# zqqqqz2000/MixGRPO

Hardware: AMD Instinct MI355X
Metric: GRPO train-step images/sec, FLUX.1-dev 1024^2 (higher is better)
Workload: dtype bf16

## Files before the change

### include/mixgrpo_hip.h

```cpp
#ifndef MIXGRPO_HIP_H
#define MIXGRPO_HIP_H
#include <stdint.h>
#ifdef __cplusplus
extern "C" {
#endif

int mgx_version(void);
const char* mgx_last_error(void);

typedef struct {
  float sigma_x0;
  float c_x;
  float c_v;
  float dt_mean;
  float sd_noise;
  float dt_det;
  float den;
  float log_sd;
  float log_c;
} mgx_flow_coeffs;

long mgx_logp_workspace_elems(int B, long n);

int mgx_flow_step_fwd(const float* x, const uint16_t* v, const uint16_t* noise, const float* prev_in,
// ... 11 lines not shown
  float s_b;
  float one_m_s;
  float s_sq;
  float half_eta2;
  float sd;
  float den;
} mgx_dance_coeffs;

int mgx_dance_step_fwd(const float* x, const uint16_t* v, const float* noise, const float* prev_in,
                       float* prev_out, float* x0_out, float* logp, double* ws, int B, long n,
                       const mgx_dance_coeffs* k , int sde, void* stream);
int mgx_dance_step_bwd(const float* x, const uint16_t* v, const float* prev, const float* g_logp, uint16_t* dv,
                       int B, long n, const mgx_dance_coeffs* k , int sde, void* stream);

typedef struct {
  int order;
  int sde;
  float sigma_x0;
  float inv_r0;
  float inv_r1;
  float c_r;
  float inv_r01;
  float cm[4];
  float cx[4];
  float sd_noise;
  float den;
  float log_sd;
  float log_c;
} mgx_dpm_coeffs;

int mgx_dpm_step_fwd(const float* sample, const uint16_t* v, const float* m1, const float* m2, const float* noise,
                     float* x_out, float* x0_out, float* logp, double* ws, int B, long n,
                     const mgx_dpm_coeffs* k , void* stream);

int mgx_dpm_step_bwd(const float* sample, const uint16_t* v, const float* x_t, const float* g_logp, uint16_t* dv, int B,
                     long n, const mgx_dpm_coeffs* k , float sigma_b, void* stream);

int mgx_x0_pred(const float* sample, const uint16_t* v, float* x0_out, long total, float sigma_x0, void* stream);

int mgx_pack_latents(const void* in, void* out, int B, int C, int H, int W, int elem_size, void* stream);
int mgx_unpack_latents(const void* in, void* out, int B, int C, int H, int W, int elem_size, void* stream);

int mgx_group_advantage(const float* rewards, float* out, int n, int G, float trimmed_ratio, float weight,
                        int accumulate, void* stream);
int mgx_global_advantage(const float* rewards, const float* gathered, float* out, int n, int n_all, void* stream);

int mgx_grpo_loss(const float* new_logp, const float* old_logp, const float* adv, int B, float clip_range,
                  float adv_clip_max, float kl_coeff, float denom, float* loss, float* policy, float* kl,
                  float* clip_frac, float* g_logp, void* stream);

enum { MGX_EPI_BIAS = 0, MGX_EPI_BIAS_GELU = 1, MGX_EPI_BIAS_GATE_RES = 2, MGX_EPI_F32_ACC = 3, MGX_EPI_DGELU = 4 };

int mgx_gemm_bf16(const uint16_t* A, const uint16_t* W, const uint16_t* bias, void* C, const uint16_t* gate,
                  uint16_t* aux, long ldaux, int M, int N, int K, long lda, long a_rpb, long a_bstride, long ldw, long ldc,
                  long c_rpb, long c_bstride, long gate_ld, int epilogue, float beta, void* stream);
long mgx_gemm_sk_workspace_elems(void);
int mgx_gemm_bf16_sk(const uint16_t* A, const uint16_t* W, const uint16_t* bias, void* C, const uint16_t* gate,
                     uint16_t* aux, long ldaux, int M, int N, int K, long lda, long a_rpb, long a_bstride, long ldw, long ldc,
                     long c_rpb, long c_bstride, long gate_ld, int epilogue, float beta, float* sk_workspace,
                     long sk_workspace_elems, void* stream);
int mgx_linear_qk_norm_rope(const uint16_t* X, const uint16_t* Wqk, const uint16_t* bias, const float* wq, const float* wk,
                            const float* cos, const float* sin, const float* cos_sin_pairs ,
                            uint16_t* Q, uint16_t* K, int B, int H, int S, int rows_per_batch, int s0, int Kdim, long ldx,
                            long ldw, float q_scale, void* stream);

int mgx_linear_bf16_t(const uint16_t* X, const uint16_t* W, const uint16_t* bias, uint16_t* Ct, int tokens, int F, int K,
                      long ldx, long ldw, long ld_ct, long tok_rpb, long ct_bstride, float* sk_workspace,
                      long sk_workspace_elems, void* stream);

int mgx_gemm_bf16_pair(const uint16_t* A1, const uint16_t* W1, const uint16_t* bias1, void* C1, const uint16_t* gate1,
                       uint16_t* aux1, int M1, long a1_rpb, long a1_bstride, long c1_rpb, long c1_bstride,
                       const uint16_t* A2, const uint16_t* W2, const uint16_t* bias2, void* C2, const uint16_t* gate2,
                       uint16_t* aux2, int M2, long a2_rpb, long a2_bstride, long c2_rpb, long c2_bstride, int N, int K,
                       long lda, long ldw, long ldc, long ldaux, long gate_ld, int epilogue, float beta,
                       float* sk_workspace, long sk_workspace_elems, void* stream);

long mgx_transpose_partial_elems(int M, int N);
int mgx_transpose_bf16(const uint16_t* in, uint16_t* out, float* colsum_partial, float* colsum_out, float colsum_beta,
                       int M, int N, long ld_in, long in_rpb, long in_bstride, long ld_out, void* stream);

int mgx_ln_modulate_fwd(const uint16_t* x, long ldx, long x_rpb, long x_bstride, const uint16_t* shift,
                        const uint16_t* scale, long mod_ld, uint16_t* y, long ldy, float* stats, long M, int D,
                        void* stream);
long mgx_ln_modulate_bwd_workspace(long M, long rpb, int D);
int mgx_ln_modulate_bwd(const uint16_t* dy, long lddy, const uint16_t* x, long ldx, long x_rpb, long x_bstride,
                        const uint16_t* scale, long mod_ld, uint16_t* dx, long lddx, long dx_rpb, long dx_bstride,
                        int accumulate, uint16_t* dshift, uint16_t* dscale, float* ws, long M, int D, void* stream);

int mgx_qk_norm_rope_fwd(const uint16_t* qkv, long ld, const float* wq, const float* wk, const float* cos,
                         const float* sin, uint16_t* Q, uint16_t* K, uint16_t* Vt, uint16_t* V, uint16_t* Qt,
                         uint16_t* Kt, int B, int H, int S, int Sp, int rows_per_batch, int s0, void* stream);
int mgx_qk_norm_rope_fwd_qs(const uint16_t* qkv, long ld, const float* wq, const float* wk, const float* cos,
                            const float* sin, uint16_t* Q, uint16_t* K, uint16_t* Vt, uint16_t* V, uint16_t* Qt,
                            uint16_t* Kt, int B, int H, int S, int Sp, int rows_per_batch, int s0, float q_scale,
                            void* stream);
long mgx_qk_norm_rope_bwd_workspace(int B, int H, int rows_per_batch);
int mgx_qk_norm_rope_bwd(const uint16_t* qkv, long ld, const float* wq, const float* wk, const float* cos,
                         const float* sin, const uint16_t* dQ, const uint16_t* dK, const uint16_t* dV, uint16_t* dqkv,
                         long ld_dqkv , float* gwq, float* gwk, float* ws, int B,
                         int H, int S, int Sp, int rows_per_batch, int s0, void* stream);

int mgx_qk_norm_rope_bwd_qs(const uint16_t* qkv, long ld, const float* wq, const float* wk, const float* cos,
                            const float* sin, const uint16_t* dQ, const uint16_t* dK, const uint16_t* dV, uint16_t* dqkv,
                            long ld_dqkv, float* gwq, float* gwk, float* ws, int B, int H, int S, int Sp,
                            int rows_per_batch, int s0, float q_scale, void* stream);

int mgx_attn_fwd(const uint16_t* Q, const uint16_t* K, const uint16_t* Vt, uint16_t* O, float* lse, int B, int H, int S,
                 int Sp, long ldo, long o_bstride, float scale, void* stream);

int mgx_attn_fwd_log2(const uint16_t* Q2, const uint16_t* K, const uint16_t* Vt, uint16_t* O, float* lse, int B, int H,
                      int S, int Sp, long ldo, long o_bstride, void* stream);

int mgx_attn_fwd_path(int B, int H, int S, int Sp, long ldo, long o_bstride);
int mgx_attn_bwd_path(int B, int H, int S, int Sp, long ldo, long o_bstride);

int mgx_attn_fp8_quantize(const uint16_t* Q, const uint16_t* K, const uint16_t* Vt, uint8_t* Q8, uint8_t* K8,
                          uint8_t* V8t, float* amax, int B, int H, int S, int Sp, void* stream);
int mgx_attn_fwd_fp8(const uint8_t* Q8, const uint8_t* K8, const uint8_t* V8t, const float* amax, uint16_t* O,
                     float* lse, int B, int H, int S, int Sp, long ldo, long o_bstride, float scale, void* stream);

int mgx_attn_bwd(const uint16_t* Q, const uint16_t* K, const uint16_t* V, const uint16_t* Qt, const uint16_t* Kt,
                 const uint16_t* O, const uint16_t* dO, const float* lse, float* delta, uint16_t* dOt, uint16_t* dQ,
                 uint16_t* dK, uint16_t* dV, int B, int H, int S, int Sp, long ldo, long o_bstride, float scale,
                 void* stream);

int mgx_skinny_linear(const uint16_t* x, long ldx, const uint16_t* W, long ldw, const uint16_t* bias, uint16_t* out,
                      long ldo, int Bn, int N, int K, void* stream);
int mgx_skinny_wgrad(const uint16_t* dout, long ldd, const uint16_t* x, long ldx, float* dW, long ldw, float* dbias,
                     int Bn, int N, int K, void* stream);
long mgx_skinny_dgrad_workspace(int Bn, int K);
int mgx_skinny_dgrad(const uint16_t* dout, long ldd, const uint16_t* W, long ldw, uint16_t* dx, long lddx, float* ws,
                     int Bn, int N, int K, int accumulate, void* stream);
int mgx_ew_bf16(const uint16_t* a, const uint16_t* b, uint16_t* y, long n, int op, void* stream);
int mgx_sincos_embed(const float* t, uint16_t* out, int Bn, void* stream);
int mgx_cast_f32_bf16(const float* x, uint16_t* y, long n, void* stream);
int mgx_cast_bf16_f32(const uint16_t* x, float* y, long n, float scale, void* stream);
int mgx_transpose_gelu_bf16(const uint16_t* in, uint16_t* out, int M, int N, long ld_in, long ld_out, void* stream);
int mgx_gelu_bf16(const uint16_t* x, long ldx, uint16_t* y, long ldy, long M, int N, void* stream);
long mgx_gate_bwd_workspace(long batches, long rows_per_batch, int D);
int mgx_gate_bwd(const uint16_t* dout, long ldd, long d_bstride, const uint16_t* y, long ldy, const uint16_t* gate,
                 long gate_ld, uint16_t* dy, long lddy, uint16_t* dgate, float* ws, int batches, long rows_per_batch,
                 int D, void* stream);

long mgx_sqnorm_workspace(void);
int mgx_sqnorm_f32(const float* g, long n, double* ws, float* out, float beta, void* stream);
int mgx_adamw_step(float* w, uint16_t* w16, const float* g, float* m, float* v, long n, double lr, double beta1,
                   double beta2, double eps, double weight_decay, int step, const float* gnorm_sq, float max_norm,
                   float grad_scale, void* stream);
int mgx_scale_f32(float* x, long n, float s, void* stream);


int mgx_conv3x3_nhwc(const uint16_t* x, const uint16_t* Wt, const uint16_t* bias, uint16_t* out, long ld_out,
                     const uint16_t* ones, int H, int W, int C, int Cout, int residual, void* stream);
long mgx_group_norm_workspace(long M, int C, int G);
int mgx_group_norm_nhwc(const uint16_t* x, long ld, const uint16_t* gamma, const uint16_t* beta, uint16_t* out, long out_row,
                        long out_px, float* ws, int H, int W, int C, int G, float eps, int silu, void* stream);
int mgx_upsample2x_pad_nhwc(const uint16_t* x, uint16_t* out, int H, int W, int C, void* stream);
int mgx_latents_to_pad_nhwc(const float* z, uint16_t* out, int Cin, int H, int W, int C, void* stream);
int mgx_nhwc_to_image(const uint16_t* x, long ld, uint16_t* img, int Cout, int H, int W, void* stream);
int mgx_softmax_rows_f32(const float* S, long lds, uint16_t* P, long ldp, int M, int n, float scale, void* stream);

#ifdef __cplusplus
}
#endif
#endif
```

### mixgrpo_amd/_lib.py

```python
import ctypes as C
import os

import torch

_HERE = os.path.dirname(os.path.abspath(__file__))
LIB_PATH = os.path.join(_HERE, "csrc", "libmixgrpo_hip.so")


class MgxError(RuntimeError):
    pass


class FlowCoeffs(C.Structure):
    _fields_ = [(n, C.c_float) for n in ("sigma_x0", "c_x", "c_v", "dt_mean", "sd_noise", "dt_det", "den", "log_sd",
                                         "log_c")]


class DanceCoeffs(C.Structure):
    _fields_ = [(n, C.c_float) for n in ("ds_r", "s_r", "ds", "ds_b", "s_b", "one_m_s", "s_sq", "half_eta2", "sd", "den")]


class DpmCoeffs(C.Structure):
    _fields_ = [("order", C.c_int), ("sde", C.c_int), ("sigma_x0", C.c_float), ("inv_r0", C.c_float),
                ("inv_r1", C.c_float), ("c_r", C.c_float), ("inv_r01", C.c_float), ("cm", C.c_float * 4),
                ("cx", C.c_float * 4), ("sd_noise", C.c_float), ("den", C.c_float), ("log_sd", C.c_float),
                ("log_c", C.c_float)]


_P = C.c_void_p
_I = C.c_int
_L = C.c_long
_F = C.c_float
_D = C.c_double

SIGNATURES = {
    "mgx_version": (_I, []),
    "mgx_last_error": (C.c_char_p, []),
    "mgx_logp_workspace_elems": (_L, [_I, _L]),
    "mgx_flow_step_fwd": (_I, [_P] * 9 + [_I, _L, C.POINTER(FlowCoeffs), _I, _P]),
    "mgx_flow_step_bwd": (_I, [_P] * 5 + [_I, _L, C.POINTER(FlowCoeffs), _P]),
    "mgx_dance_step_fwd": (_I, [_P] * 8 + [_I, _L, C.POINTER(DanceCoeffs), _I, _P]),
    "mgx_dance_step_bwd": (_I, [_P] * 5 + [_I, _L, C.POINTER(DanceCoeffs), _I, _P]),
    "mgx_dpm_step_fwd": (_I, [_P] * 9 + [_I, _L, C.POINTER(DpmCoeffs), _P]),
    "mgx_dpm_step_bwd": (_I, [_P] * 5 + [_I, _L, C.POINTER(DpmCoeffs), _F, _P]),
    "mgx_x0_pred": (_I, [_P, _P, _P, _L, _F, _P]),
    "mgx_pack_latents": (_I, [_P, _P, _I, _I, _I, _I, _I, _P]),
    "mgx_unpack_latents": (_I, [_P, _P, _I, _I, _I, _I, _I, _P]),
    "mgx_group_advantage": (_I, [_P, _P, _I, _I, _F, _F, _I, _P]),
    "mgx_global_advantage": (_I, [_P, _P, _P, _I, _I, _P]),
    "mgx_grpo_loss": (_I, [_P, _P, _P, _I, _F, _F, _F, _F, _P, _P, _P, _P, _P, _P]),
    "mgx_gemm_bf16": (_I, [_P] * 6 + [_L, _I, _I, _I] + [_L] * 8 + [_I, _F, _P]),
    "mgx_gemm_sk_workspace_elems": (_L, []),
    "mgx_gemm_bf16_sk": (_I, [_P] * 6 + [_L, _I, _I, _I] + [_L] * 8 + [_I, _F, _P, _L, _P]),
    "mgx_linear_bf16_t": (_I, [_P] * 4 + [_I] * 3 + [_L] * 5 + [_P, _L, _P]),
    "mgx_linear_qk_norm_rope": (_I, [_P] * 10 + [_I] * 6 + [_L, _L, _F, _P]),
    "mgx_gemm_bf16_pair": (_I, ([_P] * 6 + [_I] + [_L] * 4) * 2 + [_I, _I] + [_L] * 5 + [_I, _F, _P, _L, _P]),
    "mgx_transpose_partial_elems": (_L, [_I, _I]),
    "mgx_transpose_bf16": (_I, [_P, _P, _P, _P, _F, _I, _I, _L, _L, _L, _L, _P]),
    "mgx_ln_modulate_fwd": (_I, [_P, _L, _L, _L, _P, _P, _L, _P, _L, _P, _L, _I, _P]),
    "mgx_ln_modulate_bwd_workspace": (_L, [_L, _L, _I]),
    "mgx_ln_modulate_bwd": (_I, [_P, _L, _P, _L, _L, _L, _P, _L, _P, _L, _L, _L, _I, _P, _P, _P, _L, _I, _P]),
    "mgx_qk_norm_rope_fwd": (_I, [_P, _L] + [_P] * 10 + [_I] * 6 + [_P]),
    "mgx_qk_norm_rope_fwd_qs": (_I, [_P, _L] + [_P] * 10 + [_I] * 6 + [_F, _P]),
    "mgx_qk_norm_rope_bwd_workspace": (_L, [_I, _I, _I]),
    "mgx_qk_norm_rope_bwd": (_I, [_P, _L] + [_P] * 8 + [_L] + [_P] * 3 + [_I] * 6 + [_P]),
    "mgx_qk_norm_rope_bwd_qs": (_I, [_P, _L] + [_P] * 8 + [_L] + [_P] * 3 + [_I] * 6 + [_F, _P]),
    "mgx_attn_fwd": (_I, [_P] * 5 + [_I] * 4 + [_L, _L, _F, _P]),
    "mgx_attn_fwd_log2": (_I, [_P] * 5 + [_I] * 4 + [_L, _L, _P]),
    "mgx_attn_fwd_path": (_I, [_I] * 4 + [_L, _L]),
    "mgx_attn_bwd_path": (_I, [_I] * 4 + [_L, _L]),
    "mgx_attn_fp8_quantize": (_I, [_P] * 7 + [_I] * 4 + [_P]),
    "mgx_attn_fwd_fp8": (_I, [_P] * 6 + [_I] * 4 + [_L, _L, _F, _P]),
    "mgx_attn_bwd": (_I, [_P] * 13 + [_I] * 4 + [_L, _L, _F, _P]),
    "mgx_skinny_linear": (_I, [_P, _L, _P, _L, _P, _P, _L, _I, _I, _I, _P]),
    "mgx_skinny_wgrad": (_I, [_P, _L, _P, _L, _P, _L, _P, _I, _I, _I, _P]),
    "mgx_skinny_dgrad_workspace": (_L, [_I, _I]),
    "mgx_conv3x3_nhwc": (_I, [_P, _P, _P, _P, _L, _P, _I, _I, _I, _I, _I, _P]),
    "mgx_group_norm_workspace": (_L, [_L, _I, _I]),
    "mgx_group_norm_nhwc": (_I, [_P, _L, _P, _P, _P, _L, _L, _P, _I, _I, _I, _I, _F, _I, _P]),
    "mgx_upsample2x_pad_nhwc": (_I, [_P, _P, _I, _I, _I, _P]),
    "mgx_latents_to_pad_nhwc": (_I, [_P, _P, _I, _I, _I, _I, _P]),
    "mgx_nhwc_to_image": (_I, [_P, _L, _P, _I, _I, _I, _P]),
    "mgx_softmax_rows_f32": (_I, [_P, _L, _P, _L, _I, _I, _F, _P]),
    "mgx_skinny_dgrad": (_I, [_P, _L, _P, _L, _P, _L, _P, _I, _I, _I, _I, _P]),
    "mgx_ew_bf16": (_I, [_P, _P, _P, _L, _I, _P]),
    "mgx_sincos_embed": (_I, [_P, _P, _I, _P]),
    "mgx_cast_f32_bf16": (_I, [_P, _P, _L, _P]),
    "mgx_cast_bf16_f32": (_I, [_P, _P, _L, _F, _P]),
    "mgx_gelu_bf16": (_I, [_P, _L, _P, _L, _L, _I, _P]),
    "mgx_transpose_gelu_bf16": (_I, [_P, _P, _I, _I, _L, _L, _P]),
    "mgx_gate_bwd_workspace": (_L, [_L, _L, _I]),
    "mgx_gate_bwd": (_I, [_P, _L, _L, _P, _L, _P, _L, _P, _L, _P, _P, _I, _L, _I, _P]),
    "mgx_sqnorm_workspace": (_L, []),
    "mgx_sqnorm_f32": (_I, [_P, _L, _P, _P, _F, _P]),
    "mgx_adamw_step": (_I, [_P, _P, _P, _P, _P, _L, _D, _D, _D, _D, _D, _I, _P, _F, _F, _P]),
    "mgx_scale_f32": (_I, [_P, _L, _F, _P]),
}

_lib = None


def lib():
    global _lib
    if _lib is None:
        if not os.path.exists(LIB_PATH):
            raise MgxError(f"{LIB_PATH} is missing: run `python -m mixgrpo_amd.build` (hipcc, gfx950). "
                           "There is no CPU fallback for the product path.")
        h = C.CDLL(LIB_PATH)
        h.mgx_version.restype = _I
        v = h.mgx_version()
        if v < 0:
            raise MgxError(f"{LIB_PATH} is a DIAGNOSTIC build (mgx_version() = {v}, -DMGX_DIAGNOSTIC_BUILD): its timing-only "
                           "switches compute wrong results.  Rebuild with `python -m mixgrpo_amd.build --force`.")
        for name, (res, args) in SIGNATURES.items():
            fn = getattr(h, name)
            fn.restype = res
            fn.argtypes = args
        _lib = h
    return _lib


def check(code):
    if code != 0:
        raise MgxError(f"libmixgrpo_hip error {code}: {lib().mgx_last_error().decode()}")


def ptr(t):
    if t is None:
        return None
    if not t.is_cuda:
        raise MgxError("mixgrpo_amd HIP ops need device tensors (got a CPU tensor); there is no CPU path")
    if not t.is_contiguous():
        raise MgxError("mixgrpo_amd HIP ops need contiguous tensors")
    return t.data_ptr()


def stream():
    return torch.cuda.current_stream().cuda_stream


_ws_cache = {}


def logp_workspace(B, n, device):
    need = lib().mgx_logp_workspace_elems(B, n)
    key = (device, torch.cuda.current_stream().cuda_stream)
    w = _ws_cache.get(key)
    if w is None or w.numel() < need:
        w = torch.empty(max(need, 4096), dtype=torch.float64, device=device)
        _ws_cache[key] = w
    return w
```

### mixgrpo_amd/csrc/gemm.hip

```cpp
#include "../../include/mixgrpo_hip.h"
#include "common.h"

#include <cmath>
#include <cstdlib>

namespace {

constexpr int BM = 128, BN = 128, BK = 64;
constexpr int NT = 256;

struct RowMap {
  long ld;
  long rpb;
  long bstride;
};

__device__ __forceinline__ long row_off(const RowMap& r, long m) {
  const uint32_t rpb = (uint32_t)r.rpb;
  const uint32_t b = (uint32_t)m / rpb;
  return (long)b * r.bstride + (long)((uint32_t)m - b * rpb) * r.ld;
}

enum Epi { EPI_BIAS = 0, EPI_BIAS_GELU = 1, EPI_BIAS_GATE_RES = 2, EPI_F32_ACC = 3, EPI_BIAS_MULAUX = 4,
           EPI_QKNORM = 5 ,
           EPI_QKNORM_P = 6  };

struct GemmArgs {
  const bf16_raw* A;
  const bf16_raw* W;
  const bf16_raw* bias;
  void* C;
  const bf16_raw* gate;
  bf16_raw* aux;
  long ldaux;
  long gate_ld;
  int M, N, K;
  RowMap a, c;
  long ldw;
  float beta;
  int rowwise_ok;
  int span32;
  int band;
  int conv_shift;
  long conv_dy, conv_dx;
  float* sk_ws;
  int sk_minparts;
  int m_split;
  long a1_off, w1_off;
  long a2_off, w2_off;
  RowMap a2, c2;
  void* C2;
  const bf16_raw* bias2;
  const bf16_raw* gate2;
  bf16_raw* aux2;
  int bias_rows;
  long col_rpb, col_bstride;
  const float* qn_wq;
  const float* qn_wk;
  const float* qn_cos;
  const float* qn_sin;
  const float* qn_cs2;
  bf16_raw* qn_Q;
  bf16_raw* qn_K;
  int qn_H, qn_S, qn_s0, qn_dmodel;
  float qn_qscale;
};

template <bool PAIR>
__device__ __forceinline__ GemmArgs seg_args(const GemmArgs& g, long& m0) {
  if (!PAIR || g.m_split == 0 || m0 < g.m_split) {
    GemmArgs r = g;
    if (PAIR && g.m_split) r.M = g.m_split;
    return r;
  }
  GemmArgs r = g;
  r.C = g.C2; r.c = g.c2; r.bias = g.bias2; r.gate = g.gate2; r.aux = g.aux2;
  r.M = g.M - g.m_split;
  m0 -= g.m_split;
  return r;
}

template <bool CONV>
__device__ __forceinline__ long a_koff(const GemmArgs& g, int kt) {
  if (!CONV) return (long)kt * BK;
// ... 152 lines not shown
    *reinterpret_cast<uint4*>(base_ + 2 * RS * 128) = ra2;                       \
    *reinterpret_cast<uint4*>(base_ + 3 * RS * 128) = ra3;                       \
    *reinterpret_cast<uint4*>(base_ + TB) = rw0;                                 \
    *reinterpret_cast<uint4*>(base_ + TB + RS * 128) = rw1;                      \
    *reinterpret_cast<uint4*>(base_ + TB + 2 * RS * 128) = rw2;                  \
    *reinterpret_cast<uint4*>(base_ + TB + 3 * RS * 128) = rw3;                  \
  } while (0)

  f32x4 acc[NTL][MT];
#pragma unroll
  for (int i = 0; i < NTL; ++i)
#pragma unroll
    for (int j = 0; j < MT; ++j) acc[i][j] = f32x4{0.f, 0.f, 0.f, 0.f};

  const int fr = lane & 15, fq = lane >> 4;
  const int nkt = g.K / BK;
  LOAD_TILE(0);
  STORE_TILE(0);
  __syncthreads();
  int cur = 0;
  for (int kt = 0; kt < nkt; ++kt) {
    if (kt + 1 < nkt) LOAD_TILE(kt + 1);
    const char* sa = smem + cur * STAGE;
    const char* sw = sa + TB;
    s16x8 fa[2][MT], fw[2][NTL];
#pragma unroll
    for (int ks = 0; ks < 2; ++ks) {
#pragma unroll
      for (int t = 0; t < NTL; ++t) {
        const int rw_ = wn * 64 + t * 16 + fr;
        fw[ks][t] = *reinterpret_cast<const s16x8*>(sw + rw_ * 128 + swz(rw_, ks * 4 + fq) * 16);
      }
#pragma unroll
      for (int t = 0; t < MT; ++t) {
        const int ra_ = wm * (MT * 16) + t * 16 + fr;
        fa[ks][t] = *reinterpret_cast<const s16x8*>(sa + ra_ * 128 + swz(ra_, ks * 4 + fq) * 16);
      }
    }
#pragma unroll
    for (int ks = 0; ks < 2; ++ks) {
#pragma unroll
      for (int j = 0; j < MT; ++j)
#pragma unroll
        for (int i = 0; i < NTL; ++i)
          acc[i][j] = __builtin_amdgcn_mfma_f32_16x16x32_bf16(fw[ks][i], fa[ks][j], acc[i][j], 0, 0, 0);
    }
    if (kt + 1 < nkt) STORE_TILE(cur ^ 1);
    __syncthreads();
    cur ^= 1;
  }
#undef LOAD_TILE
#undef STORE_TILE

  gemm_epilogue<EPI, MT, NTL>(g, acc, lane, m0, n0, wm, wn);
}

__global__ void __launch_bounds__(256) transpose_kernel(const bf16_raw* __restrict__ in, bf16_raw* __restrict__ out,
                                                        float* __restrict__ part, int M, int N, RowMap im, long ldo) {
  __shared__ bf16_raw tile[64][66];
  const int m0 = blockIdx.y * 64, n0 = blockIdx.x * 64;
  const int tx = threadIdx.x & 63, ty = threadIdx.x >> 6;
  for (int r = ty; r < 64; r += 4) {
    const long m = m0 + r;
    const int n = n0 + tx;
    bf16_raw v = 0;
    if (m < M && n < N) v = in[row_off(im, m) + n];
    tile[r][tx] = v;
  }
  __syncthreads();
  for (int r = ty; r < 64; r += 4) {
    const int n = n0 + r;
    const long m = m0 + tx;
    if (n < N && m < ldo) out[(long)n * ldo + m] = (m < M) ? tile[tx][r] : (bf16_raw)0;
  }
  if (part && m0 < M) {
    if (ty == 0) {
      float s = 0.f;
      for (int r = 0; r < 64; ++r) s += bf2f(tile[r][tx]);
      if (n0 + tx < N) part[(long)blockIdx.y * N + n0 + tx] = s;
    }
  }
}

__device__ __forceinline__ uint32_t lo16(uint32_t a, uint32_t b) { return __builtin_amdgcn_perm(b, a, 0x05040100); }
__device__ __forceinline__ uint32_t hi16(uint32_t a, uint32_t b) { return __builtin_amdgcn_perm(b, a, 0x07060302); }
template <bool GELU>
__global__ void __launch_bounds__(256) transpose8_kernel(const bf16_raw* __restrict__ in, bf16_raw* __restrict__ out,
                                                         float* __restrict__ part, int M, int N, RowMap im, long ldo) {
  __shared__ float cs[16][129];
  const int tx = (threadIdx.x & 7) | (((threadIdx.x >> 6) & 1) << 3), ty = ((threadIdx.x >> 3) & 7) | ((threadIdx.x >> 7) << 3);
  const int n0 = blockIdx.x * 128 + tx * 8;
  const long m0 = (long)blockIdx.y * 128 + ty * 8;
  uint32_t r[8][4];
  float csum[8];
#pragma unroll
  for (int j = 0; j < 8; ++j) csum[j] = 0.f;
  const bool ncol_ok = n0 < N;
#pragma unroll
  for (int i = 0; i < 8; ++i) {
    const long m = m0 + i;
    uint4 v = make_uint4(0, 0, 0, 0);
    if (ncol_ok && m < M) v = *reinterpret_cast<const uint4*>(in + row_off(im, m) + n0);
    if (GELU && ncol_ok && m < M) {
      auto gl = [](uint32_t u) {
        return (uint32_t)f2bf(gelu_tanh_f(bf2f(u & 0xffff))) | ((uint32_t)f2bf(gelu_tanh_f(bf2f(u >> 16))) << 16);
      };
      v.x = gl(v.x); v.y = gl(v.y); v.z = gl(v.z); v.w = gl(v.w);
    }
    r[i][0] = v.x; r[i][1] = v.y; r[i][2] = v.z; r[i][3] = v.w;
    if (part) {
      csum[0] += bf2f(v.x & 0xffff); csum[1] += bf2f(v.x >> 16); csum[2] += bf2f(v.y & 0xffff); csum[3] += bf2f(v.y >> 16);
      csum[4] += bf2f(v.z & 0xffff); csum[5] += bf2f(v.z >> 16); csum[6] += bf2f(v.w & 0xffff); csum[7] += bf2f(v.w >> 16);
    }
  }
  if (ncol_ok && m0 < ldo) {
#pragma unroll
    for (int c2 = 0; c2 < 4; ++c2) {
      uint4 e, o;
      e.x = lo16(r[0][c2], r[1][c2]); e.y = lo16(r[2][c2], r[3][c2]); e.z = lo16(r[4][c2], r[5][c2]); e.w = lo16(r[6][c2], r[7][c2]);
      o.x = hi16(r[0][c2], r[1][c2]); o.y = hi16(r[2][c2], r[3][c2]); o.z = hi16(r[4][c2], r[5][c2]); o.w = hi16(r[6][c2], r[7][c2]);
      *reinterpret_cast<uint4*>(out + (long)(n0 + 2 * c2) * ldo + m0) = e;
      *reinterpret_cast<uint4*>(out + (long)(n0 + 2 * c2 + 1) * ldo + m0) = o;
    }
  }
  if (part) {
#pragma unroll
    for (int j = 0; j < 8; ++j) cs[ty][tx * 8 + j] = csum[j];
    __syncthreads();
    if (threadIdx.x < 128) {
      float t = 0.f;
#pragma unroll
      for (int k = 0; k < 16; ++k) t += cs[k][threadIdx.x];
      const int n = blockIdx.x * 128 + threadIdx.x;
      if (n < N && (long)blockIdx.y * 128 < M) part[(long)blockIdx.y * N + n] = t;
    }
  }
}

__global__ void __launch_bounds__(256) colsum_finish_kernel(const float* __restrict__ part, float* __restrict__ out, int nblk,
                                                            int N, float beta) {
  __shared__ float red[4][64];
  const int cx = threadIdx.x & 63, ky = threadIdx.x >> 6;
  const int n = blockIdx.x * 64 + cx;
  float s = 0.f;
  if (n < N)
    for (int b = ky; b < nblk; b += 4) s += part[(long)b * N + n];
  red[ky][cx] = s;
  __syncthreads();
  if (ky == 0 && n < N) out[n] = beta * out[n] + ((red[0][cx] + red[1][cx]) + (red[2][cx] + red[3][cx]));
}

__device__ __forceinline__ int wperm(int p) { return (p >> 5) * 32 + ((p & 15) >> 2) * 8 + ((p >> 4) & 1) * 4 + (p & 3); }
__device__ __forceinline__ int lane_feat(int fq, int t) { return (t >> 1) * 32 + fq * 8 + (t & 1) * 4; }

__device__ __forceinline__ void unpack8(const uint4& u, float* v) {
  v[0] = bf2f(u.x & 0xffff); v[1] = bf2f(u.x >> 16); v[2] = bf2f(u.y & 0xffff); v[3] = bf2f(u.y >> 16);
  v[4] = bf2f(u.z & 0xffff); v[5] = bf2f(u.z >> 16); v[6] = bf2f(u.w & 0xffff); v[7] = bf2f(u.w >> 16);
}
__device__ __forceinline__ uint4 pack8(const float* v) {
  uint4 o;
  o.x = (uint32_t)f2bf(v[0]) | ((uint32_t)f2bf(v[1]) << 16);
  o.y = (uint32_t)f2bf(v[2]) | ((uint32_t)f2bf(v[3]) << 16);
  o.z = (uint32_t)f2bf(v[4]) | ((uint32_t)f2bf(v[5]) << 16);
  o.w = (uint32_t)f2bf(v[6]) | ((uint32_t)f2bf(v[7]) << 16);
  return o;
}

__device__ __forceinline__ float vmul1(float a, float b) { float r; asm("v_mul_f32 %0, %1, %2" : "=v"(r) : "v"(a), "v"(b)); return r; }
// ... 926 lines not shown
  MGX_REQUIRE(X && Wqk && wq && wk && cos && sin && Q && K, "null argument");
  MGX_REQUIRE(!cos_sin_pairs || (uintptr_t)cos_sin_pairs % 16 == 0, "pair table must be 16-byte aligned");
  MGX_REQUIRE(B > 0 && H > 0 && rows_per_batch > 0 && s0 >= 0 && s0 + rows_per_batch <= S && Kdim > 0 && q_scale > 0.f, "bad sizes");
  static const int off = getenv("MGX_GEMM_QKNORM") ? atoi(getenv("MGX_GEMM_QKNORM")) == 0 : 0;
  const long tokens = (long)B * rows_per_batch;
  const int dmodel = H * 128;
  const bool ok = !off && dmodel % 256 == 0 && rows_per_batch % 128 == 0 && Kdim % BK == 0 && ldx % 8 == 0 && ldw % 8 == 0 &&
                  tokens < (1L << 31) && ((uintptr_t)X % 16 == 0) && ((uintptr_t)Wqk % 16 == 0) && ((uintptr_t)Q % 16 == 0) &&
                  ((uintptr_t)K % 16 == 0) && ((uintptr_t)cos % 16 == 0) && ((uintptr_t)sin % 16 == 0) &&
                  ((uintptr_t)wq % 16 == 0) && ((uintptr_t)wk % 16 == 0) && (!bias || (uintptr_t)bias % 16 == 0);
  if (!ok) return 1;
  GemmArgs g{};
  g.A = X; g.W = Wqk; g.bias = bias; g.C = Q;
  g.M = (int)tokens; g.N = 2 * dmodel; g.K = Kdim;
  g.a = RowMap{ldx, 1L << 30, 0};
  g.c = RowMap{128, rows_per_batch, 0};
  g.ldw = ldw;
  g.conv_shift = -1;
  g.rowwise_ok = 1;
  g.span32 = (tokens * ldx) * 2 < (1L << 32) && ((long)g.N * ldw) * 2 < (1L << 32);
  g.qn_wq = wq; g.qn_wk = wk; g.qn_cos = cos; g.qn_sin = sin; g.qn_cs2 = cos_sin_pairs; g.qn_Q = Q; g.qn_K = K;
  g.qn_H = H; g.qn_S = S; g.qn_s0 = s0; g.qn_dmodel = dmodel; g.qn_qscale = q_scale;
  if (!persistent_ok(g)) return 1;
  return cos_sin_pairs ? launch<EPI_QKNORM_P>(g, (hipStream_t)stream) : launch<EPI_QKNORM>(g, (hipStream_t)stream);
}

extern "C" int mgx_gemm_bf16(const uint16_t* A, const uint16_t* W, const uint16_t* bias, void* C, const uint16_t* gate,
                             uint16_t* aux, long ldaux, int M, int N, int K, long lda, long a_rpb, long a_bstride, long ldw, long ldc,
                             long c_rpb, long c_bstride, long gate_ld, int epilogue, float beta, void* stream) {
  return mgx_gemm_bf16_sk(A, W, bias, C, gate, aux, ldaux, M, N, K, lda, a_rpb, a_bstride, ldw, ldc, c_rpb, c_bstride, gate_ld,
                          epilogue, beta, nullptr, 0, stream);
}

extern "C" int mgx_conv3x3_nhwc(const uint16_t* x, const uint16_t* Wt, const uint16_t* bias, uint16_t* out, long ld_out,
                                const uint16_t* ones, int H, int Wd, int C, int Cout, int residual, void* stream) {
  MGX_REQUIRE(x && Wt && out && H > 0 && Wd > 0, "bad argument");
  MGX_REQUIRE(C == 64 || C == 128 || C == 256 || C == 512, "channels per tap must be 64, 128, 256 or 512 (pad with zeros)");
  MGX_REQUIRE(Cout > 0 && Cout % 4 == 0 && ld_out >= Cout && ld_out % 4 == 0, "output channels must be a multiple of 4");
  MGX_REQUIRE(!residual || ones, "the residual form needs a vector of Cout ones (bf16)");
  MGX_REQUIRE(((uintptr_t)x % 16 == 0) && ((uintptr_t)Wt % 16 == 0) && ((uintptr_t)out % 8 == 0), "operands must be 16-byte aligned");
  const long Wp = Wd + 2;
  MGX_REQUIRE((long)(H + 2) * Wp * C * 2 < (1L << 32) && (long)Cout * 9 * C * 2 < (1L << 32), "image too large for one call");
  GemmArgs g{};
  g.A = x; g.W = Wt; g.bias = bias; g.C = out; g.gate = residual ? ones : nullptr; g.aux = nullptr; g.ldaux = 0; g.gate_ld = 0;
  g.M = H * Wd; g.N = Cout; g.K = 9 * C;
  g.a = RowMap{C, Wd, Wp * C};
  g.c = RowMap{ld_out, 1L << 30, 0};
  g.ldw = 9L * C;
  g.beta = 0.f;
  g.conv_shift = C == 64 ? 0 : (C == 128 ? 1 : (C == 256 ? 2 : 3));
  g.conv_dy = Wp * C; g.conv_dx = C;
  g.sk_ws = nullptr; g.sk_minparts = 0; g.m_split = 0;
  g.rowwise_ok = (Cout % 8 == 0) && (ld_out % 8 == 0) && ((uintptr_t)out % 16 == 0) && (!bias || (uintptr_t)bias % 16 == 0) &&
                 (!residual || (uintptr_t)ones % 16 == 0);
  g.span32 = 1;
  hipStream_t st = (hipStream_t)stream;
  return residual ? launch<EPI_BIAS_GATE_RES, true>(g, st) : launch<EPI_BIAS, true>(g, st);
}

extern "C" long mgx_transpose_partial_elems(int M, int N) { return (long)cdiv(M, 64) * N; }

extern "C" int mgx_transpose_bf16(const uint16_t* in, uint16_t* out, float* colsum_partial, float* colsum_out,
                                  float colsum_beta, int M, int N, long ld_in, long in_rpb, long in_bstride, long ld_out,
                                  void* stream) {
  MGX_REQUIRE(in && out && M > 0 && N > 0, "bad argument");
  MGX_REQUIRE(ld_out >= M, "output leading dimension must cover M");
  MGX_REQUIRE((colsum_partial == nullptr) == (colsum_out == nullptr), "column sums need both workspace and output");
  hipStream_t st = (hipStream_t)stream;
  const bool fast = N % 8 == 0 && ld_in % 8 == 0 && in_bstride % 8 == 0 && ld_out % 8 == 0 &&
                    ((uintptr_t)in % 16 == 0) && ((uintptr_t)out % 16 == 0);
  if (fast) {
    dim3 grid(cdiv(N, 128), cdiv(ld_out, 128));
    transpose8_kernel<false><<<grid, 256, 0, st>>>(in, out, colsum_partial, M, N, RowMap{ld_in, in_rpb < (1L << 30) ? in_rpb : (1L << 30), in_bstride}, ld_out);
    if (colsum_out) colsum_finish_kernel<<<cdiv(N, 64), 256, 0, st>>>(colsum_partial, colsum_out, cdiv(M, 128), N, colsum_beta);
  } else {
    dim3 grid(cdiv(N, 64), cdiv(ld_out, 64));
    transpose_kernel<<<grid, 256, 0, st>>>(in, out, colsum_partial, M, N, RowMap{ld_in, in_rpb < (1L << 30) ? in_rpb : (1L << 30), in_bstride}, ld_out);
    if (colsum_out) colsum_finish_kernel<<<cdiv(N, 64), 256, 0, st>>>(colsum_partial, colsum_out, cdiv(M, 64), N, colsum_beta);
  }
  MGX_CHECK_LAUNCH();
  return MGX_OK;
}

extern "C" int mgx_transpose_gelu_bf16(const uint16_t* in, uint16_t* out, int M, int N, long ld_in, long ld_out, void* stream) {
  MGX_REQUIRE(in && out && M > 0 && N > 0, "bad argument");
  MGX_REQUIRE(ld_out >= M, "output leading dimension must cover M");
  MGX_REQUIRE(N % 8 == 0 && ld_in % 8 == 0 && ld_out % 8 == 0 && ((uintptr_t)in % 16 == 0) && ((uintptr_t)out % 16 == 0),
              "rows must be 16-byte addressable");
  dim3 grid(cdiv(N, 128), cdiv(ld_out, 128));
  transpose8_kernel<true><<<grid, 256, 0, (hipStream_t)stream>>>(in, out, nullptr, M, N, RowMap{ld_in, 1L << 30, 0}, ld_out);
  MGX_CHECK_LAUNCH();
  return MGX_OK;
}

extern "C" int mgx_gelu_bf16(const uint16_t* x, long ldx, uint16_t* y, long ldy, long M, int N, void* stream) {
  MGX_REQUIRE(x && y && M > 0 && N > 0, "bad argument");
  MGX_REQUIRE(N % 8 == 0 && ldx % 8 == 0 && ldy % 8 == 0 && ((uintptr_t)x % 16 == 0) && ((uintptr_t)y % 16 == 0),
              "rows must be 16-byte addressable");
  const long total = M * (N / 8);
  const int grid = (int)((total + 255) / 256 < 256L * 32 ? (total + 255) / 256 : 256L * 32);
  gelu_rows_kernel<<<grid, 256, 0, (hipStream_t)stream>>>(x, ldx, y, ldy, M, N / 8);
  MGX_CHECK_LAUNCH();
  return MGX_OK;
}
```

### mixgrpo_amd/csrc/norm.hip

```cpp
#include "../../include/mixgrpo_hip.h"
#include "common.h"

namespace {

struct RowMap {
  long ld, rpb, bstride;
};
__device__ __forceinline__ long row_off(const RowMap& r, long m) {
  const long b = m / r.rpb;
  return b * r.bstride + (m - b * r.rpb) * r.ld;
}

constexpr int LN_MAXV = 8;

__device__ __forceinline__ void unpack8(const uint4& u, float* f) {
  f[0] = bf2f(u.x & 0xffff); f[1] = bf2f(u.x >> 16); f[2] = bf2f(u.y & 0xffff); f[3] = bf2f(u.y >> 16);
  f[4] = bf2f(u.z & 0xffff); f[5] = bf2f(u.z >> 16); f[6] = bf2f(u.w & 0xffff); f[7] = bf2f(u.w >> 16);
}
__device__ __forceinline__ uint4 pack8(const float* f) {
  uint4 u;
  u.x = (uint32_t)f2bf(f[0]) | ((uint32_t)f2bf(f[1]) << 16);
  u.y = (uint32_t)f2bf(f[2]) | ((uint32_t)f2bf(f[3]) << 16);
  u.z = (uint32_t)f2bf(f[4]) | ((uint32_t)f2bf(f[5]) << 16);
  u.w = (uint32_t)f2bf(f[6]) | ((uint32_t)f2bf(f[7]) << 16);
  return u;
}

template <int NV>
__global__ void __launch_bounds__(256) ln_mod_fwd_kernel(const bf16_raw* __restrict__ x, RowMap xm,
                                                         const bf16_raw* __restrict__ shift,
                                                         const bf16_raw* __restrict__ scale, long mod_ld,
                                                         bf16_raw* __restrict__ y, long ldy, float* __restrict__ stats,
                                                         long M) {
  const long m = (long)blockIdx.x * 4 + (threadIdx.x >> 6);
  if (m >= M) return;
  const int lane = threadIdx.x & 63;
  const long b = m / xm.rpb;
  const bf16_raw* xr = x + row_off(xm, m);
  float v[NV][8];
  float s = 0.f;
#pragma unroll
  for (int i = 0; i < NV; ++i) {
    unpack8(*reinterpret_cast<const uint4*>(xr + (i * 64 + lane) * 8), v[i]);
#pragma unroll
    for (int j = 0; j < 8; ++j) s += v[i][j];
  }
  const float D = (float)(NV * 512);
  const float mean = wave_sum(s) / D;
  float q = 0.f;
#pragma unroll
  for (int i = 0; i < NV; ++i)
#pragma unroll
    for (int j = 0; j < 8; ++j) {
      const float d = v[i][j] - mean;
      q += d * d;
    }
  const float rstd = rsqrtf(wave_sum(q) / D + 1e-6f);
  if (stats && lane == 0) {
    stats[2 * m] = mean;
    stats[2 * m + 1] = rstd;
  }
  const bf16_raw* sh = shift + b * mod_ld;
  const bf16_raw* sc = scale + b * mod_ld;
#pragma unroll
  for (int i = 0; i < NV; ++i) {
    const int c = (i * 64 + lane) * 8;
    float fs[8], fc[8], o[8];
    unpack8(*reinterpret_cast<const uint4*>(sh + c), fs);
    unpack8(*reinterpret_cast<const uint4*>(sc + c), fc);
#pragma unroll
    for (int j = 0; j < 8; ++j) o[j] = (v[i][j] - mean) * rstd * rbf(1.0f + fc[j]) + fs[j];
    *reinterpret_cast<uint4*>(y + m * ldy + c) = pack8(o);
  }
}

constexpr int LN_BWD_ROWS = 32;
template <int NV>
__global__ void __launch_bounds__(256) ln_mod_bwd_kernel(const bf16_raw* __restrict__ dy, long lddy,
                                                         const bf16_raw* __restrict__ x, RowMap xm,
                                                         const bf16_raw* __restrict__ scale, long mod_ld,
                                                         bf16_raw* __restrict__ dx, RowMap dxm, int accumulate,
                                                         float* __restrict__ part, long M, int blocks_per_batch) {
  extern __shared__ float red[];
  const int D = NV * 512;
  const int lane = threadIdx.x & 63, w = threadIdx.x >> 6;
  const long b = blockIdx.x / blocks_per_batch;
  const long r0 = (long)(blockIdx.x % blocks_per_batch) * LN_BWD_ROWS;
  const bf16_raw* sc = scale + b * mod_ld;
  float a_sh[NV][8], a_sc[NV][8];
#pragma unroll
  for (int i = 0; i < NV; ++i)
#pragma unroll
    for (int j = 0; j < 8; ++j) a_sh[i][j] = a_sc[i][j] = 0.f;

  auto row_ok = [&](int rr) { return rr < LN_BWD_ROWS && r0 + rr < xm.rpb && b * xm.rpb + r0 + rr < M; };
  uint4 nx[NV], ng[NV], nold[NV];
  auto fetch = [&](int rr) {
    const long m = b * xm.rpb + r0 + rr;
    const bf16_raw* xr = x + row_off(xm, m);
    const bf16_raw* dxr = dx + row_off(dxm, m);
#pragma unroll
    for (int i = 0; i < NV; ++i) {
      nx[i] = *reinterpret_cast<const uint4*>(xr + (i * 64 + lane) * 8);
      ng[i] = *reinterpret_cast<const uint4*>(dy + m * lddy + (i * 64 + lane) * 8);
      nold[i] = accumulate ? *reinterpret_cast<const uint4*>(dxr + (i * 64 + lane) * 8) : make_uint4(0, 0, 0, 0);
    }
  };
  if (row_ok(w)) fetch(w);
  for (int rr = w; row_ok(rr); rr += 4) {
    const long m = b * xm.rpb + r0 + rr;
    bf16_raw* dxr = dx + row_off(dxm, m);
    float v[NV][8], g[NV][8];
    uint4 oldp[NV];
    float s = 0.f;
#pragma unroll
    for (int i = 0; i < NV; ++i) {
      unpack8(nx[i], v[i]);
      unpack8(ng[i], g[i]);
      oldp[i] = nold[i];
#pragma unroll
      for (int j = 0; j < 8; ++j) s += v[i][j];
    }
    if (row_ok(rr + 4)) fetch(rr + 4);
    const float Df = (float)D;
    const float mean = wave_sum(s) / Df;
    float q = 0.f;
#pragma unroll
    for (int i = 0; i < NV; ++i)
#pragma unroll
      for (int j = 0; j < 8; ++j) {
        const float d = v[i][j] - mean;
        q += d * d;
      }
    const float rstd = rsqrtf(wave_sum(q) / Df + 1e-6f);
    float c1 = 0.f, c2 = 0.f;
#pragma unroll
    for (int i = 0; i < NV; ++i) {
      float fc[8];
      unpack8(*reinterpret_cast<const uint4*>(sc + (i * 64 + lane) * 8), fc);
#pragma unroll
      for (int j = 0; j < 8; ++j) {
        const float xh = (v[i][j] - mean) * rstd;
        const float gx = g[i][j] * rbf(1.0f + fc[j]);
        a_sh[i][j] += g[i][j];
        a_sc[i][j] += g[i][j] * xh;
        c1 += gx;
        c2 += gx * xh;
        v[i][j] = xh;
        g[i][j] = gx;
      }
    }
    c1 = wave_sum(c1) / Df;
    c2 = wave_sum(c2) / Df;
#pragma unroll
    for (int i = 0; i < NV; ++i) {
      float o[8];
// ... 96 lines not shown
    float2 cc[U], ss[U];
    bool ok[U];
#pragma unroll
    for (int u = 0; u < U; ++u) {
      const int t = t0 + w * 16 + i0 + u;
      ok[u] = t < a.rows_per_batch;
      const int tc = ok[u] ? t : a.rows_per_batch - 1;
      const long row = (long)b * a.rows_per_batch + tc;
      const bf16_raw* base = a.qkv + row * a.ld + hh * HD + 2 * lane;
      uq[u] = *reinterpret_cast<const uint32_t*>(base);
      uk[u] = *reinterpret_cast<const uint32_t*>(base + dmodel);
      uv[u] = has_v ? *reinterpret_cast<const uint32_t*>(base + 2 * dmodel) : 0u;
      const long so = (long)(a.s0 + tc) * HD + 2 * lane;
      cc[u] = *reinterpret_cast<const float2*>(a.cos + so);
      ss[u] = *reinterpret_cast<const float2*>(a.sin + so);
    }
#pragma unroll
    for (int u = 0; u < U; ++u) {
      if (!ok[u]) continue;
      const int tl = w * 16 + i0 + u;
      const int s = a.s0 + t0 + tl;
      if (has_v) *reinterpret_cast<uint32_t*>(&vt[tl][2 * lane]) = uv[u];
      const float c0 = cc[u].x, c1 = cc[u].y, s0 = ss[u].x, s1 = ss[u].y;
      const long o = (((long)b * a.H + hh) * a.S + s) * HD + 2 * lane;
      {
        const float x0 = bf2f(uq[u] & 0xffff), x1 = bf2f(uq[u] >> 16);
        const float r = rsqrtf(head_sum(x0 * x0 + x1 * x1) / 128.f + 1e-6f);
        const float y0 = x0 * r * wq0, y1 = x1 * r * wq1;
        const uint32_t pk = (uint32_t)f2bf(y0 * c0 - y1 * s0) | ((uint32_t)f2bf(y1 * c1 + y0 * s1) << 16);
        *reinterpret_cast<uint32_t*>(a.Q + o) = pk;
        if (EMIT_T) *reinterpret_cast<uint32_t*>(&qts[tl][2 * lane]) = pk;
      }
      {
        const float x0 = bf2f(uk[u] & 0xffff), x1 = bf2f(uk[u] >> 16);
        const float r = rsqrtf(head_sum(x0 * x0 + x1 * x1) / 128.f + 1e-6f);
        const float y0 = x0 * r * wk0, y1 = x1 * r * wk1;
        const uint32_t pk = (uint32_t)f2bf(y0 * c0 - y1 * s0) | ((uint32_t)f2bf(y1 * c1 + y0 * s1) << 16);
        *reinterpret_cast<uint32_t*>(a.K + o) = pk;
        if (EMIT_T) *reinterpret_cast<uint32_t*>(&kts[tl][2 * lane]) = pk;
      }
      if (EMIT_T) *reinterpret_cast<uint32_t*>(a.V + o) = uv[u];
    }
  }
  if (!EMIT_T && !has_v) return;
  __syncthreads();
  const int ntok = min(64, a.rows_per_batch - t0);
  const int nmat = EMIT_T ? 3 : 1;
  for (int mat = 0; mat < nmat; ++mat) {
    bf16_raw (*tile)[130] = mat == 0 ? vt : (mat == 1 ? qts : kts);
    bf16_raw* outp = mat == 0 ? a.Vt : (mat == 1 ? a.Qt : a.Kt);
    for (int id = threadIdx.x; id < 128 * 8; id += 256) {
      const int d = id >> 3, c = id & 7;
      bf16_raw* dst = outp + (((long)b * a.H + hh) * HD + d) * a.Sp + a.s0 + t0 + c * 8;
      if (c * 8 + 8 <= ntok && (((a.s0 + t0) & 7) == 0)) {
        uint4 u;
        u.x = (uint32_t)tile[c * 8 + 0][d] | ((uint32_t)tile[c * 8 + 1][d] << 16);
        u.y = (uint32_t)tile[c * 8 + 2][d] | ((uint32_t)tile[c * 8 + 3][d] << 16);
        u.z = (uint32_t)tile[c * 8 + 4][d] | ((uint32_t)tile[c * 8 + 5][d] << 16);
        u.w = (uint32_t)tile[c * 8 + 6][d] | ((uint32_t)tile[c * 8 + 7][d] << 16);
        *reinterpret_cast<uint4*>(dst) = u;
      } else {
        for (int j = 0; j < 8; ++j)
          if (c * 8 + j < ntok) dst[j] = tile[c * 8 + j][d];
      }
    }
  }
}

struct QkBwdArgs {
  const bf16_raw* qkv;
  long ld;
  const float* wq;
  const float* wk;
  const float* cos;
  const float* sin;
  const bf16_raw* dQ;
  const bf16_raw* dK;
  const bf16_raw* dV;
  bf16_raw* dqkv;
  long ldo;
  float* part;
  int H, S, Sp, rows_per_batch, s0;
  float q_scale;
};

__global__ void __launch_bounds__(256) qk_norm_rope_bwd_kernel(QkBwdArgs a) {
  __shared__ float red[4][2][128];
  const int lane = threadIdx.x & 63, w = threadIdx.x >> 6;
  const int hh = blockIdx.y, b = blockIdx.z;
  const int t0 = blockIdx.x * 64;
  const int HD = 128;
  const long dmodel = (long)a.H * HD;
  const float wq0 = a.wq[2 * lane], wq1 = a.wq[2 * lane + 1];
  const float wk0 = a.wk[2 * lane], wk1 = a.wk[2 * lane + 1];
  float gq0 = 0.f, gq1 = 0.f, gk0 = 0.f, gk1 = 0.f;
  constexpr int U = 4;
  for (int i0 = 0; i0 < 16; i0 += U) {
    uint32_t ux[U][2], ug[U][2], uv[U];
    float2 cc[U], ss[U];
    bool ok[U];
#pragma unroll
    for (int u = 0; u < U; ++u) {
      const int t = t0 + w * 16 + i0 + u;
      ok[u] = t < a.rows_per_batch;
      const int tc = ok[u] ? t : a.rows_per_batch - 1;
      const long row = (long)b * a.rows_per_batch + tc;
      const int s = a.s0 + tc;
      const bf16_raw* base = a.qkv + row * a.ld + hh * HD + 2 * lane;
      const long o = (((long)b * a.H + hh) * a.S + s) * HD + 2 * lane;
      ux[u][0] = *reinterpret_cast<const uint32_t*>(base);
      ux[u][1] = *reinterpret_cast<const uint32_t*>(base + dmodel);
      ug[u][0] = *reinterpret_cast<const uint32_t*>(a.dQ + o);
      ug[u][1] = *reinterpret_cast<const uint32_t*>(a.dK + o);
      uv[u] = *reinterpret_cast<const uint32_t*>(a.dV + o);
      cc[u] = *reinterpret_cast<const float2*>(a.cos + (long)s * HD + 2 * lane);
      ss[u] = *reinterpret_cast<const float2*>(a.sin + (long)s * HD + 2 * lane);
    }
#pragma unroll
    for (int u = 0; u < U; ++u) {
      if (!ok[u]) continue;
      const int t = t0 + w * 16 + i0 + u;
      const long row = (long)b * a.rows_per_batch + t;
      bf16_raw* obase = a.dqkv + row * a.ldo + hh * HD + 2 * lane;
      const float c0 = cc[u].x, c1 = cc[u].y, s0 = ss[u].x, s1 = ss[u].y;
#pragma unroll
      for (int which = 0; which < 2; ++which) {
        const float w0 = which ? wk0 : wq0, w1 = which ? wk1 : wq1;
        const float x0 = bf2f(ux[u][which] & 0xffff), x1 = bf2f(ux[u][which] >> 16);
        const float gs = which ? 1.f : a.q_scale;
        const float go0 = bf2f(ug[u][which] & 0xffff) * gs, go1 = bf2f(ug[u][which] >> 16) * gs;
        const float gy0 = go0 * c0 + go1 * s1;
        const float gy1 = -go0 * s0 + go1 * c1;
        const float r = rsqrtf(head_sum(x0 * x0 + x1 * x1) / 128.f + 1e-6f);
        if (which) { gk0 += gy0 * x0 * r; gk1 += gy1 * x1 * r; } else { gq0 += gy0 * x0 * r; gq1 += gy1 * x1 * r; }
        const float gz0 = gy0 * w0, gz1 = gy1 * w1;
        const float dot = wave_sum(gz0 * x0 + gz1 * x1) / 128.f;
        const float dx0 = r * gz0 - x0 * r * r * r * dot;
        const float dx1 = r * gz1 - x1 * r * r * r * dot;
        *reinterpret_cast<uint32_t*>(obase + which * dmodel) = (uint32_t)f2bf(dx0) | ((uint32_t)f2bf(dx1) << 16);
      }
      *reinterpret_cast<uint32_t*>(obase + 2 * dmodel) = uv[u];
    }
  }
  red[w][0][2 * lane] = gq0; red[w][0][2 * lane + 1] = gq1;
  red[w][1][2 * lane] = gk0; red[w][1][2 * lane + 1] = gk1;
  __syncthreads();
  const long blk = ((long)blockIdx.z * gridDim.y + blockIdx.y) * gridDim.x + blockIdx.x;
  {
    const int which = threadIdx.x >> 7, c = threadIdx.x & 127;
    a.part[(blk * 2 + which) * 128 + c] = red[0][which][c] + red[1][which][c] + red[2][which][c] + red[3][which][c];
  }
}

constexpr int QK_FIN_G = 128;
__global__ void __launch_bounds__(256) qk_bwd_partial_kernel(const float* __restrict__ part, float* __restrict__ mid,
                                                             long nblocks) {
  float s = 0.f;
  for (long k = blockIdx.x; k < nblocks; k += QK_FIN_G) s += part[k * 256 + threadIdx.x];
  mid[(long)blockIdx.x * 256 + threadIdx.x] = s;
}

__global__ void __launch_bounds__(256) qk_bwd_finish_kernel(const float* __restrict__ part, float* __restrict__ gq,
                                                            float* __restrict__ gk, long nblocks) {
  __shared__ float red[16][17];
  const int which = blockIdx.x >> 3, c0 = (blockIdx.x & 7) * 16;
  const int cx = threadIdx.x & 15, ry = threadIdx.x >> 4;
  float s = 0.f;
  for (long k = ry; k < nblocks; k += 16) s += part[(k * 2 + which) * 128 + c0 + cx];
  red[ry][cx] = s;
  __syncthreads();
  if (ry == 0) {
    float t = 0.f;
#pragma unroll
    for (int i = 0; i < 16; ++i) t += red[i][cx];
    float* dst = which ? gk : gq;
    dst[c0 + cx] += t;
  }
}

}

extern "C" int mgx_ln_modulate_fwd(const uint16_t* x, long ldx, long x_rpb, long x_bstride, const uint16_t* shift,
                                   const uint16_t* scale, long mod_ld, uint16_t* y, long ldy, float* stats, long M, int D,
                                   void* stream) {
  MGX_REQUIRE(x && shift && scale && y && M > 0, "bad argument");
  MGX_REQUIRE(D % 512 == 0 && D <= 4096, "feature size must be a multiple of 512 up to 4096");
  MGX_REQUIRE(ldx % 8 == 0 && ldy % 8 == 0 && mod_ld % 8 == 0 && x_bstride % 8 == 0, "16-byte row alignment");
  hipStream_t st = (hipStream_t)stream;
  const RowMap xm{ldx, x_rpb, x_bstride};
  const int grid = cdiv(M, 4);
  switch (D / 512) {
#define CASE(nv) case nv: ln_mod_fwd_kernel<nv><<<grid, 256, 0, st>>>(x, xm, shift, scale, mod_ld, y, ldy, stats, M); break;
    CASE(1) CASE(2) CASE(3) CASE(4) CASE(5) CASE(6) CASE(7) CASE(8)
#undef CASE
  }
  MGX_CHECK_LAUNCH();
  return MGX_OK;
}

extern "C" long mgx_ln_modulate_bwd_workspace(long M, long rpb, int D) {
  const long batches = (M + rpb - 1) / rpb;
  const long bpb = ((rpb < M ? rpb : M) + LN_BWD_ROWS - 1) / LN_BWD_ROWS;
  return batches * bpb * 2 * D;
}

extern "C" int mgx_ln_modulate_bwd(const uint16_t* dy, long lddy, const uint16_t* x, long ldx, long x_rpb, long x_bstride,
                                   const uint16_t* scale, long mod_ld, uint16_t* dx, long lddx, long dx_rpb,
                                   long dx_bstride, int accumulate, uint16_t* dshift, uint16_t* dscale, float* ws, long M,
                                   int D, void* stream) {
  MGX_REQUIRE(dy && x && scale && dx && dshift && dscale && ws && M > 0, "bad argument");
  MGX_REQUIRE(D % 512 == 0 && D <= 4096, "feature size must be a multiple of 512 up to 4096");
  MGX_REQUIRE(x_rpb == dx_rpb, "x and dx must be batched alike");
  hipStream_t st = (hipStream_t)stream;
  const long rpb = x_rpb < M ? x_rpb : M;
  const int batches = cdiv(M, rpb);
  const int bpb = cdiv(rpb, LN_BWD_ROWS);
  const RowMap xm{ldx, rpb, x_bstride}, dxm{lddx, rpb, dx_bstride};
  const size_t lds = (size_t)2 * D * sizeof(float);
  switch (D / 512) {
#define CASE(nv)                                                                                                  \
  case nv:                                                                                                        \
    ln_mod_bwd_kernel<nv><<<batches * bpb, 256, lds, st>>>(dy, lddy, x, xm, scale, mod_ld, dx, dxm, accumulate, ws, M, bpb); \
    break;
    CASE(1) CASE(2) CASE(3) CASE(4) CASE(5) CASE(6) CASE(7) CASE(8)
#undef CASE
  }
  ln_mod_bwd_finish_kernel<<<dim3(cdiv(D, 64), batches), 256, 0, st>>>(ws, dshift, dscale, mod_ld, D, bpb);
  MGX_CHECK_LAUNCH();
  return MGX_OK;
}

extern "C" int mgx_qk_norm_rope_fwd_qs(const uint16_t* qkv, long ld, const float* wq, const float* wk, const float* cos,
                                       const float* sin, uint16_t* Q, uint16_t* K, uint16_t* Vt, uint16_t* V, uint16_t* Qt,
                                       uint16_t* Kt, int B, int H, int S, int Sp, int rows_per_batch, int s0, float q_scale,
                                       void* stream) {
  MGX_REQUIRE(qkv && wq && wk && cos && sin && Q && K, "null argument");
  MGX_REQUIRE((V != nullptr) == (Qt != nullptr) && (V != nullptr) == (Kt != nullptr), "V, Qt, Kt come together");
  MGX_REQUIRE(Vt || !V, "Vt may only be left out (V^T written by mgx_linear_bf16_t) without the backward's extra layouts");
  MGX_REQUIRE(B > 0 && H > 0 && rows_per_batch > 0 && s0 >= 0 && s0 + rows_per_batch <= S && Sp >= S, "bad sizes");
  MGX_REQUIRE(ld == 3L * H * 128, "qkv rows must be [q | k | v] of H*128 each");
  MGX_REQUIRE(q_scale > 0.f, "q_scale must be positive");
  QkArgs a{qkv, ld, wq, wk, cos, sin, Q, K, Vt, V, Qt, Kt, H, S, Sp, rows_per_batch, s0, q_scale};
  dim3 grid(cdiv(rows_per_batch, 64), H, B);
  if (V) qk_norm_rope_fwd_kernel<true><<<grid, 256, 0, (hipStream_t)stream>>>(a);
  else qk_norm_rope_fwd_kernel<false><<<grid, 256, 0, (hipStream_t)stream>>>(a);
  MGX_CHECK_LAUNCH();
  return MGX_OK;
}

extern "C" int mgx_qk_norm_rope_fwd(const uint16_t* qkv, long ld, const float* wq, const float* wk, const float* cos,
                                    const float* sin, uint16_t* Q, uint16_t* K, uint16_t* Vt, uint16_t* V, uint16_t* Qt,
                                    uint16_t* Kt, int B, int H, int S, int Sp, int rows_per_batch, int s0, void* stream) {
  return mgx_qk_norm_rope_fwd_qs(qkv, ld, wq, wk, cos, sin, Q, K, Vt, V, Qt, Kt, B, H, S, Sp, rows_per_batch, s0, 1.0f, stream);
}

extern "C" long mgx_qk_norm_rope_bwd_workspace(int B, int H, int rows_per_batch) {
  return ((long)cdiv(rows_per_batch, 64) * H * B + QK_FIN_G) * 2 * 128;
}

extern "C" int mgx_qk_norm_rope_bwd_qs(const uint16_t* qkv, long ld, const float* wq, const float* wk, const float* cos,
                                       const float* sin, const uint16_t* dQ, const uint16_t* dK, const uint16_t* dV,
                                       uint16_t* dqkv, long ld_dqkv, float* gwq, float* gwk, float* ws, int B, int H, int S,
                                       int Sp, int rows_per_batch, int s0, float q_scale, void* stream) {
  MGX_REQUIRE(qkv && wq && wk && cos && sin && dQ && dK && dV && dqkv && gwq && gwk && ws, "null argument");
  MGX_REQUIRE(ld == 3L * H * 128, "qkv rows must be [q | k | v] of H*128 each");
  MGX_REQUIRE(ld_dqkv >= ld && ld_dqkv % 2 == 0, "dqkv rows must hold [dq | dk | dv] and keep 4-byte alignment");
  hipStream_t st = (hipStream_t)stream;
  QkBwdArgs a{qkv, ld, wq, wk, cos, sin, dQ, dK, dV, dqkv, ld_dqkv, ws, H, S, Sp, rows_per_batch, s0, q_scale};
  dim3 grid(cdiv(rows_per_batch, 64), H, B);
  qk_norm_rope_bwd_kernel<<<grid, 256, 0, st>>>(a);
  const long nblocks = (long)grid.x * grid.y * grid.z;
  float* mid = ws + nblocks * 256;
  qk_bwd_partial_kernel<<<QK_FIN_G, 256, 0, st>>>(ws, mid, nblocks);
  qk_bwd_finish_kernel<<<16, 256, 0, st>>>(mid, gwq, gwk, QK_FIN_G);
  MGX_CHECK_LAUNCH();
  return MGX_OK;
}

extern "C" int mgx_qk_norm_rope_bwd(const uint16_t* qkv, long ld, const float* wq, const float* wk, const float* cos,
                                    const float* sin, const uint16_t* dQ, const uint16_t* dK, const uint16_t* dV,
                                    uint16_t* dqkv, long ld_dqkv, float* gwq, float* gwk, float* ws, int B, int H, int S,
                                    int Sp, int rows_per_batch, int s0, void* stream) {
  return mgx_qk_norm_rope_bwd_qs(qkv, ld, wq, wk, cos, sin, dQ, dK, dV, dqkv, ld_dqkv, gwq, gwk, ws, B, H, S, Sp, rows_per_batch,
                                 s0, 1.0f, stream);
}
```

### mixgrpo_amd/csrc/small.hip

```cpp
#include "../../include/mixgrpo_hip.h"
#include "common.h"

namespace {

__global__ void __launch_bounds__(256) skinny_linear_kernel(const bf16_raw* __restrict__ x, long ldx,
                                                            const bf16_raw* __restrict__ W, long ldw,
                                                            const bf16_raw* __restrict__ bias,
                                                            bf16_raw* __restrict__ out, long ldo, int Bn, int N, int K) {
  __shared__ f32x4 red[3][64];
  const int lane = threadIdx.x & 63, w = threadIdx.x >> 6;
  const int n0 = blockIdx.x * 16;
  const int fr = lane & 15, fq = lane >> 4;
  int nrow = n0 + fr;
  if (nrow >= N) nrow = N - 1;
  int brow = fr < Bn ? fr : Bn - 1;
  const int kchunk = ((K / 32 + 3) / 4) * 32;
  const int kbeg = min(w * kchunk, K), kend = min(kbeg + kchunk, K);
  const bf16_raw* wp = W + (long)nrow * ldw + fq * 8;
  const bf16_raw* xp = x + (long)brow * ldx + fq * 8;
  f32x4 acc = {0.f, 0.f, 0.f, 0.f};
  int k = kbeg;
  for (; k + 128 <= kend; k += 128) {
    s16x8 a0 = *reinterpret_cast<const s16x8*>(wp + k), a1 = *reinterpret_cast<const s16x8*>(wp + k + 32);
    s16x8 a2 = *reinterpret_cast<const s16x8*>(wp + k + 64), a3 = *reinterpret_cast<const s16x8*>(wp + k + 96);
    s16x8 b0 = *reinterpret_cast<const s16x8*>(xp + k), b1 = *reinterpret_cast<const s16x8*>(xp + k + 32);
    s16x8 b2 = *reinterpret_cast<const s16x8*>(xp + k + 64), b3 = *reinterpret_cast<const s16x8*>(xp + k + 96);
    acc = __builtin_amdgcn_mfma_f32_16x16x32_bf16(a0, b0, acc, 0, 0, 0);
    acc = __builtin_amdgcn_mfma_f32_16x16x32_bf16(a1, b1, acc, 0, 0, 0);
    acc = __builtin_amdgcn_mfma_f32_16x16x32_bf16(a2, b2, acc, 0, 0, 0);
    acc = __builtin_amdgcn_mfma_f32_16x16x32_bf16(a3, b3, acc, 0, 0, 0);
  }
  for (; k < kend; k += 32) {
    s16x8 a0 = *reinterpret_cast<const s16x8*>(wp + k);
    s16x8 b0 = *reinterpret_cast<const s16x8*>(xp + k);
    acc = __builtin_amdgcn_mfma_f32_16x16x32_bf16(a0, b0, acc, 0, 0, 0);
  }
  if (w > 0) red[w - 1][lane] = acc;
  __syncthreads();
  if (w > 0) return;
#pragma unroll
  for (int i = 0; i < 3; ++i) {
    const f32x4 o = red[i][lane];
    acc[0] += o[0]; acc[1] += o[1]; acc[2] += o[2]; acc[3] += o[3];
  }
  if (fr < Bn) {
#pragma unroll
    for (int r = 0; r < 4; ++r) {
      const int n = n0 + 4 * fq + r;
      if (n < N) {
        float v = acc[r];
        if (bias) v += bf2f(bias[n]);
        out[(long)fr * ldo + n] = f2bf(v);
      }
    }
  }
}

__global__ void __launch_bounds__(256) skinny_wgrad_kernel(const bf16_raw* __restrict__ dout, long ldd,
                                                           const bf16_raw* __restrict__ x, long ldx,
                                                           float* __restrict__ dW, long ldw, float* __restrict__ dbias,
                                                           int Bn, int N, int K) {
  const int n = blockIdx.y;
  float dn[16];
  float sb = 0.f;
#pragma unroll
  for (int b = 0; b < 16; ++b) {
    dn[b] = b < Bn ? bf2f(dout[(long)b * ldd + n]) : 0.f;
    sb += dn[b];
  }
  if (dbias && blockIdx.x == 0 && threadIdx.x == 0) dbias[n] += sb;
  for (int k = (blockIdx.x * 256 + threadIdx.x) * 4; k < K; k += gridDim.x * 256 * 4) {
    float4 g = *reinterpret_cast<float4*>(dW + (long)n * ldw + k);
    for (int b = 0; b < Bn; ++b) {
      const uint2 u = *reinterpret_cast<const uint2*>(x + (long)b * ldx + k);
      g.x += dn[b] * bf2f(u.x & 0xffff); g.y += dn[b] * bf2f(u.x >> 16);
      g.z += dn[b] * bf2f(u.y & 0xffff); g.w += dn[b] * bf2f(u.y >> 16);
    }
    *reinterpret_cast<float4*>(dW + (long)n * ldw + k) = g;
  }
}

constexpr int SD_G = 128;
__global__ void __launch_bounds__(256) skinny_dgrad_kernel(const bf16_raw* __restrict__ dout, long ldd,
                                                           const bf16_raw* __restrict__ W, long ldw, float* __restrict__ part,
// ... 56 lines not shown
  if (id >= (long)Bn * K) return;
  const int b = (int)(id / K), k = (int)(id - (long)b * K);
  float s = 0.f;
  for (int g = 0; g < SD_G; ++g) s += part[((long)g * Bn + b) * K + k];
  bf16_raw* o = dx + (long)b * lddx + k;
  const float r = rbf(s);
  *o = f2bf(accumulate ? bf2f(*o) + r : r);
}

__device__ __forceinline__ float silu_f(float x) { return x / (1.0f + expf(-x)); }

__global__ void ew_kernel(const bf16_raw* __restrict__ a, const bf16_raw* __restrict__ b, bf16_raw* __restrict__ y,
                          long n, int op) {
  for (long i = (long)blockIdx.x * blockDim.x + threadIdx.x; i < n; i += (long)gridDim.x * blockDim.x) {
    const float fa = bf2f(a[i]);
    float r;
    if (op == 0) r = silu_f(fa);
    else if (op == 1) {
      const float s = 1.0f / (1.0f + expf(-fa));
      r = bf2f(b[i]) * (s * (1.0f + fa * (1.0f - s)));
    } else if (op == 2) r = fa + bf2f(b[i]);
    else r = bf2f(y[i]) + fa;
    y[i] = f2bf(r);
  }
}

__global__ void sincos_embed_kernel(const float* __restrict__ t, bf16_raw* __restrict__ out, int Bn) {
  const int b = blockIdx.x, k = threadIdx.x;
  if (b >= Bn) return;
  const float f = expf(-logf(10000.0f) * (float)k / 128.0f);
  const float ang = t[b] * f;
  out[(long)b * 256 + k] = f2bf(cosf(ang));
  out[(long)b * 256 + 128 + k] = f2bf(sinf(ang));
}

__global__ void cast_f32_bf16_kernel(const float* __restrict__ x, bf16_raw* __restrict__ y, long n) {
  for (long i = ((long)blockIdx.x * blockDim.x + threadIdx.x) * 4; i < n; i += (long)gridDim.x * blockDim.x * 4) {
    const float4 v = *reinterpret_cast<const float4*>(x + i);
    uint2 o;
    o.x = (uint32_t)f2bf(v.x) | ((uint32_t)f2bf(v.y) << 16);
    o.y = (uint32_t)f2bf(v.z) | ((uint32_t)f2bf(v.w) << 16);
    *reinterpret_cast<uint2*>(y + i) = o;
  }
}

__global__ void cast_bf16_f32_kernel(const bf16_raw* __restrict__ x, float* __restrict__ y, long n, float scale) {
  for (long i = ((long)blockIdx.x * blockDim.x + threadIdx.x) * 8; i < n; i += (long)gridDim.x * blockDim.x * 8) {
    const uint4 u = *reinterpret_cast<const uint4*>(x + i);
    float4 a, b;
    a.x = bf2f(u.x & 0xffff) * scale; a.y = bf2f(u.x >> 16) * scale; a.z = bf2f(u.y & 0xffff) * scale; a.w = bf2f(u.y >> 16) * scale;
    b.x = bf2f(u.z & 0xffff) * scale; b.y = bf2f(u.z >> 16) * scale; b.z = bf2f(u.w & 0xffff) * scale; b.w = bf2f(u.w >> 16) * scale;
    *reinterpret_cast<float4*>(y + i) = a;
    *reinterpret_cast<float4*>(y + i + 4) = b;
  }
}

constexpr int GR_ROWS = 64;
__global__ void __launch_bounds__(256) gate_bwd_kernel(const bf16_raw* __restrict__ dout, long ldd, long d_rpb,
                                                       long d_bstride, const bf16_raw* __restrict__ y, long ldy,
                                                       const bf16_raw* __restrict__ gate, long gate_ld,
                                                       bf16_raw* __restrict__ dy, long lddy, float* __restrict__ part,
                                                       long rows_per_batch, int D, int blocks_per_batch) {
  const long b = blockIdx.y / blocks_per_batch;
  const long r0 = (long)(blockIdx.y % blocks_per_batch) * GR_ROWS;
  const int c = (blockIdx.x * 256 + threadIdx.x) * 2;
  if (c >= D) return;
  const uint32_t gu = *reinterpret_cast<const uint32_t*>(gate + b * gate_ld + c);
  const float g0 = bf2f(gu & 0xffff), g1 = bf2f(gu >> 16);
  float a0 = 0.f, a1 = 0.f;
  const long rend = min(r0 + (long)GR_ROWS, rows_per_batch);
  for (long r = r0; r < rend; ++r) {
    const long m = b * rows_per_batch + r;
    const uint32_t du = *reinterpret_cast<const uint32_t*>(dout + b * d_bstride + r * ldd + c);
    const uint32_t yu = *reinterpret_cast<const uint32_t*>(y + m * ldy + c);
    const float d0 = bf2f(du & 0xffff), d1 = bf2f(du >> 16);
    a0 += d0 * bf2f(yu & 0xffff);
    a1 += d1 * bf2f(yu >> 16);
    *reinterpret_cast<uint32_t*>(dy + m * lddy + c) = (uint32_t)f2bf(g0 * d0) | ((uint32_t)f2bf(g1 * d1) << 16);
  }
  part[(long)blockIdx.y * D + c] = a0;
  part[(long)blockIdx.y * D + c + 1] = a1;
}

__global__ void __launch_bounds__(256) gate_bwd_finish_kernel(const float* __restrict__ part, bf16_raw* __restrict__ dgate,
                                                              long gate_ld, int D, int blocks_per_batch) {
  __shared__ float red[4][64];
  const int b = blockIdx.y;
  const int cx = threadIdx.x & 63, ky = threadIdx.x >> 6;
  const int c = blockIdx.x * 64 + cx;
  float s = 0.f;
  if (c < D)
    for (int k = ky; k < blocks_per_batch; k += 4) s += part[((long)b * blocks_per_batch + k) * D + c];
  red[ky][cx] = s;
  __syncthreads();
  if (ky == 0 && c < D) dgate[(long)b * gate_ld + c] = f2bf((red[0][cx] + red[1][cx]) + (red[2][cx] + red[3][cx]));
}

}

extern "C" int mgx_skinny_linear(const uint16_t* x, long ldx, const uint16_t* W, long ldw, const uint16_t* bias,
                                 uint16_t* out, long ldo, int Bn, int N, int K, void* stream) {
  MGX_REQUIRE(x && W && out, "null operand");
  MGX_REQUIRE(Bn >= 1 && Bn <= 16, "skinny linear handles 1..16 rows");
  MGX_REQUIRE(K % 32 == 0 && ldx % 8 == 0 && ldw % 8 == 0, "K must be a multiple of 32 with 16-byte aligned rows");
  skinny_linear_kernel<<<cdiv(N, 16), 256, 0, (hipStream_t)stream>>>(x, ldx, W, ldw, bias, out, ldo, Bn, N, K);
  MGX_CHECK_LAUNCH();
  return MGX_OK;
}

extern "C" int mgx_skinny_wgrad(const uint16_t* dout, long ldd, const uint16_t* x, long ldx, float* dW, long ldw,
                                float* dbias, int Bn, int N, int K, void* stream) {
  MGX_REQUIRE(dout && x && dW, "null operand");
  MGX_REQUIRE(Bn >= 1 && Bn <= 16, "skinny wgrad handles 1..16 rows");
  MGX_REQUIRE(K % 4 == 0 && ldx % 4 == 0 && ldw % 4 == 0, "K must be a multiple of 4");
  int gx = cdiv(K, 1024);
  skinny_wgrad_kernel<<<dim3(gx, N), 256, 0, (hipStream_t)stream>>>(dout, ldd, x, ldx, dW, ldw, dbias, Bn, N, K);
  MGX_CHECK_LAUNCH();
  return MGX_OK;
}

extern "C" long mgx_skinny_dgrad_workspace(int Bn, int K) { return (long)SD_G * (Bn < 8 ? Bn : 8) * K; }

extern "C" int mgx_skinny_dgrad(const uint16_t* dout, long ldd, const uint16_t* W, long ldw, uint16_t* dx, long lddx,
                                float* ws, int Bn, int N, int K, int accumulate, void* stream) {
  MGX_REQUIRE(dout && W && dx && ws, "null operand");
  MGX_REQUIRE(Bn >= 1 && Bn <= 8, "skinny dgrad handles 1..8 rows per call");
  MGX_REQUIRE(N >= SD_G && K % 8 == 0 && ldw % 8 == 0 && ((uintptr_t)W % 16 == 0), "weight rows must be 16-byte addressable");
  hipStream_t st = (hipStream_t)stream;
  const size_t lds = (size_t)cdiv(N, SD_G) * 8 * sizeof(float);
  MGX_REQUIRE(lds <= 65536, "too many weight rows");
  skinny_dgrad_kernel<<<dim3(cdiv(K, 2048), SD_G), 256, lds, st>>>(dout, ldd, W, ldw, ws, Bn, N, K);
  skinny_dgrad_finish_kernel<<<cdiv((long)Bn * K, 256), 256, 0, st>>>(ws, dx, lddx, Bn, K, accumulate);
  MGX_CHECK_LAUNCH();
  return MGX_OK;
}

extern "C" int mgx_ew_bf16(const uint16_t* a, const uint16_t* b, uint16_t* y, long n, int op, void* stream) {
  MGX_REQUIRE(a && y && n > 0 && op >= 0 && op <= 3, "bad argument");
  MGX_REQUIRE(op == 0 || op == 3 || b, "binary op needs b");
  int nb = cdiv(n, 256);
  if (nb > 2048) nb = 2048;
  ew_kernel<<<nb, 256, 0, (hipStream_t)stream>>>(a, b, y, n, op);
  MGX_CHECK_LAUNCH();
  return MGX_OK;
}

extern "C" int mgx_sincos_embed(const float* t, uint16_t* out, int Bn, void* stream) {
  MGX_REQUIRE(t && out && Bn > 0, "bad argument");
  sincos_embed_kernel<<<Bn, 128, 0, (hipStream_t)stream>>>(t, out, Bn);
  MGX_CHECK_LAUNCH();
  return MGX_OK;
}

extern "C" int mgx_cast_f32_bf16(const float* x, uint16_t* y, long n, void* stream) {
  MGX_REQUIRE(x && y && n > 0 && n % 4 == 0, "bad argument");
  int nb = cdiv(n, 1024);
  if (nb > 4096) nb = 4096;
  cast_f32_bf16_kernel<<<nb, 256, 0, (hipStream_t)stream>>>(x, y, n);
  MGX_CHECK_LAUNCH();
  return MGX_OK;
}

extern "C" int mgx_cast_bf16_f32(const uint16_t* x, float* y, long n, float scale, void* stream) {
  MGX_REQUIRE(x && y && n > 0 && n % 8 == 0, "bad argument");
  MGX_REQUIRE(((uintptr_t)x % 16 == 0) && ((uintptr_t)y % 16 == 0), "operands must be 16-byte aligned");
  int nb = cdiv(n, 2048);
  if (nb > 4096) nb = 4096;
  cast_bf16_f32_kernel<<<nb, 256, 0, (hipStream_t)stream>>>(x, y, n, scale);
  MGX_CHECK_LAUNCH();
  return MGX_OK;
}

extern "C" long mgx_gate_bwd_workspace(long batches, long rows_per_batch, int D) {
  return batches * ((rows_per_batch + GR_ROWS - 1) / GR_ROWS) * D;
}

extern "C" int mgx_gate_bwd(const uint16_t* dout, long ldd, long d_bstride, const uint16_t* y, long ldy,
                            const uint16_t* gate, long gate_ld, uint16_t* dy, long lddy, uint16_t* dgate, float* ws,
                            int batches, long rows_per_batch, int D, void* stream) {
  MGX_REQUIRE(dout && y && gate && dy && dgate && ws, "null operand");
  MGX_REQUIRE(D % 2 == 0 && batches > 0 && rows_per_batch > 0, "bad sizes");
  const int bpb = cdiv(rows_per_batch, GR_ROWS);
  hipStream_t st = (hipStream_t)stream;
  gate_bwd_kernel<<<dim3(cdiv(D, 512), batches * bpb), 256, 0, st>>>(dout, ldd, rows_per_batch, d_bstride, y, ldy, gate,
                                                                      gate_ld, dy, lddy, ws, rows_per_batch, D, bpb);
  gate_bwd_finish_kernel<<<dim3(cdiv(D, 64), batches), 256, 0, st>>>(ws, dgate, gate_ld, D, bpb);
  MGX_CHECK_LAUNCH();
  return MGX_OK;
}
```

### mixgrpo_amd/flux.py

```python
import json
import math
import os
from dataclasses import asdict, dataclass
from typing import Dict, List, Tuple

import torch

from . import ops
from ._lib import MgxError
from .ops import BF16, F32, Rows, EPI_BIAS, EPI_BIAS_GELU, EPI_BIAS_GATE_RES


@dataclass
class FluxConfig:
    patch_size: int = 1
    in_channels: int = 64
    num_layers: int = 19
    num_single_layers: int = 38
    attention_head_dim: int = 128
    num_attention_heads: int = 24
    joint_attention_dim: int = 4096
    pooled_projection_dim: int = 768
    guidance_embeds: bool = True
    axes_dims_rope: Tuple[int, int, int] = (16, 56, 56)
# ... 327 lines not shown
        hit = self._rope_cache.get("k")
        if hit is not None and hit[0] == key:
            return hit[1], hit[2]
        ids = torch.cat([txt_ids.float(), img_ids.float()], dim=0)
        cos, sin = rope_tables(ids, self.cfg.axes_dims_rope)
        self._rope_cache["k"] = (key, cos, sin, txt_ids, img_ids)
        return cos, sin

    def _rope_pairs(self, cos, sin):
        if not ops.ROPE_PAIR_TABLE:
            return None
        hit = self._rope_cache.get("pairs")
        if hit is None or hit[0] is not cos:
            hit = (cos, ops.rope_pair_table(cos, sin))
            self._rope_cache["pairs"] = hit
        return hit[1]

    def _temb(self, B, timestep, guidance, pooled, keep=None):
        d = self.cfg.dim
        dev = self.store.device
        t = (timestep.to(BF16) * 1000).float().contiguous()
        gd = guidance.to(dev)
        gd = (gd.to(BF16) * 1000).float()
        gd = gd.expand(B).contiguous() if gd.numel() == 1 else gd.contiguous()

        def mlp(name, x, K):
            h1 = torch.empty(B, d, dtype=BF16, device=dev)
            ops.skinny_linear(x, self.W(f"time_text_embed.{name}.linear_1.weight"),
                              self.W(f"time_text_embed.{name}.linear_1.bias"), h1, d, K)
            a1 = torch.empty_like(h1)
            ops.ew(h1, None, a1, 0)
            h2 = torch.empty_like(h1)
            ops.skinny_linear(a1, self.W(f"time_text_embed.{name}.linear_2.weight"),
                              self.W(f"time_text_embed.{name}.linear_2.bias"), h2, d, d)
            if keep is not None:
                keep[name] = (x, h1, a1)
            return h2

        te = torch.empty(B, 256, dtype=BF16, device=dev)
        ops.sincos_embed(t, te)
        temb = mlp("timestep_embedder", te, 256)
        if self.cfg.guidance_embeds:
            ge = torch.empty(B, 256, dtype=BF16, device=dev)
            ops.sincos_embed(gd, ge)
            gemb = mlp("guidance_embedder", ge, 256)
            t2 = torch.empty_like(temb)
            ops.ew(temb, gemb, t2, 2)
            temb = t2
        pe = mlp("text_embedder", pooled.to(BF16).contiguous(), self.cfg.pooled_projection_dim)
        t3 = torch.empty_like(temb)
        ops.ew(temb, pe, t3, 2)
        st = torch.empty_like(t3)
        ops.ew(t3, None, st, 0)
        return t3, st

    def _stream_rows(self, t, w, which, width):
        if which == "txt":
            return Rows(t, w.B * w.L, width, w.L, w.S * width)
        return Rows(t[0, w.L:], w.B * w.N, width, w.N, w.S * width)

    def _double_block(self, i, w, st, cos, sin, save=None, mods_in=None, keep=None, replay=False, x_in=None):
        cfg, d, H = self.cfg, self.cfg.dim, self.cfg.num_attention_heads
        p = f"transformer_blocks.{i}"
        B = w.B
        dev = self.store.device
        mods = {}
        streams = (("txt", "norm1_context", ("add_q_proj", "add_k_proj", "add_v_proj"), "norm_added_q", "norm_added_k",
                    "to_add_out", "ff_context", w.L, 0),
                   ("img", "norm1", ("to_q", "to_k", "to_v"), "norm_q", "norm_k", "to_out.0", "ff", w.N, w.L))
        row0 = {"txt": 0, "img": w.B * w.L}
        sl = {n: slice(row0[n], row0[n] + B * r) for n, r in (("txt", w.L), ("img", w.N))}
        W16, fused = self.W, self.store.fused
        qkv_kept = keep is not None and "qkv" in keep
        qkv_buf = keep["qkv"] if qkv_kept else w.qkv
        nrm1 = w.nrm if save is None else save["nrm1"]
        for name, norm, qkvn, nq, nk, outn, ffn, rows, s0 in streams:
            if mods_in is not None:
                m = mods_in[name]
            else:
                m = torch.empty(B, 6 * d, dtype=BF16, device=dev)
                ops.skinny_linear(st, W16(f"{p}.{norm}.linear.weight"), W16(f"{p}.{norm}.linear.bias"), m, 6 * d, d)
            mods[name] = m
            Xs = self._stream_rows(w.X if x_in is None else x_in, w, name, d)
            ops.ln_modulate(Xs, m[:, 0:d], m[:, d:2 * d], 6 * d, nrm1[sl[name]], d)
        nograd = save is None and keep is None
        if nograd:
            for name, _, qkvn, nq, nk, _, _, rows, s0 in streams:
                self._qkv_nograd(nrm1[sl[name]], f"{p}.attn.{qkvn[0]}", qkv_buf[sl[name]], w, rows, s0,
                                 self.W32(f"{p}.attn.{nq}.weight"), self.W32(f"{p}.attn.{nk}.weight"), cos, sin)
        elif not (replay and qkv_kept):
            ops.gemm_pair(*(x for name, _, qkvn, *_ in streams for x in (
                Rows.of(nrm1[sl[name]]), fused(self.store.w16, f"{p}.attn.{qkvn[0]}.weight", 3 * d),
                fused(self.store.w16, f"{p}.attn.{qkvn[0]}.bias", 3 * d), Rows.of(qkv_buf[sl[name]]))), 3 * d, d)
        for name, norm, qkvn, nq, nk, outn, ffn, rows, s0 in (() if nograd else streams):
            ops.qk_norm_rope(qkv_buf[sl[name]], self.W32(f"{p}.attn.{nq}.weight"), self.W32(f"{p}.attn.{nk}.weight"), cos, sin,
                             w.Q, w.K, w.Vt, B, H, w.S, w.Sp, rows, s0, q_scale=self.q_scale(),
                             **({} if save is None else dict(V=save["V"], Qt=save["Qt"], Kt=save["Kt"])))
        O_buf = keep["O"] if keep is not None else w.O
        if not replay:
            self._attn(w, O_buf, keep["lse"] if keep is not None else (w.lse if save is not None else None), d, w.S * d)
        aux1 = aux2 = hpre = None
        if keep is not None and not replay:
            aux1, aux2 = keep["y_attn"], keep["y_ff"]
        elif save is not None:
            aux1, aux2 = save["y_attn"], save["y_ff"]
        ff_kept = keep is not None and "hid_pre" in keep
        if save is not None:
            hpre = save["hid_pre"]
        elif ff_kept:
            hpre = keep["hid_pre"]
        part = lambda t, name: None if t is None else t[sl[name]]
        if not replay:
            ops.gemm_pair(*(x for name, _, _, _, _, outn, *_ in streams for x in (
                self._stream_rows(O_buf, w, name, d), W16(f"{p}.attn.{outn}.weight"), W16(f"{p}.attn.{outn}.bias"),
                self._stream_rows(w.X, w, name, d))), d, d, EPI_BIAS_GATE_RES, gate1=mods["txt"][:, 2 * d:3 * d],
                gate2=mods["img"][:, 2 * d:3 * d], gate_ld=6 * d, aux1=part(aux1, "txt"), aux2=part(aux1, "img"))
            xm = keep["x_mid"] if keep is not None else (save["x_mid"] if save is not None else None)
            if xm is not None:
                xm.copy_(w.X)
        x_mid = keep["x_mid"] if replay else w.X
        nrm2 = w.nrm if save is None else save["nrm2"]
        for name in ("txt", "img"):
            m = mods[name]
            ops.ln_modulate(self._stream_rows(x_mid, w, name, d), m[:, 3 * d:4 * d], m[:, 4 * d:5 * d], 6 * d, nrm2[sl[name]], d)
        if replay and ff_kept:
            pass
        else:
            ops.gemm_pair(*(x for name, _, _, _, _, _, ffn, *_ in streams for x in (
                Rows.of(nrm2[sl[name]]), W16(f"{p}.{ffn}.net.0.proj.weight"), W16(f"{p}.{ffn}.net.0.proj.bias"),
                Rows.of(w.hid[sl[name]]))), 4 * d, d, EPI_BIAS_GELU, aux1=part(hpre, "txt"), aux2=part(hpre, "img"))
        if not replay:
            ops.gemm_pair(*(x for name, _, _, _, _, _, ffn, *_ in streams for x in (
                Rows.of(w.hid[sl[name]]), W16(f"{p}.{ffn}.net.2.weight"), W16(f"{p}.{ffn}.net.2.bias"),
                self._stream_rows(w.X, w, name, d))), d, 4 * d, EPI_BIAS_GATE_RES, gate1=mods["txt"][:, 5 * d:6 * d],
                gate2=mods["img"][:, 5 * d:6 * d], gate_ld=6 * d, aux1=part(aux2, "txt"), aux2=part(aux2, "img"))
        return mods

    def _single_block(self, i, w, st, cos, sin, save=None, mod_in=None, keep=None, replay=False, x_in=None):
        cfg, d, H = self.cfg, self.cfg.dim, self.cfg.num_attention_heads
        p = f"single_transformer_blocks.{i}"
        B, S = w.B, w.S
        M = B * S
        if mod_in is not None:
            m = mod_in
        else:
            m = torch.empty(B, 3 * d, dtype=BF16, device=self.store.device)
            ops.skinny_linear(st, self.W(f"{p}.norm.linear.weight"), self.W(f"{p}.norm.linear.bias"), m, 3 * d, d)
        Xa = Rows(w.X if x_in is None else x_in, M, d, S, S * d)
        nrm = w.nrm if save is None else save["nrm1"]
        ops.ln_modulate(Xa, m[:, 0:d], m[:, d:2 * d], 3 * d, nrm, d)
        qkv_kept = keep is not None and "qkv" in keep
        qkv = keep["qkv"] if qkv_kept else w.qkv
        nograd = save is None and keep is None
        if nograd:
            self._qkv_nograd(nrm, f"{p}.attn.to_q", qkv, w, S, 0, self.W32(f"{p}.attn.norm_q.weight"),
                             self.W32(f"{p}.attn.norm_k.weight"), cos, sin)
        elif not (replay and qkv_kept):
            ops.gemm(Rows.of(nrm), self.store.fused(self.store.w16, f"{p}.attn.to_q.weight", 3 * d),
                     self.store.fused(self.store.w16, f"{p}.attn.to_q.bias", 3 * d), Rows.of(qkv), 3 * d, d)
        cat2 = w.cat.view(M, 5 * d)
        ff_kept = keep is not None and "hid_pre" in keep
        if replay and ff_kept:
            pass
        else:
            ops.gemm(Rows.of(nrm), self.W(f"{p}.proj_mlp.weight"), self.W(f"{p}.proj_mlp.bias"),
                     Rows(cat2[0, d:], M, 5 * d), 4 * d, d, EPI_BIAS_GELU,
                     aux=save["hid_pre"] if save is not None else (keep["hid_pre"] if ff_kept else None))
        if not nograd:
            ops.qk_norm_rope(qkv, self.W32(f"{p}.attn.norm_q.weight"), self.W32(f"{p}.attn.norm_k.weight"), cos, sin,
                             w.Q, w.K, w.Vt, B, H, S, w.Sp, S, 0, q_scale=self.q_scale(),
                             **({} if save is None else dict(V=save["V"], Qt=save["Qt"], Kt=save["Kt"])))
        if replay:
            if not ff_kept:
                w.cat[:, :, :d].copy_(keep["O"])
            return m
        self._attn(w, w.cat, keep["lse"] if keep is not None else (w.lse if save is not None else None), 5 * d, S * 5 * d)
        if keep is not None:
            keep["O"].copy_(w.cat[:, :, :d])
        aux = keep["y_attn"] if keep is not None else (None if save is None else save["y_attn"])
        ops.gemm(Rows.of(cat2), self.W(f"{p}.proj_out.weight"), self.W(f"{p}.proj_out.bias"), Xa, d, 5 * d,
                 EPI_BIAS_GATE_RES, gate=m[:, 2 * d:3 * d], gate_ld=3 * d, aux=aux)
        return m

    def _embed(self, w, hidden_states, encoder_hidden_states):
        d = self.cfg.dim
        B, N, L = w.B, w.N, w.L
        hs = hidden_states.detach()
        if hs.dtype == BF16:
            w.in16.copy_(hs.reshape(B * N, -1))
        else:
            ops.cast_bf16(hs.to(F32).contiguous().view(-1), w.in16.view(-1))
        ops.gemm(Rows.of(w.in16), self.W("x_embedder.weight"), self.W("x_embedder.bias"),
                 self._stream_rows(w.X, w, "img", d), d, self.cfg.in_channels)
        ehs = encoder_hidden_states.detach().to(BF16).contiguous()
        ops.gemm(Rows.of(ehs.view(B * L, -1)), self.W("context_embedder.weight"), self.W("context_embedder.bias"),
                 self._stream_rows(w.X, w, "txt", d), d, self.cfg.joint_attention_dim)
        return ehs

    def _head(self, w, st):
        d = self.cfg.dim
        B, N = w.B, w.N
        e = torch.empty(B, 2 * d, dtype=BF16, device=self.store.device)
        ops.skinny_linear(st, self.W("norm_out.linear.weight"), self.W("norm_out.linear.bias"), e, 2 * d, d)
        nrm = w.nrm[:B * N]
        ops.ln_modulate(self._stream_rows(w.X, w, "img", d), e[:, d:2 * d], e[:, 0:d], 2 * d, nrm, d)
        cout = self.cfg.patch_size * self.cfg.patch_size * self.cfg.in_channels
        out = torch.empty(B, N, cout, dtype=BF16, device=self.store.device)
        ops.gemm(Rows.of(nrm), self.W("proj_out.weight"), self.W("proj_out.bias"), Rows.of(out.view(B * N, cout)), cout, d)
        return out, e

    def forward(self, hidden_states, encoder_hidden_states, timestep, guidance, txt_ids, pooled_projections, img_ids,
                joint_attention_kwargs=None, return_dict=False):
        if torch.is_grad_enabled() and self.training and self.flat_param.requires_grad:
            from .flux_backward import FluxFunction
            out = FluxFunction.apply(self.flat_param, self, hidden_states, encoder_hidden_states, timestep, guidance,
                                     txt_ids, pooled_projections, img_ids)
            return (out,)
        with torch.no_grad():
            out = self._forward_nograd(hidden_states, encoder_hidden_states, timestep, guidance, txt_ids,
                                       pooled_projections, img_ids)
        return (out,)

    def _forward_nograd(self, hidden_states, encoder_hidden_states, timestep, guidance, txt_ids, pooled_projections,
                        img_ids, collect=None):
        B, N, _ = hidden_states.shape
        L = encoder_hidden_states.shape[1]
        w = self._workspace(B, L, N)
        self._embed(w, hidden_states, encoder_hidden_states)
        temb, st = self._temb(B, timestep.to(self.store.device), guidance, pooled_projections)
        cos, sin = self._rope(txt_ids, img_ids)
        if collect is not None:
            collect.update(temb=temb.clone(), x_embed=w.X[:, L:].clone(), ctx_embed=w.X[:, :L].clone())
        for i in range(self.cfg.num_layers):
            self._double_block(i, w, st, cos, sin)
            if collect is not None:
# ... 41 lines not shown
```

### mixgrpo_amd/flux_backward.py

```python
import math

import torch

from . import ops
from .ops import BF16, F32, Rows, EPI_BIAS, EPI_BIAS_GATE_RES, EPI_DGELU, EPI_F32_ACC


import os

KEEP_ACTS = os.environ.get("MGX_KEEP_ACTS", "1") != "0"
KEEP_FF = os.environ.get("MGX_KEEP_FF_BLOCKS", "auto")
KEEP_FF_RESERVE_GIB = float(os.environ.get("MGX_KEEP_FF_RESERVE_GIB", "12"))
KEEP_QKV = os.environ.get("MGX_KEEP_QKV_BLOCKS", "auto")


def _pad64(n):
    return (n + 63) // 64 * 64


class _Train:

    def __init__(self, cfg, w, device):
        d, H, hd = cfg.dim, cfg.num_attention_heads, cfg.attention_head_dim
        B, S, Sp = w.B, w.S, w.Sp
        self.B, self.S = B, S
        M = B * S
        e = lambda *shape, dtype=BF16: torch.empty(*shape, dtype=dtype, device=device)
        z = lambda *shape, dtype=BF16: torch.zeros(*shape, dtype=dtype, device=device)
        nblk = cfg.num_layers + cfg.num_single_layers
        self.block_in = e(nblk, B, S, d)
        self.x_final = e(B, S, d)
        self.keep = None
        if KEEP_ACTS:
            self.keep = []
            for b in range(nblk):
                k = dict(O=e(B, S, d), lse=e(B, H, S, dtype=F32), y_attn=e(M, d))
                if b < cfg.num_layers:
                    k.update(y_ff=e(M, d), x_mid=e(B, S, d))
                self.keep.append(k)
            self._ff_shape, self._ff_device = (M, 4 * d), device
            self._qkv_shape = (M, 3 * d)
            if KEEP_FF != "auto":
                self.grow_ff(int(KEEP_FF))
            if KEEP_QKV != "auto":
                self.grow_qkv(int(KEEP_QKV))
        self.save = dict(nrm1=e(M, d), nrm2=e(M, d), y_attn=e(M, d), y_ff=e(M, d), hid_pre=e(M, 4 * d),
                         x_mid=e(B, S, d), V=e(B, H, S, hd), Qt=z(B, H, hd, Sp), Kt=z(B, H, hd, Sp))
        self.dX = e(B, S, d)
        self.dO = e(B, S, 5 * d)
        self.dQ, self.dK, self.dV = e(B, H, S, hd), e(B, H, S, hd), e(B, H, S, hd)
        self.dOt = z(B, H, hd, Sp)
        self.delta = e(B, H, S, dtype=F32)
        self.dy = e(M, d)
        self.dbig = e(M, 7 * d)
        self.dnrm = e(M, d)
        Mp = _pad64(M)
        self.dCt = e(7 * d * Mp)
        self.At = e(5 * d * Mp)
        self.Wt = e(7 * d * max(d, 64) + 5 * d * d)
        self.ones = torch.ones(1, 5 * d, dtype=BF16, device=device)

    def view(self, B):
        return self if B == self.B else _TrainView(self, B)

    def ff_block_bytes(self):
        return self._ff_shape[0] * self._ff_shape[1] * 2

    def ff_kept(self):
        return sum(1 for k in (self.keep or []) if "hid_pre" in k)

    def qkv_block_bytes(self):
        return self._qkv_shape[0] * self._qkv_shape[1] * 2

    def qkv_kept(self):
        return sum(1 for k in (self.keep or []) if "qkv" in k)

    def grow_ff(self, n_total):
        if self.keep is None:
            return 0
        for k in self.keep[:max(0, n_total)]:
            if "hid_pre" not in k:
                k["hid_pre"] = torch.empty(*self._ff_shape, dtype=BF16, device=self._ff_device)
        return self.ff_kept()

    def grow_qkv(self, n_total):
        if self.keep is None:
            return 0
        for k in self.keep[:max(0, n_total)]:
            if "qkv" not in k:
                k["qkv"] = torch.empty(*self._qkv_shape, dtype=BF16, device=self._ff_device)
        return self.qkv_kept()

    def grow_auto(self, budget_bytes):
        if self.keep is None:
            return budget_bytes
        for i, k in enumerate(self.keep):
            for name, auto, size, grow in (("hid_pre", KEEP_FF == "auto", self.ff_block_bytes(), self.grow_ff),
                                           ("qkv", KEEP_QKV == "auto", self.qkv_block_bytes(), self.grow_qkv)):
                if name in k or not auto:
                    continue
                if budget_bytes < size:
                    return budget_bytes
                k[name] = torch.empty(*(self._ff_shape if name == "hid_pre" else self._qkv_shape), dtype=BF16,
                                      device=self._ff_device)
                budget_bytes -= size
        return budget_bytes


class _TrainView:

    def __init__(self, base, B):
        assert B <= base.B
        M = B * base.S
        self.B, self.S = B, base.S
        self.block_in = [base.block_in[i, :B] for i in range(base.block_in.shape[0])]
        self.x_final = base.x_final[:B]
        rows = ("nrm1", "nrm2", "y_attn", "y_ff", "hid_pre")
        self.save = {k: (v[:M] if k in rows else v[:B]) for k, v in base.save.items()}
        self.keep = None
        if base.keep is not None:
            self.keep = [{k: (v[:M] if k in ("y_attn", "y_ff", "hid_pre", "qkv") else v[:B]) for k, v in kb.items()}
                         for kb in base.keep]
        self.dX, self.dO, self.dQ, self.dK, self.dV, self.dOt, self.delta = (
            t[:B] for t in (base.dX, base.dO, base.dQ, base.dK, base.dV, base.dOt, base.delta))
        self.dy, self.dbig, self.dnrm = base.dy[:M], base.dbig[:M], base.dnrm[:M]
        self.dCt, self.At, self.Wt, self.ones = base.dCt, base.At, base.Wt, base.ones


def _train_buffers(cfg, w, device):
    base = w.train
    if base is None or base.B < w.B:
        w.train = None
        del base
        torch.cuda.empty_cache()
        base = _Train(cfg, w, device)
        w.train = base
    return base.view(w.B)


class FluxFunction(torch.autograd.Function):
    @staticmethod
    def forward(ctx, flat_param, model, hidden_states, encoder_hidden_states, timestep, guidance, txt_ids,
                pooled_projections, img_ids):
        cfg = model.cfg
        B, N, _ = hidden_states.shape
        L = encoder_hidden_states.shape[1]
        w = model._workspace(B, L, N)
        tr = _train_buffers(cfg, w, model.store.device)
        ehs = model._embed(w, hidden_states, encoder_hidden_states)
        keep = {}
        temb, st = model._temb(B, timestep.to(model.store.device), guidance, pooled_projections, keep=keep)
        cos, sin = model._rope(txt_ids, img_ids)
        mods = []
        blk = 0
        for i in range(cfg.num_layers):
            tr.block_in[blk].copy_(w.X)
            mods.append(model._double_block(i, w, st, cos, sin, keep=tr.keep[blk] if tr.keep else None))
            blk += 1
        for i in range(cfg.num_single_layers):
            tr.block_in[blk].copy_(w.X)
            mods.append(model._single_block(i, w, st, cos, sin, keep=tr.keep[blk] if tr.keep else None))
            blk += 1
        tr.x_final.copy_(w.X)
        out, e = model._head(w, st)
        w.train.generation = getattr(w.train, "generation", 0) + 1
        ctx.generation = w.train.generation
        ctx.model, ctx.w, ctx.tr = model, w, tr
        ctx.saved = dict(ehs=ehs, in16=w.in16.clone(), temb=temb, st=st, keep=keep, cos=cos, sin=sin, mods=mods, e=e)
        return out

    @staticmethod
    def backward(ctx, dout):
        if getattr(ctx.w.train, "generation", None) != ctx.generation:
            from ._lib import MgxError
            raise MgxError("FluxTransformer2DModel: the activations of this forward pass were overwritten by a later "
                           "grad-enabled forward of the same model (one pending backward per model; call backward() "
                           "before the next training forward)")
        _backward(ctx.model, ctx.w, ctx.tr, ctx.saved, dout.contiguous().to(BF16))
        return (None,) * 9


def _wgrad(model, tr, A, K, dC: Rows, N, wname, bname, rows=None):
    st = model.store
    g = st.ensure_grad()
    parts = A if isinstance(A, list) else [(A, K, False)]
    M = parts[0][0].M
    Mp = _pad64(M)
    dCt = tr.dCt[:N * Mp].view(N, Mp)
    At = tr.At[:K * Mp].view(K, Mp)
    gb = None
    if bname is not None:
        gb = st.fused(g, bname, N) if rows else st.view(g, bname)
    ops.transpose(dC, N, dCt, Mp, colsum_out=gb, colsum_beta=1.0)
    k0 = 0
    for a_rows, width, gelu in parts:
        ops.transpose(a_rows, width, At[k0:k0 + width], Mp, gelu=gelu)
        k0 += width
    assert k0 == K
    gw = st.fused(g, wname, N) if rows else st.view(g, wname)
    ops.gemm(Rows.of(dCt), At, None, Rows(gw, N, K), K, Mp, EPI_F32_ACC, beta=1.0, ldw=Mp)


def _dgrad(model, tr, dC: Rows, N, K, wname, out: Rows, rows=None, epi=EPI_BIAS, aux=None, ldaux=None, row_lo=0,
           row_hi=None, gate=None):
    st = model.store
    W = st.fused(st.w16, wname, N) if rows else st.view(st.w16, wname)
    Wt = tr.Wt[:K * N].view(K, N)
    ops.transpose(Rows.of(W), K, Wt, N)
    row_hi = K if row_hi is None else row_hi
    ops.gemm(dC, Wt[row_lo:row_hi], None, out, row_hi - row_lo, N, epi, aux=aux, ldaux=ldaux, gate=gate, gate_ld=0)


def _dgrad_pair(model, tr, dC1: Rows, wname1, out1: Rows, dC2: Rows, wname2, out2: Rows, N, K, rows=None, epi=EPI_BIAS, aux1=None,
                aux2=None, ldaux=None):
    st = model.store
    Wts = []
    for j, wname in enumerate((wname1, wname2)):
        W = st.fused(st.w16, wname, N) if rows else st.view(st.w16, wname)
        Wt = tr.Wt[j * K * N:(j + 1) * K * N].view(K, N)
        ops.transpose(Rows.of(W), K, Wt, N)
        Wts.append(Wt)
    ops.gemm_pair(dC1, Wts[0], None, out1, dC2, Wts[1], None, out2, K, N, epi, aux1=aux1, aux2=aux2, ldaux=ldaux)


def _skinny_bwd(model, tr, dmod, x, wname, bname, N, K, dx_acc):
    st = model.store
    g = st.ensure_grad()
    ops.skinny_wgrad(dmod, x, st.view(g, wname), st.view(g, bname), N, K)
    if dx_acc is not None:
        ops.skinny_dgrad(dmod, st.view(st.w16, wname), dx_acc, N, K)


def _backward(model, w, tr, sv, dout):
    cfg = model.cfg
    d, H = cfg.dim, cfg.num_attention_heads
    B, L, N, S, Sp = w.B, w.L, w.N, w.S, w.Sp
    M = B * S
    dev = model.store.device
    st_, cos, sin = sv["st"], sv["cos"], sv["sin"]
    scale, q_scale = model.attn_scale(), model.q_scale()
    store = model.store
    g32 = store.ensure_grad()
    dst = torch.zeros(B, d, dtype=BF16, device=dev)
    save0 = tr.save
    save = save0
    row0 = {"txt": 0, "img": B * L}

    def srows(t, which, width):
        return model._stream_rows(t, w, which, width)

    cout = cfg.patch_size * cfg.patch_size * cfg.in_channels
    e = sv["e"]
    nrm = save["nrm1"][:B * N]
    ops.ln_modulate(srows(tr.x_final, "img", d), e[:, d:2 * d], e[:, 0:d], 2 * d, nrm, d)
    dC = Rows.of(dout.view(B * N, cout))
    _wgrad(model, tr, Rows.of(nrm), d, dC, cout, "proj_out.weight", "proj_out.bias")
    dn = tr.dnrm[:B * N]
    _dgrad(model, tr, dC, cout, d, "proj_out.weight", Rows.of(dn))
    tr.dX.zero_()
    de = torch.zeros(B, 2 * d, dtype=BF16, device=dev)
    ops.ln_modulate_bwd(dn, srows(tr.x_final, "img", d), e[:, 0:d], 2 * d, srows(tr.dX, "img", d), False,
                        de[:, d:2 * d], de[:, 0:d], d)
    _skinny_bwd(model, tr, de, st_, "norm_out.linear.weight", "norm_out.linear.bias", 2 * d, d, dst)

    grad_ready = getattr(model, "_grad_ready", None) or (lambda prefix: None)
    grad_ready("tail")
    nblk = cfg.num_layers + cfg.num_single_layers
    for i in reversed(range(cfg.num_single_layers)):
        blk = cfg.num_layers + i
        p = f"single_transformer_blocks.{i}"
        m = sv["mods"][blk]
        kept = tr.keep[blk] if tr.keep else None
        save = dict(save0, y_attn=kept["y_attn"]) if kept else save0
        if kept and "hid_pre" in kept:
            save["hid_pre"] = kept["hid_pre"]
        if kept is None:
            w.X.copy_(tr.block_in[blk])
        model._single_block(i, w, st_, cos, sin, save=save, mod_in=m, keep=kept, replay=kept is not None,
                            x_in=tr.block_in[blk] if kept is not None else None)
        lse_b = kept["lse"] if kept is not None else w.lse
        dmod = torch.empty(B, 3 * d, dtype=BF16, device=dev)
        x_in = Rows(tr.block_in[blk], M, d, S, S * d)
        dXr = Rows(tr.dX, M, d, S, S * d)
        cat2 = w.cat.view(M, 5 * d)
        lean = kept is not None and "hid_pre" in kept
        ops.gate_bwd(dXr, save["y_attn"], m[:, 2 * d:3 * d], 3 * d, tr.dy, dmod[:, 2 * d:3 * d], B, S, d)
        dyr = Rows.of(tr.dy)
        a_op = [(Rows.of(kept["O"].view(M, d)), d, False), (Rows.of(kept["hid_pre"]), 4 * d, True)] if lean else Rows.of(cat2)
        _wgrad(model, tr, a_op, 5 * d, dyr, d, f"{p}.proj_out.weight", f"{p}.proj_out.bias")
        dcat = tr.dO.view(M, 5 * d)
        dO1 = tr.dO.view(-1)[:M * d].view(B, S, d)
        dbig = tr.dbig
        stW = store.view(store.w16, f"{p}.proj_out.weight")
        Wt = tr.Wt[:5 * d * d].view(5 * d, d)
        ops.transpose(Rows.of(stW), 5 * d, Wt, d)
        ops.gemm(dyr, Wt[0:d], None, Rows.of(dO1.view(M, d)) if lean else Rows(dcat, M, 5 * d), d, d, EPI_BIAS)
        ops.gemm(dyr, Wt[d:5 * d], None, Rows(dbig[0, 3 * d:], M, 7 * d), 4 * d, d, EPI_DGELU, aux=save["hid_pre"],
                 ldaux=4 * d)
        if lean:
            ops.attn_bwd(w.Q, w.K, save["V"], save["Qt"], save["Kt"], kept["O"], dO1, lse_b, tr.delta, tr.dOt, tr.dQ, tr.dK,
                         tr.dV, B, H, S, Sp, d, S * d, scale)
        else:
            ops.attn_bwd(w.Q, w.K, save["V"], save["Qt"], save["Kt"], w.cat, tr.dO, lse_b, tr.delta, tr.dOt, tr.dQ, tr.dK,
                         tr.dV, B, H, S, Sp, 5 * d, S * 5 * d, scale)
        qkv_b = kept["qkv"] if kept is not None and "qkv" in kept else w.qkv
        ops.qk_norm_rope_bwd(qkv_b, model.W32(f"{p}.attn.norm_q.weight"), model.W32(f"{p}.attn.norm_k.weight"), cos, sin,
                             tr.dQ, tr.dK, tr.dV, dbig, store.view(g32, f"{p}.attn.norm_q.weight"),
                             store.view(g32, f"{p}.attn.norm_k.weight"), B, H, S, Sp, S, 0, ld_dqkv=7 * d, q_scale=q_scale)
        dbr = Rows.of(dbig)
        _wgrad(model, tr, Rows.of(save["nrm1"]), d, dbr, 7 * d, f"{p}.attn.to_q.weight", f"{p}.attn.to_q.bias", rows=True)
        _dgrad(model, tr, dbr, 7 * d, d, f"{p}.attn.to_q.weight", Rows.of(tr.dnrm), rows=True)
        ops.ln_modulate_bwd(tr.dnrm, x_in, m[:, d:2 * d], 3 * d, dXr, True, dmod[:, 0:d], dmod[:, d:2 * d], d)
        _skinny_bwd(model, tr, dmod, st_, f"{p}.norm.linear.weight", f"{p}.norm.linear.bias", 3 * d, d, dst)
        grad_ready(p)

    streams = (("txt", "norm1_context", ("add_q_proj", "add_k_proj", "add_v_proj"), "norm_added_q", "norm_added_k",
                "to_add_out", "ff_context", L, 0),
               ("img", "norm1", ("to_q", "to_k", "to_v"), "norm_q", "norm_k", "to_out.0", "ff", N, L))
    sl = {"txt": slice(0, B * L), "img": slice(B * L, B * S)}
    dO3 = tr.dO.view(-1)[:B * S * d].view(B, S, d)
    dh_all = tr.dbig.view(-1)[:M * 4 * d].view(M, 4 * d)
    dqkv_all = tr.dbig.view(-1)[:M * 3 * d].view(M, 3 * d)
    for i in reversed(range(cfg.num_layers)):
        p = f"transformer_blocks.{i}"
        mods = sv["mods"][i]
        kept = tr.keep[i] if tr.keep else None
        save = dict(save0, y_attn=kept["y_attn"], y_ff=kept["y_ff"], x_mid=kept["x_mid"]) if kept else save0
        if kept and "hid_pre" in kept:
            save["hid_pre"] = kept["hid_pre"]
        if kept is None:
            w.X.copy_(tr.block_in[i])
        model._double_block(i, w, st_, cos, sin, save=save, mods_in=mods, keep=kept, replay=kept is not None,
                            x_in=tr.block_in[i] if kept is not None else None)
        O_b, lse_b = (kept["O"], kept["lse"]) if kept is not None else (w.O, w.lse)
        dmods = {k: torch.empty(B, 6 * d, dtype=BF16, device=dev) for k in ("img", "txt")}
        for name, norm, qkvn, nq, nk, outn, ffn, rows, s0 in streams:
            m, dm = mods[name], dmods[name]
            ops.gate_bwd(srows(tr.dX, name, d), save["y_ff"][sl[name]], m[:, 5 * d:6 * d], 6 * d, tr.dy[sl[name]],
                         dm[:, 5 * d:6 * d], B, rows, d)
            a_op = [(Rows.of(kept["hid_pre"][sl[name]]), 4 * d, True)] if kept is not None and "hid_pre" in kept \
                else Rows.of(w.hid[sl[name]])
            _wgrad(model, tr, a_op, 4 * d, Rows.of(tr.dy[sl[name]]), d, f"{p}.{ffn}.net.2.weight", f"{p}.{ffn}.net.2.bias")
        _dgrad_pair(model, tr, Rows.of(tr.dy[sl["txt"]]), f"{p}.ff_context.net.2.weight", Rows.of(dh_all[sl["txt"]]),
                    Rows.of(tr.dy[sl["img"]]), f"{p}.ff.net.2.weight", Rows.of(dh_all[sl["img"]]), d, 4 * d, epi=EPI_DGELU,
                    aux1=save["hid_pre"][sl["txt"]], aux2=save["hid_pre"][sl["img"]], ldaux=4 * d)
        for name, norm, qkvn, nq, nk, outn, ffn, rows, s0 in streams:
            _wgrad(model, tr, Rows.of(save["nrm2"][sl[name]]), d, Rows.of(dh_all[sl[name]]), 4 * d, f"{p}.{ffn}.net.0.proj.weight",
                   f"{p}.{ffn}.net.0.proj.bias")
        _dgrad_pair(model, tr, Rows.of(dh_all[sl["txt"]]), f"{p}.ff_context.net.0.proj.weight", Rows.of(tr.dnrm[sl["txt"]]),
                    Rows.of(dh_all[sl["img"]]), f"{p}.ff.net.0.proj.weight", Rows.of(tr.dnrm[sl["img"]]), 4 * d, d)
        for name, norm, qkvn, nq, nk, outn, ffn, rows, s0 in streams:
            m, dm = mods[name], dmods[name]
            dXs = srows(tr.dX, name, d)
            ops.ln_modulate_bwd(tr.dnrm[sl[name]], srows(save["x_mid"], name, d), m[:, 4 * d:5 * d], 6 * d, dXs, True,
                                dm[:, 3 * d:4 * d], dm[:, 4 * d:5 * d], d)
            ops.gate_bwd(dXs, save["y_attn"][sl[name]], m[:, 2 * d:3 * d], 6 * d, tr.dy[sl[name]], dm[:, 2 * d:3 * d], B, rows, d)
            _wgrad(model, tr, srows(O_b, name, d), d, Rows.of(tr.dy[sl[name]]), d, f"{p}.attn.{outn}.weight",
                   f"{p}.attn.{outn}.bias")
        _dgrad_pair(model, tr, Rows.of(tr.dy[sl["txt"]]), f"{p}.attn.to_add_out.weight", srows(dO3, "txt", d),
                    Rows.of(tr.dy[sl["img"]]), f"{p}.attn.to_out.0.weight", srows(dO3, "img", d), d, d)
        ops.attn_bwd(w.Q, w.K, save["V"], save["Qt"], save["Kt"], O_b, dO3, lse_b, tr.delta, tr.dOt, tr.dQ, tr.dK, tr.dV,
                     B, H, S, Sp, d, S * d, scale)
        qkv_b = kept["qkv"] if kept is not None and "qkv" in kept else w.qkv
        for name, norm, qkvn, nq, nk, outn, ffn, rows, s0 in streams:
            ops.qk_norm_rope_bwd(qkv_b[sl[name]], model.W32(f"{p}.attn.{nq}.weight"), model.W32(f"{p}.attn.{nk}.weight"), cos,
                                 sin, tr.dQ, tr.dK, tr.dV, dqkv_all[sl[name]], store.view(g32, f"{p}.attn.{nq}.weight"),
                                 store.view(g32, f"{p}.attn.{nk}.weight"), B, H, S, Sp, rows, s0, q_scale=q_scale)
            _wgrad(model, tr, Rows.of(save["nrm1"][sl[name]]), d, Rows.of(dqkv_all[sl[name]]), 3 * d, f"{p}.attn.{qkvn[0]}.weight",
                   f"{p}.attn.{qkvn[0]}.bias", rows=True)
        _dgrad_pair(model, tr, Rows.of(dqkv_all[sl["txt"]]), f"{p}.attn.add_q_proj.weight", Rows.of(tr.dnrm[sl["txt"]]),
                    Rows.of(dqkv_all[sl["img"]]), f"{p}.attn.to_q.weight", Rows.of(tr.dnrm[sl["img"]]), 3 * d, d, rows=True)
        for name, norm, qkvn, nq, nk, outn, ffn, rows, s0 in streams:
            m, dm = mods[name], dmods[name]
            ops.ln_modulate_bwd(tr.dnrm[sl[name]], srows(tr.block_in[i], name, d), m[:, d:2 * d], 6 * d, srows(tr.dX, name, d),
                                True, dm[:, 0:d], dm[:, d:2 * d], d)
            _skinny_bwd(model, tr, dm, st_, f"{p}.{norm}.linear.weight", f"{p}.{norm}.linear.bias", 6 * d, d, dst)
        grad_ready(p)

    _wgrad(model, tr, Rows.of(sv["in16"]), cfg.in_channels, srows(tr.dX, "img", d), d, "x_embedder.weight",
           "x_embedder.bias")
    _wgrad(model, tr, Rows.of(sv["ehs"].view(B * L, -1)), cfg.joint_attention_dim, srows(tr.dX, "txt", d), d,
           "context_embedder.weight", "context_embedder.bias")

    dtemb = torch.empty(B, d, dtype=BF16, device=dev)
    ops.ew(sv["temb"], dst, dtemb, 1)
    for name, (x, h1, a1) in sv["keep"].items():
        K = x.shape[1]
        da1 = torch.zeros(B, d, dtype=BF16, device=dev)
        _skinny_bwd(model, tr, dtemb, a1, f"time_text_embed.{name}.linear_2.weight",
                    f"time_text_embed.{name}.linear_2.bias", d, d, da1)
        dh1 = torch.empty(B, d, dtype=BF16, device=dev)
        ops.ew(h1, da1, dh1, 1)
        _skinny_bwd(model, tr, dh1, x, f"time_text_embed.{name}.linear_1.weight",
                    f"time_text_embed.{name}.linear_1.bias", d, K, None)
    if model.flat_param.grad is None:
        model.flat_param.grad = g32
```

### mixgrpo_amd/ops.py

```python
import os
from dataclasses import dataclass

import torch

from ._lib import check, lib, ptr, stream

EPI_BIAS, EPI_BIAS_GELU, EPI_BIAS_GATE_RES, EPI_F32_ACC, EPI_DGELU = 0, 1, 2, 3, 4
BF16 = torch.bfloat16
F32 = torch.float32


@dataclass
class Rows:
    t: torch.Tensor
    M: int
    ld: int
    rpb: int = 1 << 40
    bstride: int = 0

    @staticmethod
    def of(t):
        cols = t.shape[-1]
        return Rows(t, t.numel() // cols, cols)

# ... 24 lines not shown
        e0, e1 = torch.cuda.Event(enable_timing=True), torch.cuda.Event(enable_timing=True)
        e0.record()
    rc = lib().mgx_linear_bf16_t(ptr(X), ptr(W), ptr(bias), Ct.data_ptr(), tokens, F, K, K, K, ld_ct, tok_rpb, ct_bstride,
                                 None if ws is None else ws.data_ptr(), 0 if ws is None else ws.numel(), stream())
    if rc == 1:
        return False
    check(rc)
    if prof:
        e1.record()
        GEMM_PROFILE.append((e0, e1, 2.0 * tokens * F * K, (F, tokens, K, EPI_BIAS)))
    return True


def _gemm_launch(A, W, bias, C, N, K, epi, gate, gate_ld, aux, beta, ldw, ldaux):
    ws = _sk_workspace(C.t.device) if GEMM_STREAM_K else None
    check(lib().mgx_gemm_bf16_sk(ptr(A.t), ptr(W), ptr(bias), ptr(C.t), None if gate is None else gate.data_ptr(),
                                 None if aux is None else aux.data_ptr(), (N if ldaux is None else ldaux), A.M, N, K, A.ld,
                                 A.rpb, A.bstride, K if ldw is None else ldw, C.ld, C.rpb, C.bstride, gate_ld, epi, beta,
                                 None if ws is None else ws.data_ptr(), 0 if ws is None else ws.numel(), stream()))


def gemm_pair(A1: Rows, W1, bias1, C1: Rows, A2: Rows, W2, bias2, C2: Rows, N, K, epi=EPI_BIAS, gate1=None, gate2=None, gate_ld=0,
              aux1=None, aux2=None, ldaux=None):
    assert A1.M == C1.M and A2.M == C2.M and A1.ld == A2.ld and C1.ld == C2.ld
    if not GEMM_PAIR:
        gemm(A1, W1, bias1, C1, N, K, epi, gate=gate1, gate_ld=gate_ld, aux=aux1, ldaux=ldaux)
        gemm(A2, W2, bias2, C2, N, K, epi, gate=gate2, gate_ld=gate_ld, aux=aux2, ldaux=ldaux)
        return
    prof = GEMM_PROFILE
    if prof is not None:
        e0, e1 = torch.cuda.Event(enable_timing=True), torch.cuda.Event(enable_timing=True)
        e0.record()
    ws = _sk_workspace(C1.t.device) if GEMM_STREAM_K else None
    dp = lambda t: None if t is None else t.data_ptr()
    check(lib().mgx_gemm_bf16_pair(ptr(A1.t), ptr(W1), ptr(bias1), ptr(C1.t), dp(gate1), dp(aux1), A1.M, A1.rpb, A1.bstride, C1.rpb,
                                   C1.bstride, ptr(A2.t), ptr(W2), ptr(bias2), ptr(C2.t), dp(gate2), dp(aux2), A2.M, A2.rpb,
                                   A2.bstride, C2.rpb, C2.bstride, N, K, A1.ld, K, C1.ld, (N if ldaux is None else ldaux), gate_ld,
                                   epi, 0.0, dp(ws), 0 if ws is None else ws.numel(), stream()))
    if prof is not None:
        e1.record()
        prof.append((e0, e1, 2.0 * (A1.M + A2.M) * N * K, (A1.M + A2.M, N, K, epi)))


GEMM_PAIR = os.environ.get("MGX_GEMM_PAIR", "0") == "1"


GEMM_STREAM_K = os.environ.get("MGX_GEMM_STREAM_K", "1") != "0"
_sk_ws = {}


def _sk_workspace(device):
    key = (device, torch.cuda.current_stream().cuda_stream)
    w = _sk_ws.get(key)
    if w is None:
        w = torch.empty(lib().mgx_gemm_sk_workspace_elems(), dtype=F32, device=device)
        _sk_ws[key] = w
    return w


_scratch = {}


def scratch(name, numel, dtype, device):
    key = (name, dtype, device)
    t = _scratch.get(key)
    if t is None or t.numel() < numel:
        t = torch.empty(int(numel), dtype=dtype, device=device)
        _scratch[key] = t
    return t[:numel]


def transpose(inp: Rows, N, out, ld_out, colsum_out=None, colsum_beta=1.0, gelu=False):
    if gelu:
        assert colsum_out is None and inp.rpb >= inp.M
        check(lib().mgx_transpose_gelu_bf16(ptr(inp.t), ptr(out), inp.M, N, inp.ld, ld_out, stream()))
        return
    part = None
    if colsum_out is not None:
        part = scratch("colsum_partial", lib().mgx_transpose_partial_elems(inp.M, N), F32, out.device)
    check(lib().mgx_transpose_bf16(ptr(inp.t), ptr(out), ptr(part), ptr(colsum_out), colsum_beta, inp.M, N, inp.ld,
                                   inp.rpb, inp.bstride, ld_out, stream()))


def ln_modulate(x: Rows, shift, scale, mod_ld, y, D, stats=None):
    check(lib().mgx_ln_modulate_fwd(ptr(x.t), x.ld, x.rpb, x.bstride, shift.data_ptr(), scale.data_ptr(), mod_ld, ptr(y),
                                    D, ptr(stats), x.M, D, stream()))


def ln_modulate_bwd(dy, x: Rows, scale, mod_ld, dx: Rows, accumulate, dshift, dscale, D):
    ws = scratch("ln_bwd", lib().mgx_ln_modulate_bwd_workspace(x.M, min(x.rpb, x.M), D), F32, dy.device)
    check(lib().mgx_ln_modulate_bwd(ptr(dy), D, ptr(x.t), x.ld, min(x.rpb, x.M), x.bstride, scale.data_ptr(), mod_ld,
                                    ptr(dx.t), dx.ld, min(dx.rpb, dx.M), dx.bstride, int(accumulate), dshift.data_ptr(),
                                    dscale.data_ptr(), ptr(ws), x.M, D, stream()))


LN2, LOG2E = 0.6931471805599453, 1.4426950408889634
Q_PRESCALE = os.environ.get("MGX_ATTN_Q_PRESCALE", "1") != "0"


def qk_norm_rope(qkv, wq, wk, cos, sin, Q, K, Vt, B, H, S, Sp, rows_per_batch, s0, V=None, Qt=None, Kt=None, q_scale=1.0):
    check(lib().mgx_qk_norm_rope_fwd_qs(ptr(qkv), qkv.shape[-1], ptr(wq), ptr(wk), ptr(cos), ptr(sin), ptr(Q), ptr(K),
                                        ptr(Vt), ptr(V), ptr(Qt), ptr(Kt), B, H, S, Sp, rows_per_batch, s0, float(q_scale),
                                        stream()))


def qk_norm_rope_bwd(qkv, wq, wk, cos, sin, dQ, dK, dV, dqkv, gwq, gwk, B, H, S, Sp, rows_per_batch, s0, ld_dqkv=None,
                     q_scale=1.0):
    ws = scratch("qk_bwd", lib().mgx_qk_norm_rope_bwd_workspace(B, H, rows_per_batch), F32, qkv.device)
    check(lib().mgx_qk_norm_rope_bwd_qs(ptr(qkv), qkv.shape[-1], ptr(wq), ptr(wk), ptr(cos), ptr(sin), ptr(dQ), ptr(dK),
                                        ptr(dV), dqkv.data_ptr(), qkv.shape[-1] if ld_dqkv is None else ld_dqkv, ptr(gwq),
                                        ptr(gwk), ptr(ws), B, H, S, Sp, rows_per_batch, s0, float(q_scale), stream()))


def linear_qk_norm_rope(X, Wqk, bias, wq, wk, cos, sin, Q, K, B, H, S, rows_per_batch, s0, Kdim, q_scale=1.0, pairs=None):
    prof = GEMM_PROFILE is not None
    if prof:
        e0, e1 = torch.cuda.Event(enable_timing=True), torch.cuda.Event(enable_timing=True)
        e0.record()
    rc = lib().mgx_linear_qk_norm_rope(ptr(X), ptr(Wqk), ptr(bias), ptr(wq), ptr(wk), ptr(cos), ptr(sin), ptr(pairs), ptr(Q), ptr(K),
                                       B, H, S, rows_per_batch, s0, Kdim, Kdim, Kdim, float(q_scale), stream())
    if rc == 1:
        return False
    check(rc)
    if prof:
        e1.record()
        GEMM_PROFILE.append((e0, e1, 2.0 * B * rows_per_batch * 2 * H * 128 * Kdim, (B * rows_per_batch, 2 * H * 128, Kdim, 5)))
    return True


def rope_pair_table(cos, sin):
    if not (torch.equal(cos[:, 0::2], cos[:, 1::2]) and torch.equal(sin[:, 0::2], sin[:, 1::2])):
        return None
    return torch.stack([cos[:, 0::2], sin[:, 0::2]], dim=-1).contiguous()


def attn_fwd(Q, K, Vt, O_ptr_tensor, lse, B, H, S, Sp, ldo, o_bstride, scale):
    check(lib().mgx_attn_fwd(ptr(Q), ptr(K), ptr(Vt), O_ptr_tensor.data_ptr(), ptr(lse), B, H, S, Sp, ldo, o_bstride,
                             scale, stream()))


def attn_fwd_log2(Q2, K, Vt, O_ptr_tensor, lse, B, H, S, Sp, ldo, o_bstride):
    check(lib().mgx_attn_fwd_log2(ptr(Q2), ptr(K), ptr(Vt), O_ptr_tensor.data_ptr(), ptr(lse), B, H, S, Sp, ldo, o_bstride,
                                  stream()))


def attn_fwd_path(B, H, S, Sp, ldo, o_bstride):
    r = lib().mgx_attn_fwd_path(B, H, S, Sp, ldo, o_bstride)
    check(min(r, 0))
    return r


def attn_bwd_path(B, H, S, Sp, ldo, o_bstride):
    r = lib().mgx_attn_bwd_path(B, H, S, Sp, ldo, o_bstride)
    check(min(r, 0))
    return r


def attn_fp8_quantize(Q, K, Vt, Q8, K8, V8t, amax, B, H, S, Sp):
    check(lib().mgx_attn_fp8_quantize(ptr(Q), ptr(K), ptr(Vt), ptr(Q8), ptr(K8), ptr(V8t), ptr(amax), B, H, S, Sp,
                                      stream()))


def attn_fwd_fp8(Q8, K8, V8t, amax, O_ptr_tensor, lse, B, H, S, Sp, ldo, o_bstride, scale):
    check(lib().mgx_attn_fwd_fp8(ptr(Q8), ptr(K8), ptr(V8t), ptr(amax), O_ptr_tensor.data_ptr(), ptr(lse), B, H, S, Sp,
                                 ldo, o_bstride, scale, stream()))


def skinny_linear(x, W, bias, out, N, K):
    Bn = x.shape[0]
    for b0 in range(0, Bn, 16):
        nb = min(16, Bn - b0)
        check(lib().mgx_skinny_linear(x[b0:].data_ptr(), x.stride(0), ptr(W), K, ptr(bias), out[b0:].data_ptr(),
                                      out.stride(0), nb, N, K, stream()))


def skinny_wgrad(dout, x, dW, dbias, N, K):
    Bn = x.shape[0]
    for b0 in range(0, Bn, 16):
        nb = min(16, Bn - b0)
        check(lib().mgx_skinny_wgrad(dout[b0:].data_ptr(), dout.stride(0), x[b0:].data_ptr(), x.stride(0), ptr(dW), K,
                                     ptr(dbias), nb, N, K, stream()))


def skinny_dgrad(dout, W, dx, N, K, accumulate=True):
    Bn = dout.shape[0]
    for b0 in range(0, Bn, 8):
        nb = min(8, Bn - b0)
        ws = scratch("skinny_dgrad", lib().mgx_skinny_dgrad_workspace(nb, K), F32, dout.device)
        check(lib().mgx_skinny_dgrad(dout[b0:].data_ptr(), dout.stride(0), ptr(W), K, dx[b0:].data_ptr(), dx.stride(0),
                                     ptr(ws), nb, N, K, 1 if accumulate else 0, stream()))


def ew(a, b, y, op):
    check(lib().mgx_ew_bf16(ptr(a), ptr(b), ptr(y), a.numel(), op, stream()))


def sincos_embed(t, out):
    check(lib().mgx_sincos_embed(ptr(t), ptr(out), t.numel(), stream()))


def cast_bf16(x, y):
    check(lib().mgx_cast_f32_bf16(ptr(x), ptr(y), x.numel(), stream()))


def gelu_rows(x, ldx, y, ldy, M, N):
    check(lib().mgx_gelu_bf16(ptr(x), ldx, ptr(y), ldy, M, N, stream()))


def cast_f32(x, y, scale=1.0):
    check(lib().mgx_cast_bf16_f32(ptr(x), ptr(y), x.numel(), float(scale), stream()))


def gate_bwd(dout: Rows, y, gate, gate_ld, dy, dgate, batches, rows_per_batch, D):
    ws = scratch("gate_bwd", lib().mgx_gate_bwd_workspace(batches, rows_per_batch, D), F32, y.device)
    check(lib().mgx_gate_bwd(ptr(dout.t), dout.ld, dout.bstride, ptr(y), D, gate.data_ptr(), gate_ld, ptr(dy), D,
                             dgate.data_ptr(), ptr(ws), batches, rows_per_batch, D, stream()))


def sqnorm(g, out, beta=0.0):
    ws = scratch("sqnorm", lib().mgx_sqnorm_workspace(), torch.float64, g.device)
    check(lib().mgx_sqnorm_f32(ptr(g), g.numel(), ptr(ws), ptr(out), beta, stream()))


def adamw_step(w, w16, g, m, v, lr, beta1, beta2, eps, wd, step, gnorm_sq, max_norm, grad_scale=1.0):
    check(lib().mgx_adamw_step(ptr(w), ptr(w16), ptr(g), ptr(m), ptr(v), w.numel(), lr, beta1, beta2, eps, wd, step,
                               ptr(gnorm_sq), max_norm, grad_scale, stream()))


def attn_bwd(Q, K, V, Qt, Kt, O, dO, lse, delta, dOt, dQ, dK, dV, B, H, S, Sp, ldo, o_bstride, scale):
    check(lib().mgx_attn_bwd(ptr(Q), ptr(K), ptr(V), ptr(Qt), ptr(Kt), O.data_ptr(), dO.data_ptr(), ptr(lse), ptr(delta),
                             ptr(dOt), ptr(dQ), ptr(dK), ptr(dV), B, H, S, Sp, ldo, o_bstride, scale, stream()))


def conv3x3(xpad, Wt, bias, out, H, W, C, Cout, ones=None, ld_out=None):
    check(lib().mgx_conv3x3_nhwc(ptr(xpad), ptr(Wt), ptr(bias), ptr(out), Cout if ld_out is None else ld_out, ptr(ones), H, W, C,
                                 Cout, 0 if ones is None else 1, stream()))


def group_norm(x, gamma, beta, out, H, W, C, G, silu, padded, eps=1e-6):
    ws = scratch("group_norm", lib().mgx_group_norm_workspace(H * W, C, G), F32, x.device)
    if padded:
        o, out_row = out.view(-1)[(W + 2) * C + C:], (W + 2) * C
    else:
        o, out_row = out, W * C
    check(lib().mgx_group_norm_nhwc(ptr(x), C, ptr(gamma), ptr(beta), o.data_ptr(), out_row, C, ptr(ws), H, W, C, G, eps,
                                    1 if silu else 0, stream()))


def upsample2x_pad(x, outpad, H, W, C):
    check(lib().mgx_upsample2x_pad_nhwc(ptr(x), outpad.view(-1)[(2 * W + 2) * C + C:].data_ptr(), H, W, C, stream()))


def latents_to_pad(z, outpad, Cin, H, W, C):
    check(lib().mgx_latents_to_pad_nhwc(ptr(z), outpad.view(-1)[(W + 2) * C + C:].data_ptr(), Cin, H, W, C, stream()))


def nhwc_to_image(x, ld, img, Cout, H, W):
    check(lib().mgx_nhwc_to_image(ptr(x), ld, ptr(img), Cout, H, W, stream()))


def softmax_rows(S, P, M, n, scale):
    check(lib().mgx_softmax_rows_f32(ptr(S), S.stride(0), ptr(P), P.stride(0), M, n, scale, stream()))
```

Baseline: 0.4383.

## Fuse transposed wgrad operands into LN-modulate, gate-bwd and QK-norm-rope-bwd kernels

```diff
diff --git a/include/mixgrpo_hip.h b/include/mixgrpo_hip.h
--- a/include/mixgrpo_hip.h
+++ b/include/mixgrpo_hip.h
@@ -117,6 +117,9 @@
 int mgx_ln_modulate_fwd(const uint16_t* x, long ldx, long x_rpb, long x_bstride, const uint16_t* shift,
                         const uint16_t* scale, long mod_ld, uint16_t* y, long ldy, float* stats, long M, int D,
                         void* stream);
+int mgx_ln_modulate_fwd_t(const uint16_t* x, long ldx, long x_rpb, long x_bstride, const uint16_t* shift,
+                          const uint16_t* scale, long mod_ld, uint16_t* out, long ld_out, float* stats, int stats_ready,
+                          long M, int D, void* stream);
 long mgx_ln_modulate_bwd_workspace(long M, long rpb, int D);
 int mgx_ln_modulate_bwd(const uint16_t* dy, long lddy, const uint16_t* x, long ldx, long x_rpb, long x_bstride,
                         const uint16_t* scale, long mod_ld, uint16_t* dx, long lddx, long dx_rpb, long dx_bstride,
@@ -139,6 +142,10 @@
                             const float* sin, const uint16_t* dQ, const uint16_t* dK, const uint16_t* dV, uint16_t* dqkv,
                             long ld_dqkv, float* gwq, float* gwk, float* ws, int B, int H, int S, int Sp,
                             int rows_per_batch, int s0, float q_scale, void* stream);
+int mgx_qk_norm_rope_bwd_t(const uint16_t* qkv, long ld, const float* wq, const float* wk, const float* cos, const float* sin,
+                           const uint16_t* dQ, const uint16_t* dK, const uint16_t* dV, uint16_t* dqkv, long ld_dqkv,
+                           float* gwq, float* gwk, float* ws, uint16_t* dct, long ldt, float* colsum_partial, int B, int H,
+                           int S, int Sp, int rows_per_batch, int s0, float q_scale, void* stream);
 
 int mgx_attn_fwd(const uint16_t* Q, const uint16_t* K, const uint16_t* Vt, uint16_t* O, float* lse, int B, int H, int S,
                  int Sp, long ldo, long o_bstride, float scale, void* stream);
@@ -176,6 +183,10 @@
 int mgx_gate_bwd(const uint16_t* dout, long ldd, long d_bstride, const uint16_t* y, long ldy, const uint16_t* gate,
                  long gate_ld, uint16_t* dy, long lddy, uint16_t* dgate, float* ws, int batches, long rows_per_batch,
                  int D, void* stream);
+int mgx_gate_bwd_t(const uint16_t* dout, long ldd, long d_bstride, const uint16_t* y, long ldy, const uint16_t* gate,
+                   long gate_ld, uint16_t* dy, long lddy, uint16_t* dgate, float* ws, uint16_t* dyt, long ldt,
+                   float* colsum_partial, int batches, long rows_per_batch, int D, void* stream);
+int mgx_colsum_finish(const float* colsum_partial, float* colsum_out, float colsum_beta, int nblk, int N, void* stream);
 
 long mgx_sqnorm_workspace(void);
 int mgx_sqnorm_f32(const float* g, long n, double* ws, float* out, float beta, void* stream);
diff --git a/mixgrpo_amd/_lib.py b/mixgrpo_amd/_lib.py
--- a/mixgrpo_amd/_lib.py
+++ b/mixgrpo_amd/_lib.py
@@ -58,6 +58,7 @@
     "mgx_transpose_partial_elems": (_L, [_I, _I]),
     "mgx_transpose_bf16": (_I, [_P, _P, _P, _P, _F, _I, _I, _L, _L, _L, _L, _P]),
     "mgx_ln_modulate_fwd": (_I, [_P, _L, _L, _L, _P, _P, _L, _P, _L, _P, _L, _I, _P]),
+    "mgx_ln_modulate_fwd_t": (_I, [_P, _L, _L, _L, _P, _P, _L, _P, _L, _P, _I, _L, _I, _P]),
     "mgx_ln_modulate_bwd_workspace": (_L, [_L, _L, _I]),
     "mgx_ln_modulate_bwd": (_I, [_P, _L, _P, _L, _L, _L, _P, _L, _P, _L, _L, _L, _I, _P, _P, _P, _L, _I, _P]),
     "mgx_qk_norm_rope_fwd": (_I, [_P, _L] + [_P] * 10 + [_I] * 6 + [_P]),
@@ -65,6 +66,7 @@
     "mgx_qk_norm_rope_bwd_workspace": (_L, [_I, _I, _I]),
     "mgx_qk_norm_rope_bwd": (_I, [_P, _L] + [_P] * 8 + [_L] + [_P] * 3 + [_I] * 6 + [_P]),
     "mgx_qk_norm_rope_bwd_qs": (_I, [_P, _L] + [_P] * 8 + [_L] + [_P] * 3 + [_I] * 6 + [_F, _P]),
+    "mgx_qk_norm_rope_bwd_t": (_I, [_P, _L] + [_P] * 8 + [_L] + [_P] * 4 + [_L, _P] + [_I] * 6 + [_F, _P]),
     "mgx_attn_fwd": (_I, [_P] * 5 + [_I] * 4 + [_L, _L, _F, _P]),
     "mgx_attn_fwd_log2": (_I, [_P] * 5 + [_I] * 4 + [_L, _L, _P]),
     "mgx_attn_fwd_path": (_I, [_I] * 4 + [_L, _L]),
@@ -91,6 +93,8 @@
     "mgx_transpose_gelu_bf16": (_I, [_P, _P, _I, _I, _L, _L, _P]),
     "mgx_gate_bwd_workspace": (_L, [_L, _L, _I]),
     "mgx_gate_bwd": (_I, [_P, _L, _L, _P, _L, _P, _L, _P, _L, _P, _P, _I, _L, _I, _P]),
+    "mgx_gate_bwd_t": (_I, [_P, _L, _L, _P, _L, _P, _L, _P, _L, _P, _P, _P, _L, _P, _I, _L, _I, _P]),
+    "mgx_colsum_finish": (_I, [_P, _P, _F, _I, _I, _P]),
     "mgx_sqnorm_workspace": (_L, []),
     "mgx_sqnorm_f32": (_I, [_P, _L, _P, _P, _F, _P]),
     "mgx_adamw_step": (_I, [_P, _P, _P, _P, _P, _L, _D, _D, _D, _D, _D, _I, _P, _F, _F, _P]),
diff --git a/mixgrpo_amd/csrc/gemm.hip b/mixgrpo_amd/csrc/gemm.hip
--- a/mixgrpo_amd/csrc/gemm.hip
+++ b/mixgrpo_amd/csrc/gemm.hip
@@ -1,5 +1,6 @@
 #include "../../include/mixgrpo_hip.h"
 #include "common.h"
+#include "transpose8.h"
 
 #include <cmath>
 #include <cstdlib>
@@ -318,8 +319,6 @@
   }
 }
 
-__device__ __forceinline__ uint32_t lo16(uint32_t a, uint32_t b) { return __builtin_amdgcn_perm(b, a, 0x05040100); }
-__device__ __forceinline__ uint32_t hi16(uint32_t a, uint32_t b) { return __builtin_amdgcn_perm(b, a, 0x07060302); }
 template <bool GELU>
 __global__ void __launch_bounds__(256) transpose8_kernel(const bf16_raw* __restrict__ in, bf16_raw* __restrict__ out,
                                                          float* __restrict__ part, int M, int N, RowMap im, long ldo) {
@@ -1412,6 +1411,13 @@
   return MGX_OK;
 }
 
+extern "C" int mgx_colsum_finish(const float* colsum_partial, float* colsum_out, float colsum_beta, int nblk, int N, void* stream) {
+  MGX_REQUIRE(colsum_partial && colsum_out && nblk > 0 && N > 0, "bad argument");
+  colsum_finish_kernel<<<cdiv(N, 64), 256, 0, (hipStream_t)stream>>>(colsum_partial, colsum_out, nblk, N, colsum_beta);
+  MGX_CHECK_LAUNCH();
+  return MGX_OK;
+}
+
 extern "C" int mgx_transpose_gelu_bf16(const uint16_t* in, uint16_t* out, int M, int N, long ld_in, long ld_out, void* stream) {
   MGX_REQUIRE(in && out && M > 0 && N > 0, "bad argument");
   MGX_REQUIRE(ld_out >= M, "output leading dimension must cover M");
diff --git a/mixgrpo_amd/csrc/norm.hip b/mixgrpo_amd/csrc/norm.hip
--- a/mixgrpo_amd/csrc/norm.hip
+++ b/mixgrpo_amd/csrc/norm.hip
@@ -1,5 +1,6 @@
 #include "../../include/mixgrpo_hip.h"
 #include "common.h"
+#include "transpose8.h"
 
 namespace {
 
@@ -26,7 +27,7 @@
   return u;
 }
 
-template <int NV>
+template <int NV, bool STATS_ONLY = false>
 __global__ void __launch_bounds__(256) ln_mod_fwd_kernel(const bf16_raw* __restrict__ x, RowMap xm,
                                                          const bf16_raw* __restrict__ shift,
                                                          const bf16_raw* __restrict__ scale, long mod_ld,
@@ -60,6 +61,7 @@
     stats[2 * m] = mean;
     stats[2 * m + 1] = rstd;
   }
+  if (STATS_ONLY) return;
   const bf16_raw* sh = shift + b * mod_ld;
   const bf16_raw* sc = scale + b * mod_ld;
 #pragma unroll
@@ -72,6 +74,58 @@
     for (int j = 0; j < 8; ++j) o[j] = (v[i][j] - mean) * rstd * rbf(1.0f + fc[j]) + fs[j];
     *reinterpret_cast<uint4*>(y + m * ldy + c) = pack8(o);
   }
+}
+
+__global__ void __launch_bounds__(256) ln_mod_t_kernel(const bf16_raw* __restrict__ x, RowMap xm,
+                                                       const bf16_raw* __restrict__ shift,
+                                                       const bf16_raw* __restrict__ scale, long mod_ld,
+                                                       const float* __restrict__ stats, bf16_raw* __restrict__ out, long ldo,
+                                                       long M, int D) {
+  int tx, ty;
+  t8_map(threadIdx.x, tx, ty);
+  const int n0 = blockIdx.x * 128 + tx * 8;
+  const long m0 = (long)blockIdx.y * 128 + ty * 8;
+  if (n0 >= D || m0 >= ldo) return;
+  uint32_t r[8][4];
+  uint4 xv[8];
+  float2 ms[8];
+#pragma unroll
+  for (int i = 0; i < 8; ++i) {
+    const long m = m0 + i;
+    xv[i] = make_uint4(0, 0, 0, 0);
+    ms[i] = make_float2(0.f, 0.f);
+    if (m < M) {
+      xv[i] = *reinterpret_cast<const uint4*>(x + row_off(xm, m) + n0);
+      ms[i] = *reinterpret_cast<const float2*>(stats + 2 * m);
+    }
+  }
+  long bcur = -1;
+  float fs[8], sc1[8];
+#pragma unroll
+  for (int i = 0; i < 8; ++i) {
+    const long m = m0 + i;
+    if (m < M) {
+      const long b = m / xm.rpb;
+      if (b != bcur) {
+        bcur = b;
+        float fc[8];
+        unpack8(*reinterpret_cast<const uint4*>(shift + b * mod_ld + n0), fs);
+        unpack8(*reinterpret_cast<const uint4*>(scale + b * mod_ld + n0), fc);
+#pragma unroll
+        for (int j = 0; j < 8; ++j) sc1[j] = rbf(1.0f + fc[j]);
+      }
+      float v[8], o[8];
+      unpack8(xv[i], v);
+      const float mean = ms[i].x, rstd = ms[i].y;
+#pragma unroll
+      for (int j = 0; j < 8; ++j) o[j] = (v[j] - mean) * rstd * sc1[j] + fs[j];
+      const uint4 u = pack8(o);
+      r[i][0] = u.x; r[i][1] = u.y; r[i][2] = u.z; r[i][3] = u.w;
+    } else {
+      r[i][0] = r[i][1] = r[i][2] = r[i][3] = 0;
+    }
+  }
+  t8_store(r, out, n0, m0, ldo);
 }
 
 constexpr int LN_BWD_ROWS = 32;
@@ -334,17 +388,32 @@
   float* part;
   int H, S, Sp, rows_per_batch, s0;
   float q_scale;
+  bf16_raw* dct;
+  long ldt;
+  float* cpart;
 };
 
+template <bool EMIT_T>
 __global__ void __launch_bounds__(256) qk_norm_rope_bwd_kernel(QkBwdArgs a) {
   __shared__ float red[4][2][128];
+  __shared__ uint32_t tile[EMIT_T ? 3 : 1][EMIT_T ? 64 : 1][65];
   const int lane = threadIdx.x & 63, w = threadIdx.x >> 6;
   const int hh = blockIdx.y, b = blockIdx.z;
-  const int t0 = blockIdx.x * 64;
   const int HD = 128;
   const long dmodel = (long)a.H * HD;
   const float wq0 = a.wq[2 * lane], wq1 = a.wq[2 * lane + 1];
   const float wk0 = a.wk[2 * lane], wk1 = a.wk[2 * lane + 1];
+  const int gx = EMIT_T ? (a.rows_per_batch + 63) / 64 : (int)gridDim.x;
+  float carry[6][2];
+#pragma unroll
+  for (int it = 0; it < 6; ++it) carry[it][0] = carry[it][1] = 0.f;
+#pragma unroll 1
+  for (int half = 0; half < (EMIT_T ? 2 : 1); ++half) {
+  const int bx = EMIT_T ? blockIdx.x * 2 + half : (int)blockIdx.x;
+  const int t0 = bx * 64;
+  if (EMIT_T && t0 >= a.rows_per_batch) {
+    for (int i = threadIdx.x; i < 3 * 64 * 64; i += 256) tile[i >> 12][(i >> 6) & 63][i & 63] = 0;
+  } else {
   float gq0 = 0.f, gq1 = 0.f, gk0 = 0.f, gk1 = 0.f;
   constexpr int U = 4;
   for (int i0 = 0; i0 < 16; i0 += U) {
@@ -370,7 +439,10 @@
     }
 #pragma unroll
     for (int u = 0; u < U; ++u) {
-      if (!ok[u]) continue;
+      if (!ok[u]) {
+        if (EMIT_T) tile[0][w * 16 + i0 + u][lane] = tile[1][w * 16 + i0 + u][lane] = tile[2][w * 16 + i0 + u][lane] = 0;
+        continue;
+      }
       const int t = t0 + w * 16 + i0 + u;
       const long row = (long)b * a.rows_per_batch + t;
       bf16_raw* obase = a.dqkv + row * a.ldo + hh * HD + 2 * lane;
@@ -389,18 +461,55 @@
         const float dot = wave_sum(gz0 * x0 + gz1 * x1) / 128.f;
         const float dx0 = r * gz0 - x0 * r * r * r * dot;
         const float dx1 = r * gz1 - x1 * r * r * r * dot;
-        *reinterpret_cast<uint32_t*>(obase + which * dmodel) = (uint32_t)f2bf(dx0) | ((uint32_t)f2bf(dx1) << 16);
+        const uint32_t dxu = (uint32_t)f2bf(dx0) | ((uint32_t)f2bf(dx1) << 16);
+        *reinterpret_cast<uint32_t*>(obase + which * dmodel) = dxu;
+        if (EMIT_T) tile[which][w * 16 + i0 + u][lane] = dxu;
       }
       *reinterpret_cast<uint32_t*>(obase + 2 * dmodel) = uv[u];
+      if (EMIT_T) tile[2][w * 16 + i0 + u][lane] = uv[u];
     }
   }
   red[w][0][2 * lane] = gq0; red[w][0][2 * lane + 1] = gq1;
   red[w][1][2 * lane] = gk0; red[w][1][2 * lane + 1] = gk1;
   __syncthreads();
-  const long blk = ((long)blockIdx.z * gridDim.y + blockIdx.y) * gridDim.x + blockIdx.x;
+  const long blk = ((long)blockIdx.z * gridDim.y + blockIdx.y) * gx + bx;
   {
     const int which = threadIdx.x >> 7, c = threadIdx.x & 127;
     a.part[(blk * 2 + which) * 128 + c] = red[0][which][c] + red[1][which][c] + red[2][which][c] + red[3][which][c];
+  }
+  }
+  if (EMIT_T) {
+    __syncthreads();
+    const int tg = lane & 7, cpl = lane >> 3;
+    const long m = (long)b * a.rows_per_batch + t0 + tg * 8;
+#pragma unroll
+    for (int it = 0; it < 6; ++it) {
+      const int item = it * 32 + w * 8 + cpl, which = item >> 6, cp = item & 63;
+      uint32_t r[8];
+#pragma unroll
+      for (int i = 0; i < 8; ++i) r[i] = tile[which][tg * 8 + i][cp];
+      const long n = which * dmodel + hh * HD + 2 * cp;
+      if (m < a.ldt) {
+        *reinterpret_cast<uint4*>(a.dct + n * a.ldt + m) =
+            make_uint4(lo16(r[0], r[1]), lo16(r[2], r[3]), lo16(r[4], r[5]), lo16(r[6], r[7]));
+        *reinterpret_cast<uint4*>(a.dct + (n + 1) * a.ldt + m) =
+            make_uint4(hi16(r[0], r[1]), hi16(r[2], r[3]), hi16(r[4], r[5]), hi16(r[6], r[7]));
+      }
+      float c0 = 0.f, c1 = 0.f;
+#pragma unroll
+      for (int i = 0; i < 8; ++i) { c0 += bf2f(r[i] & 0xffff); c1 += bf2f(r[i] >> 16); }
+#pragma unroll
+      for (int k = 0; k < 8; ++k) {
+        carry[it][0] += __shfl(c0, (lane & ~7) | k, 64);
+        carry[it][1] += __shfl(c1, (lane & ~7) | k, 64);
+      }
+      if (half == 1 && tg == 0) {
+        const long blk128 = ((long)b * a.rows_per_batch + (long)blockIdx.x * 128) >> 7;
+        *reinterpret_cast<float2*>(a.cpart + blk128 * 3 * dmodel + n) = make_float2(carry[it][0], carry[it][1]);
+      }
+    }
+    __syncthreads();
+  }
   }
 }
 
@@ -446,6 +555,30 @@
     CASE(1) CASE(2) CASE(3) CASE(4) CASE(5) CASE(6) CASE(7) CASE(8)
 #undef CASE
   }
+  MGX_CHECK_LAUNCH();
+  return MGX_OK;
+}
+
+extern "C" int mgx_ln_modulate_fwd_t(const uint16_t* x, long ldx, long x_rpb, long x_bstride, const uint16_t* shift,
+                                     const uint16_t* scale, long mod_ld, uint16_t* out, long ld_out, float* stats,
+                                     int stats_ready, long M, int D, void* stream) {
+  MGX_REQUIRE(x && shift && scale && out && stats && M > 0, "bad argument");
+  MGX_REQUIRE(D % 512 == 0 && D <= 4096, "feature size must be a multiple of 512 up to 4096");
+  MGX_REQUIRE(ldx % 8 == 0 && mod_ld % 8 == 0 && x_bstride % 8 == 0, "16-byte row alignment");
+  MGX_REQUIRE(ld_out >= M && ld_out % 8 == 0, "output leading dimension must cover M in 16-byte steps");
+  MGX_REQUIRE(((uintptr_t)x % 16 == 0) && ((uintptr_t)shift % 16 == 0) && ((uintptr_t)scale % 16 == 0) && ((uintptr_t)out % 16 == 0) &&
+              ((uintptr_t)stats % 8 == 0), "operands must be 16-byte aligned");
+  hipStream_t st = (hipStream_t)stream;
+  const RowMap xm{ldx, x_rpb, x_bstride};
+  if (!stats_ready) {
+    const int grid = cdiv(M, 4);
+    switch (D / 512) {
+#define CASE(nv) case nv: ln_mod_fwd_kernel<nv, true><<<grid, 256, 0, st>>>(x, xm, shift, scale, mod_ld, nullptr, 0, stats, M); break;
+      CASE(1) CASE(2) CASE(3) CASE(4) CASE(5) CASE(6) CASE(7) CASE(8)
+#undef CASE
+    }
+  }
+  ln_mod_t_kernel<<<dim3(cdiv(D, 128), cdiv(ld_out, 128)), 256, 0, st>>>(x, xm, shift, scale, mod_ld, stats, out, ld_out, M, D);
   MGX_CHECK_LAUNCH();
   return MGX_OK;
 }
@@ -510,17 +643,30 @@
   return ((long)cdiv(rows_per_batch, 64) * H * B + QK_FIN_G) * 2 * 128;
 }
 
-extern "C" int mgx_qk_norm_rope_bwd_qs(const uint16_t* qkv, long ld, const float* wq, const float* wk, const float* cos,
-                                       const float* sin, const uint16_t* dQ, const uint16_t* dK, const uint16_t* dV,
-                                       uint16_t* dqkv, long ld_dqkv, float* gwq, float* gwk, float* ws, int B, int H, int S,
-                                       int Sp, int rows_per_batch, int s0, float q_scale, void* stream) {
+static int qk_norm_rope_bwd_launch(const uint16_t* qkv, long ld, const float* wq, const float* wk, const float* cos,
+                                   const float* sin, const uint16_t* dQ, const uint16_t* dK, const uint16_t* dV,
+                                   uint16_t* dqkv, long ld_dqkv, float* gwq, float* gwk, float* ws, uint16_t* dct, long ldt,
+                                   float* cpart, int B, int H, int S, int Sp, int rows_per_batch, int s0, float q_scale,
+                                   void* stream) {
   MGX_REQUIRE(qkv && wq && wk && cos && sin && dQ && dK && dV && dqkv && gwq && gwk && ws, "null argument");
   MGX_REQUIRE(ld == 3L * H * 128, "qkv rows must be [q | k | v] of H*128 each");
   MGX_REQUIRE(ld_dqkv >= ld && ld_dqkv % 2 == 0, "dqkv rows must hold [dq | dk | dv] and keep 4-byte alignment");
+  if (dct) {
+    const long M = (long)B * rows_per_batch;
+    MGX_REQUIRE(cpart, "the transposed output comes with its column partial sums");
+    MGX_REQUIRE(rows_per_batch % 8 == 0 && (B == 1 || rows_per_batch % 128 == 0),
+                "the transposing form takes whole 128-row blocks per batch (any multiple of 8 rows for one batch)");
+    MGX_REQUIRE(ldt >= M && ldt % 8 == 0 && ldt <= (long)cdiv(M, 128) * 128 && ((uintptr_t)dct % 16 == 0) && ((uintptr_t)cpart % 8 == 0),
+                "transposed leading dimension must cover M, in 16-byte steps, within its last 128-row block");
+  }
   hipStream_t st = (hipStream_t)stream;
-  QkBwdArgs a{qkv, ld, wq, wk, cos, sin, dQ, dK, dV, dqkv, ld_dqkv, ws, H, S, Sp, rows_per_batch, s0, q_scale};
+  QkBwdArgs a{qkv, ld, wq, wk, cos, sin, dQ, dK, dV, dqkv, ld_dqkv, ws, H, S, Sp, rows_per_batch, s0, q_scale, dct, ldt, cpart};
   dim3 grid(cdiv(rows_per_batch, 64), H, B);
-  qk_norm_rope_bwd_kernel<<<grid, 256, 0, st>>>(a);
+  if (dct) {
+    qk_norm_rope_bwd_kernel<true><<<dim3(cdiv(rows_per_batch, 128), H, B), 256, 0, st>>>(a);
+  } else {
+    qk_norm_rope_bwd_kernel<false><<<grid, 256, 0, st>>>(a);
+  }
   const long nblocks = (long)grid.x * grid.y * grid.z;
   float* mid = ws + nblocks * 256;
   qk_bwd_partial_kernel<<<QK_FIN_G, 256, 0, st>>>(ws, mid, nblocks);
@@ -529,6 +675,24 @@
   return MGX_OK;
 }
 
+extern "C" int mgx_qk_norm_rope_bwd_qs(const uint16_t* qkv, long ld, const float* wq, const float* wk, const float* cos,
+                                       const float* sin, const uint16_t* dQ, const uint16_t* dK, const uint16_t* dV,
+                                       uint16_t* dqkv, long ld_dqkv, float* gwq, float* gwk, float* ws, int B, int H, int S,
+                                       int Sp, int rows_per_batch, int s0, float q_scale, void* stream) {
+  return qk_norm_rope_bwd_launch(qkv, ld, wq, wk, cos, sin, dQ, dK, dV, dqkv, ld_dqkv, gwq, gwk, ws, nullptr, 0, nullptr, B, H, S, Sp,
+                                 rows_per_batch, s0, q_scale, stream);
+}
+
+extern "C" int mgx_qk_norm_rope_bwd_t(const uint16_t* qkv, long ld, const float* wq, const float* wk, const float* cos,
+                                      const float* sin, const uint16_t* dQ, const uint16_t* dK, const uint16_t* dV,
+                                      uint16_t* dqkv, long ld_dqkv, float* gwq, float* gwk, float* ws, uint16_t* dct, long ldt,
+                                      float* colsum_partial, int B, int H, int S, int Sp, int rows_per_batch, int s0,
+                                      float q_scale, void* stream) {
+  MGX_REQUIRE(dct && colsum_partial, "null argument");
+  return qk_norm_rope_bwd_launch(qkv, ld, wq, wk, cos, sin, dQ, dK, dV, dqkv, ld_dqkv, gwq, gwk, ws, dct, ldt, colsum_partial, B, H, S,
+                                 Sp, rows_per_batch, s0, q_scale, stream);
+}
+
 extern "C" int mgx_qk_norm_rope_bwd(const uint16_t* qkv, long ld, const float* wq, const float* wk, const float* cos,
                                     const float* sin, const uint16_t* dQ, const uint16_t* dK, const uint16_t* dV,
                                     uint16_t* dqkv, long ld_dqkv, float* gwq, float* gwk, float* ws, int B, int H, int S,
diff --git a/mixgrpo_amd/csrc/small.hip b/mixgrpo_amd/csrc/small.hip
--- a/mixgrpo_amd/csrc/small.hip
+++ b/mixgrpo_amd/csrc/small.hip
@@ -1,5 +1,6 @@
 #include "../../include/mixgrpo_hip.h"
 #include "common.h"
+#include "transpose8.h"
 
 namespace {
 
@@ -222,6 +223,75 @@
   part[(long)blockIdx.y * D + c + 1] = a1;
 }
 
+__global__ void __launch_bounds__(256) gate_bwd_t_kernel(const bf16_raw* __restrict__ dout, long ldd, long d_bstride,
+                                                         const bf16_raw* __restrict__ y, long ldy,
+                                                         const bf16_raw* __restrict__ gate, long gate_ld,
+                                                         bf16_raw* __restrict__ dy, long lddy, float* __restrict__ part,
+                                                         bf16_raw* __restrict__ dyt, long ldt, float* __restrict__ cpart,
+                                                         long rows_per_batch, long M, int D, int blocks_per_batch) {
+  __shared__ float cs[16][129];
+  int tx, ty;
+  t8_map(threadIdx.x, tx, ty);
+  const int n0 = blockIdx.x * 128 + tx * 8;
+  const long m0 = (long)blockIdx.y * 128 + ty * 8;
+  const bool live = n0 < D && m0 < M;
+  uint32_t r[8][4], du[8][4], yu[8][4];
+#pragma unroll
+  for (int i = 0; i < 8; ++i)
+#pragma unroll
+    for (int k = 0; k < 4; ++k) r[i][k] = du[i][k] = yu[i][k] = 0;
+  long blk = 0;
+  if (live) {
+    const long b = m0 / rows_per_batch, rr = m0 - b * rows_per_batch;
+    blk = b * blocks_per_batch + rr / GR_ROWS;
+    const uint4 gu = *reinterpret_cast<const uint4*>(gate + b * gate_ld + n0);
+    const uint32_t gw[4] = {gu.x, gu.y, gu.z, gu.w};
+#pragma unroll
+    for (int i = 0; i < 8; ++i) {
+      const uint4 d4 = *reinterpret_cast<const uint4*>(dout + b * d_bstride + (rr + i) * ldd + n0);
+      const uint4 y4 = *reinterpret_cast<const uint4*>(y + (m0 + i) * ldy + n0);
+      du[i][0] = d4.x; du[i][1] = d4.y; du[i][2] = d4.z; du[i][3] = d4.w;
+      yu[i][0] = y4.x; yu[i][1] = y4.y; yu[i][2] = y4.z; yu[i][3] = y4.w;
+    }
+#pragma unroll
+    for (int i = 0; i < 8; ++i) {
+#pragma unroll
+      for (int k = 0; k < 4; ++k)
+        r[i][k] = (uint32_t)f2bf(bf2f(gw[k] & 0xffff) * bf2f(du[i][k] & 0xffff)) |
+                  ((uint32_t)f2bf(bf2f(gw[k] >> 16) * bf2f(du[i][k] >> 16)) << 16);
+      *reinterpret_cast<uint4*>(dy + (m0 + i) * lddy + n0) = make_uint4(r[i][0], r[i][1], r[i][2], r[i][3]);
+    }
+  }
+  float a[8];
+#pragma unroll
+  for (int j = 0; j < 8; ++j) a[j] = 0.f;
+  const int tyl = ty & 7;
+#pragma unroll
+  for (int s = 0; s < 8; ++s) {
+    if (s > 0) {
+#pragma unroll
+      for (int j = 0; j < 8; ++j) a[j] = __shfl_up(a[j], 8, 64);
+    }
+    if (live && tyl == s) {
+#pragma unroll
+      for (int i = 0; i < 8; ++i)
+#pragma unroll
+        for (int k = 0; k < 4; ++k) {
+          a[2 * k] = __builtin_fmaf(bf2f(du[i][k] & 0xffff), bf2f(yu[i][k] & 0xffff), a[2 * k]);
+          a[2 * k + 1] = __builtin_fmaf(bf2f(du[i][k] >> 16), bf2f(yu[i][k] >> 16), a[2 * k + 1]);
+        }
+    }
+  }
+  if (live && tyl == 7) {
+    *reinterpret_cast<float4*>(part + blk * D + n0) = make_float4(a[0], a[1], a[2], a[3]);
+    *reinterpret_cast<float4*>(part + blk * D + n0 + 4) = make_float4(a[4], a[5], a[6], a[7]);
+  }
+  if (n0 < D && m0 < ldt) t8_store(r, dyt, n0, m0, ldt);
+  float csum[8];
+  t8_colsum_rows(r, csum);
+  t8_colsum_block(cs, csum, tx, ty, cpart, M, D);
+}
+
 __global__ void __launch_bounds__(256) gate_bwd_finish_kernel(const float* __restrict__ part, bf16_raw* __restrict__ dgate,
                                                               long gate_ld, int D, int blocks_per_batch) {
   __shared__ float red[4][64];
@@ -328,3 +398,24 @@
   MGX_CHECK_LAUNCH();
   return MGX_OK;
 }
+
+extern "C" int mgx_gate_bwd_t(const uint16_t* dout, long ldd, long d_bstride, const uint16_t* y, long ldy,
+                              const uint16_t* gate, long gate_ld, uint16_t* dy, long lddy, uint16_t* dgate, float* ws,
+                              uint16_t* dyt, long ldt, float* colsum_partial, int batches, long rows_per_batch, int D,
+                              void* stream) {
+  MGX_REQUIRE(dout && y && gate && dy && dgate && ws && dyt && colsum_partial, "null operand");
+  MGX_REQUIRE(D % 8 == 0 && batches > 0 && rows_per_batch > 0, "bad sizes");
+  MGX_REQUIRE(rows_per_batch % GR_ROWS == 0, "the transposing form takes whole 64-row blocks per batch");
+  const long M = (long)batches * rows_per_batch;
+  MGX_REQUIRE(ldt >= M && ldt % 8 == 0, "transposed leading dimension must cover M in 16-byte steps");
+  MGX_REQUIRE(ldd % 8 == 0 && d_bstride % 8 == 0 && ldy % 8 == 0 && lddy % 8 == 0 && gate_ld % 8 == 0, "16-byte row alignment");
+  MGX_REQUIRE(((uintptr_t)dout % 16 == 0) && ((uintptr_t)y % 16 == 0) && ((uintptr_t)gate % 16 == 0) && ((uintptr_t)dy % 16 == 0) &&
+              ((uintptr_t)dyt % 16 == 0) && ((uintptr_t)ws % 16 == 0), "operands must be 16-byte aligned");
+  const int bpb = cdiv(rows_per_batch, GR_ROWS);
+  hipStream_t st = (hipStream_t)stream;
+  gate_bwd_t_kernel<<<dim3(cdiv(D, 128), cdiv(ldt, 128)), 256, 0, st>>>(dout, ldd, d_bstride, y, ldy, gate, gate_ld, dy, lddy, ws,
+                                                                        dyt, ldt, colsum_partial, rows_per_batch, M, D, bpb);
+  gate_bwd_finish_kernel<<<dim3(cdiv(D, 64), batches), 256, 0, st>>>(ws, dgate, gate_ld, D, bpb);
+  MGX_CHECK_LAUNCH();
+  return MGX_OK;
+}
diff --git a/mixgrpo_amd/csrc/transpose8.h b/mixgrpo_amd/csrc/transpose8.h
--- /dev/null
+++ b/mixgrpo_amd/csrc/transpose8.h
@@ -0,0 +1,47 @@
+#pragma once
+#include "common.h"
+
+__device__ __forceinline__ uint32_t lo16(uint32_t a, uint32_t b) { return __builtin_amdgcn_perm(b, a, 0x05040100); }
+__device__ __forceinline__ uint32_t hi16(uint32_t a, uint32_t b) { return __builtin_amdgcn_perm(b, a, 0x07060302); }
+
+__device__ __forceinline__ void t8_map(int tid, int& tx, int& ty) {
+  tx = (tid & 7) | (((tid >> 6) & 1) << 3);
+  ty = ((tid >> 3) & 7) | ((tid >> 7) << 3);
+}
+
+__device__ __forceinline__ void t8_store(const uint32_t (&r)[8][4], bf16_raw* __restrict__ out, long n0, long m0, long ldo) {
+#pragma unroll
+  for (int c2 = 0; c2 < 4; ++c2) {
+    uint4 e, o;
+    e.x = lo16(r[0][c2], r[1][c2]); e.y = lo16(r[2][c2], r[3][c2]); e.z = lo16(r[4][c2], r[5][c2]); e.w = lo16(r[6][c2], r[7][c2]);
+    o.x = hi16(r[0][c2], r[1][c2]); o.y = hi16(r[2][c2], r[3][c2]); o.z = hi16(r[4][c2], r[5][c2]); o.w = hi16(r[6][c2], r[7][c2]);
+    *reinterpret_cast<uint4*>(out + (n0 + 2 * c2) * ldo + m0) = e;
+    *reinterpret_cast<uint4*>(out + (n0 + 2 * c2 + 1) * ldo + m0) = o;
+  }
+}
+
+__device__ __forceinline__ void t8_colsum_rows(const uint32_t (&r)[8][4], float (&csum)[8]) {
+#pragma unroll
+  for (int j = 0; j < 8; ++j) csum[j] = 0.f;
+#pragma unroll
+  for (int i = 0; i < 8; ++i)
+#pragma unroll
+    for (int c2 = 0; c2 < 4; ++c2) {
+      csum[2 * c2] += bf2f(r[i][c2] & 0xffff);
+      csum[2 * c2 + 1] += bf2f(r[i][c2] >> 16);
+    }
+}
+
+__device__ __forceinline__ void t8_colsum_block(float (*cs)[129], const float (&csum)[8], int tx, int ty, float* __restrict__ part,
+                                                long M, int N) {
+#pragma unroll
+  for (int j = 0; j < 8; ++j) cs[ty][tx * 8 + j] = csum[j];
+  __syncthreads();
+  if (threadIdx.x < 128) {
+    float t = 0.f;
+#pragma unroll
+    for (int k = 0; k < 16; ++k) t += cs[k][threadIdx.x];
+    const int n = blockIdx.x * 128 + threadIdx.x;
+    if (n < N && (long)blockIdx.y * 128 < M) part[(long)blockIdx.y * N + n] = t;
+  }
+}
diff --git a/mixgrpo_amd/flux.py b/mixgrpo_amd/flux.py
--- a/mixgrpo_amd/flux.py
+++ b/mixgrpo_amd/flux.py
@@ -433,7 +433,10 @@
                 ops.skinny_linear(st, W16(f"{p}.{norm}.linear.weight"), W16(f"{p}.{norm}.linear.bias"), m, 6 * d, d)
             mods[name] = m
             Xs = self._stream_rows(w.X if x_in is None else x_in, w, name, d)
-            ops.ln_modulate(Xs, m[:, 0:d], m[:, d:2 * d], 6 * d, nrm1[sl[name]], d)
+            if replay and qkv_kept:
+                continue
+            ops.ln_modulate(Xs, m[:, 0:d], m[:, d:2 * d], 6 * d, nrm1[sl[name]], d,
+                            stats=keep["st1"][sl[name]] if keep is not None and not replay else None)
         nograd = save is None and keep is None
         if nograd:
             for name, _, qkvn, nq, nk, _, _, rows, s0 in streams:
@@ -472,8 +475,11 @@
         x_mid = keep["x_mid"] if replay else w.X
         nrm2 = w.nrm if save is None else save["nrm2"]
         for name in ("txt", "img"):
+            if replay and ff_kept:
+                break
             m = mods[name]
-            ops.ln_modulate(self._stream_rows(x_mid, w, name, d), m[:, 3 * d:4 * d], m[:, 4 * d:5 * d], 6 * d, nrm2[sl[name]], d)
+            ops.ln_modulate(self._stream_rows(x_mid, w, name, d), m[:, 3 * d:4 * d], m[:, 4 * d:5 * d], 6 * d, nrm2[sl[name]], d,
+                            stats=keep["st2"][sl[name]] if keep is not None and not replay else None)
         if replay and ff_kept:
             pass
         else:
@@ -499,9 +505,11 @@
             ops.skinny_linear(st, self.W(f"{p}.norm.linear.weight"), self.W(f"{p}.norm.linear.bias"), m, 3 * d, d)
         Xa = Rows(w.X if x_in is None else x_in, M, d, S, S * d)
         nrm = w.nrm if save is None else save["nrm1"]
-        ops.ln_modulate(Xa, m[:, 0:d], m[:, d:2 * d], 3 * d, nrm, d)
         qkv_kept = keep is not None and "qkv" in keep
         qkv = keep["qkv"] if qkv_kept else w.qkv
+        if not (replay and qkv_kept and "hid_pre" in keep):
+            ops.ln_modulate(Xa, m[:, 0:d], m[:, d:2 * d], 3 * d, nrm, d,
+                            stats=keep["st1"] if keep is not None and not replay else None)
         nograd = save is None and keep is None
         if nograd:
             self._qkv_nograd(nrm, f"{p}.attn.to_q", qkv, w, S, 0, self.W32(f"{p}.attn.norm_q.weight"),
diff --git a/mixgrpo_amd/flux_backward.py b/mixgrpo_amd/flux_backward.py
--- a/mixgrpo_amd/flux_backward.py
+++ b/mixgrpo_amd/flux_backward.py
@@ -1,4 +1,5 @@
 import math
+from dataclasses import dataclass
 
 import torch
 
@@ -34,9 +35,9 @@
         if KEEP_ACTS:
             self.keep = []
             for b in range(nblk):
-                k = dict(O=e(B, S, d), lse=e(B, H, S, dtype=F32), y_attn=e(M, d))
+                k = dict(O=e(B, S, d), lse=e(B, H, S, dtype=F32), y_attn=e(M, d), st1=e(M, 2, dtype=F32))
                 if b < cfg.num_layers:
-                    k.update(y_ff=e(M, d), x_mid=e(B, S, d))
+                    k.update(y_ff=e(M, d), x_mid=e(B, S, d), st2=e(M, 2, dtype=F32))
                 self.keep.append(k)
             self._ff_shape, self._ff_device = (M, 4 * d), device
             self._qkv_shape = (M, 3 * d)
@@ -119,7 +120,7 @@
         self.save = {k: (v[:M] if k in rows else v[:B]) for k, v in base.save.items()}
         self.keep = None
         if base.keep is not None:
-            self.keep = [{k: (v[:M] if k in ("y_attn", "y_ff", "hid_pre", "qkv") else v[:B]) for k, v in kb.items()}
+            self.keep = [{k: (v[:M] if k in ("y_attn", "y_ff", "hid_pre", "qkv", "st1", "st2") else v[:B]) for k, v in kb.items()}
                          for kb in base.keep]
         self.dX, self.dO, self.dQ, self.dK, self.dV, self.dOt, self.delta = (
             t[:B] for t in (base.dX, base.dO, base.dQ, base.dK, base.dV, base.dOt, base.delta))
@@ -180,25 +181,71 @@
         return (None,) * 9
 
 
-def _wgrad(model, tr, A, K, dC: Rows, N, wname, bname, rows=None):
+@dataclass
+class _LnRows:
+    x: Rows
+    shift: torch.Tensor
+    scale: torch.Tensor
+    mod_ld: int
+    stats: torch.Tensor = None
+
+    @property
+    def M(self):
+        return self.x.M
+
+
+def _dct(tr, N, M):
+    Mp = _pad64(M)
+    return tr.dCt[:N * Mp].view(N, Mp), Mp
+
+
+def _wgrad(model, tr, A, K, dC: Rows, N, wname, bname, rows=None, dct_done=0):
     st = model.store
     g = st.ensure_grad()
     parts = A if isinstance(A, list) else [(A, K, False)]
     M = parts[0][0].M
-    Mp = _pad64(M)
-    dCt = tr.dCt[:N * Mp].view(N, Mp)
+    dCt, Mp = _dct(tr, N, M)
     At = tr.At[:K * Mp].view(K, Mp)
     gb = None
     if bname is not None:
         gb = st.fused(g, bname, N) if rows else st.view(g, bname)
-    ops.transpose(dC, N, dCt, Mp, colsum_out=gb, colsum_beta=1.0)
+    if dct_done < N:
+        rest = dC if dct_done == 0 else Rows(dC.t.view(-1)[dct_done:], dC.M, dC.ld, dC.rpb, dC.bstride)
+        ops.transpose(rest, N - dct_done, dCt[dct_done:], Mp, colsum_out=None if gb is None else gb[dct_done:], colsum_beta=1.0)
     k0 = 0
     for a_rows, width, gelu in parts:
-        ops.transpose(a_rows, width, At[k0:k0 + width], Mp, gelu=gelu)
+        if isinstance(a_rows, _LnRows):
+            ops.ln_modulate_t(a_rows.x, a_rows.shift, a_rows.scale, a_rows.mod_ld, At[k0:k0 + width], Mp, width, stats=a_rows.stats)
+        else:
+            ops.transpose(a_rows, width, At[k0:k0 + width], Mp, gelu=gelu)
         k0 += width
     assert k0 == K
     gw = st.fused(g, wname, N) if rows else st.view(g, wname)
     ops.gemm(Rows.of(dCt), At, None, Rows(gw, N, K), K, Mp, EPI_F32_ACC, beta=1.0, ldw=Mp)
+
+
+def _gate_bwd(model, tr, dout: Rows, y, gate, gate_ld, dy, dgate, B, rows, D, bname):
+    if rows % 64 != 0:
+        ops.gate_bwd(dout, y, gate, gate_ld, dy, dgate, B, rows, D)
+        return 0
+    st = model.store
+    dyt, Mp = _dct(tr, D, B * rows)
+    ops.gate_bwd_t(dout, y, gate, gate_ld, dy, dgate, B, rows, D, dyt, Mp, st.view(st.ensure_grad(), bname))
+    return D
+
+
+def _qk_bwd(model, tr, qkv, p, nq, nk, cos, sin, dqkv, B, H, S, Sp, rows, s0, q_scale, N, bname, ld_dqkv=None):
+    st = model.store
+    g32 = st.ensure_grad()
+    args = (qkv, model.W32(f"{p}.attn.{nq}.weight"), model.W32(f"{p}.attn.{nk}.weight"), cos, sin, tr.dQ, tr.dK, tr.dV, dqkv,
+            st.view(g32, f"{p}.attn.{nq}.weight"), st.view(g32, f"{p}.attn.{nk}.weight"), B, H, S, Sp, rows, s0)
+    if not ops.qk_norm_rope_bwd_t_ok(B, rows):
+        ops.qk_norm_rope_bwd(*args, ld_dqkv=ld_dqkv, q_scale=q_scale)
+        return 0
+    d3 = qkv.shape[-1]
+    dct, Mp = _dct(tr, N, B * rows)
+    ops.qk_norm_rope_bwd_t(*args, dct, Mp, st.fused(g32, bname, N)[:d3], ld_dqkv=ld_dqkv, q_scale=q_scale)
+    return d3
 
 
 def _dgrad(model, tr, dC: Rows, N, K, wname, out: Rows, rows=None, epi=EPI_BIAS, aux=None, ldaux=None, row_lo=0,
@@ -251,10 +298,9 @@
 
     cout = cfg.patch_size * cfg.patch_size * cfg.in_channels
     e = sv["e"]
-    nrm = save["nrm1"][:B * N]
-    ops.ln_modulate(srows(tr.x_final, "img", d), e[:, d:2 * d], e[:, 0:d], 2 * d, nrm, d)
     dC = Rows.of(dout.view(B * N, cout))
-    _wgrad(model, tr, Rows.of(nrm), d, dC, cout, "proj_out.weight", "proj_out.bias")
+    _wgrad(model, tr, _LnRows(srows(tr.x_final, "img", d), e[:, d:2 * d], e[:, 0:d], 2 * d), d, dC, cout, "proj_out.weight",
+           "proj_out.bias")
     dn = tr.dnrm[:B * N]
     _dgrad(model, tr, dC, cout, d, "proj_out.weight", Rows.of(dn))
     tr.dX.zero_()
@@ -284,10 +330,11 @@
         dXr = Rows(tr.dX, M, d, S, S * d)
         cat2 = w.cat.view(M, 5 * d)
         lean = kept is not None and "hid_pre" in kept
-        ops.gate_bwd(dXr, save["y_attn"], m[:, 2 * d:3 * d], 3 * d, tr.dy, dmod[:, 2 * d:3 * d], B, S, d)
+        done = _gate_bwd(model, tr, dXr, save["y_attn"], m[:, 2 * d:3 * d], 3 * d, tr.dy, dmod[:, 2 * d:3 * d], B, S, d,
+                         f"{p}.proj_out.bias")
         dyr = Rows.of(tr.dy)
         a_op = [(Rows.of(kept["O"].view(M, d)), d, False), (Rows.of(kept["hid_pre"]), 4 * d, True)] if lean else Rows.of(cat2)
-        _wgrad(model, tr, a_op, 5 * d, dyr, d, f"{p}.proj_out.weight", f"{p}.proj_out.bias")
+        _wgrad(model, tr, a_op, 5 * d, dyr, d, f"{p}.proj_out.weight", f"{p}.proj_out.bias", dct_done=done)
         dcat = tr.dO.view(M, 5 * d)
         dO1 = tr.dO.view(-1)[:M * d].view(B, S, d)
         dbig = tr.dbig
@@ -304,11 +351,11 @@
             ops.attn_bwd(w.Q, w.K, save["V"], save["Qt"], save["Kt"], w.cat, tr.dO, lse_b, tr.delta, tr.dOt, tr.dQ, tr.dK,
                          tr.dV, B, H, S, Sp, 5 * d, S * 5 * d, scale)
         qkv_b = kept["qkv"] if kept is not None and "qkv" in kept else w.qkv
-        ops.qk_norm_rope_bwd(qkv_b, model.W32(f"{p}.attn.norm_q.weight"), model.W32(f"{p}.attn.norm_k.weight"), cos, sin,
-                             tr.dQ, tr.dK, tr.dV, dbig, store.view(g32, f"{p}.attn.norm_q.weight"),
-                             store.view(g32, f"{p}.attn.norm_k.weight"), B, H, S, Sp, S, 0, ld_dqkv=7 * d, q_scale=q_scale)
+        done = _qk_bwd(model, tr, qkv_b, p, "norm_q", "norm_k", cos, sin, dbig, B, H, S, Sp, S, 0, q_scale, 7 * d,
+                       f"{p}.attn.to_q.bias", ld_dqkv=7 * d)
         dbr = Rows.of(dbig)
-        _wgrad(model, tr, Rows.of(save["nrm1"]), d, dbr, 7 * d, f"{p}.attn.to_q.weight", f"{p}.attn.to_q.bias", rows=True)
+        a_op = _LnRows(x_in, m[:, 0:d], m[:, d:2 * d], 3 * d, kept["st1"]) if lean and "qkv" in kept else Rows.of(save["nrm1"])
+        _wgrad(model, tr, a_op, d, dbr, 7 * d, f"{p}.attn.to_q.weight", f"{p}.attn.to_q.bias", rows=True, dct_done=done)
         _dgrad(model, tr, dbr, 7 * d, d, f"{p}.attn.to_q.weight", Rows.of(tr.dnrm), rows=True)
         ops.ln_modulate_bwd(tr.dnrm, x_in, m[:, d:2 * d], 3 * d, dXr, True, dmod[:, 0:d], dmod[:, d:2 * d], d)
         _skinny_bwd(model, tr, dmod, st_, f"{p}.norm.linear.weight", f"{p}.norm.linear.bias", 3 * d, d, dst)
@@ -336,16 +383,20 @@
         dmods = {k: torch.empty(B, 6 * d, dtype=BF16, device=dev) for k in ("img", "txt")}
         for name, norm, qkvn, nq, nk, outn, ffn, rows, s0 in streams:
             m, dm = mods[name], dmods[name]
-            ops.gate_bwd(srows(tr.dX, name, d), save["y_ff"][sl[name]], m[:, 5 * d:6 * d], 6 * d, tr.dy[sl[name]],
-                         dm[:, 5 * d:6 * d], B, rows, d)
+            done = _gate_bwd(model, tr, srows(tr.dX, name, d), save["y_ff"][sl[name]], m[:, 5 * d:6 * d], 6 * d, tr.dy[sl[name]],
+                             dm[:, 5 * d:6 * d], B, rows, d, f"{p}.{ffn}.net.2.bias")
             a_op = [(Rows.of(kept["hid_pre"][sl[name]]), 4 * d, True)] if kept is not None and "hid_pre" in kept \
                 else Rows.of(w.hid[sl[name]])
-            _wgrad(model, tr, a_op, 4 * d, Rows.of(tr.dy[sl[name]]), d, f"{p}.{ffn}.net.2.weight", f"{p}.{ffn}.net.2.bias")
+            _wgrad(model, tr, a_op, 4 * d, Rows.of(tr.dy[sl[name]]), d, f"{p}.{ffn}.net.2.weight", f"{p}.{ffn}.net.2.bias",
+                   dct_done=done)
         _dgrad_pair(model, tr, Rows.of(tr.dy[sl["txt"]]), f"{p}.ff_context.net.2.weight", Rows.of(dh_all[sl["txt"]]),
                     Rows.of(tr.dy[sl["img"]]), f"{p}.ff.net.2.weight", Rows.of(dh_all[sl["img"]]), d, 4 * d, epi=EPI_DGELU,
                     aux1=save["hid_pre"][sl["txt"]], aux2=save["hid_pre"][sl["img"]], ldaux=4 * d)
         for name, norm, qkvn, nq, nk, outn, ffn, rows, s0 in streams:
-            _wgrad(model, tr, Rows.of(save["nrm2"][sl[name]]), d, Rows.of(dh_all[sl[name]]), 4 * d, f"{p}.{ffn}.net.0.proj.weight",
+            m = mods[name]
+            a_op = _LnRows(srows(save["x_mid"], name, d), m[:, 3 * d:4 * d], m[:, 4 * d:5 * d], 6 * d, kept["st2"][sl[name]]) \
+                if kept is not None and "hid_pre" in kept else Rows.of(save["nrm2"][sl[name]])
+            _wgrad(model, tr, a_op, d, Rows.of(dh_all[sl[name]]), 4 * d, f"{p}.{ffn}.net.0.proj.weight",
                    f"{p}.{ffn}.net.0.proj.bias")
         _dgrad_pair(model, tr, Rows.of(dh_all[sl["txt"]]), f"{p}.ff_context.net.0.proj.weight", Rows.of(tr.dnrm[sl["txt"]]),
                     Rows.of(dh_all[sl["img"]]), f"{p}.ff.net.0.proj.weight", Rows.of(tr.dnrm[sl["img"]]), 4 * d, d)
@@ -354,20 +405,23 @@
             dXs = srows(tr.dX, name, d)
             ops.ln_modulate_bwd(tr.dnrm[sl[name]], srows(save["x_mid"], name, d), m[:, 4 * d:5 * d], 6 * d, dXs, True,
                                 dm[:, 3 * d:4 * d], dm[:, 4 * d:5 * d], d)
-            ops.gate_bwd(dXs, save["y_attn"][sl[name]], m[:, 2 * d:3 * d], 6 * d, tr.dy[sl[name]], dm[:, 2 * d:3 * d], B, rows, d)
+            done = _gate_bwd(model, tr, dXs, save["y_attn"][sl[name]], m[:, 2 * d:3 * d], 6 * d, tr.dy[sl[name]],
+                             dm[:, 2 * d:3 * d], B, rows, d, f"{p}.attn.{outn}.bias")
             _wgrad(model, tr, srows(O_b, name, d), d, Rows.of(tr.dy[sl[name]]), d, f"{p}.attn.{outn}.weight",
-                   f"{p}.attn.{outn}.bias")
+                   f"{p}.attn.{outn}.bias", dct_done=done)
         _dgrad_pair(model, tr, Rows.of(tr.dy[sl["txt"]]), f"{p}.attn.to_add_out.weight", srows(dO3, "txt", d),
                     Rows.of(tr.dy[sl["img"]]), f"{p}.attn.to_out.0.weight", srows(dO3, "img", d), d, d)
         ops.attn_bwd(w.Q, w.K, save["V"], save["Qt"], save["Kt"], O_b, dO3, lse_b, tr.delta, tr.dOt, tr.dQ, tr.dK, tr.dV,
                      B, H, S, Sp, d, S * d, scale)
         qkv_b = kept["qkv"] if kept is not None and "qkv" in kept else w.qkv
         for name, norm, qkvn, nq, nk, outn, ffn, rows, s0 in streams:
-            ops.qk_norm_rope_bwd(qkv_b[sl[name]], model.W32(f"{p}.attn.{nq}.weight"), model.W32(f"{p}.attn.{nk}.weight"), cos,
-                                 sin, tr.dQ, tr.dK, tr.dV, dqkv_all[sl[name]], store.view(g32, f"{p}.attn.{nq}.weight"),
-                                 store.view(g32, f"{p}.attn.{nk}.weight"), B, H, S, Sp, rows, s0, q_scale=q_scale)
-            _wgrad(model, tr, Rows.of(save["nrm1"][sl[name]]), d, Rows.of(dqkv_all[sl[name]]), 3 * d, f"{p}.attn.{qkvn[0]}.weight",
-                   f"{p}.attn.{qkvn[0]}.bias", rows=True)
+            done = _qk_bwd(model, tr, qkv_b[sl[name]], p, nq, nk, cos, sin, dqkv_all[sl[name]], B, H, S, Sp, rows, s0, q_scale,
+                           3 * d, f"{p}.attn.{qkvn[0]}.bias")
+            m = mods[name]
+            a_op = _LnRows(srows(tr.block_in[i], name, d), m[:, 0:d], m[:, d:2 * d], 6 * d, kept["st1"][sl[name]]) \
+                if kept is not None and "qkv" in kept else Rows.of(save["nrm1"][sl[name]])
+            _wgrad(model, tr, a_op, d, Rows.of(dqkv_all[sl[name]]), 3 * d, f"{p}.attn.{qkvn[0]}.weight",
+                   f"{p}.attn.{qkvn[0]}.bias", rows=True, dct_done=done)
         _dgrad_pair(model, tr, Rows.of(dqkv_all[sl["txt"]]), f"{p}.attn.add_q_proj.weight", Rows.of(tr.dnrm[sl["txt"]]),
                     Rows.of(dqkv_all[sl["img"]]), f"{p}.attn.to_q.weight", Rows.of(tr.dnrm[sl["img"]]), 3 * d, d, rows=True)
         for name, norm, qkvn, nq, nk, outn, ffn, rows, s0 in streams:
diff --git a/mixgrpo_amd/ops.py b/mixgrpo_amd/ops.py
--- a/mixgrpo_amd/ops.py
+++ b/mixgrpo_amd/ops.py
@@ -130,9 +130,21 @@
                                    inp.rpb, inp.bstride, ld_out, stream()))
 
 
+def _colsum_finish(part, colsum_out, M, N, beta=1.0):
+    check(lib().mgx_colsum_finish(ptr(part), ptr(colsum_out), beta, (M + 127) // 128, N, stream()))
+
+
 def ln_modulate(x: Rows, shift, scale, mod_ld, y, D, stats=None):
     check(lib().mgx_ln_modulate_fwd(ptr(x.t), x.ld, x.rpb, x.bstride, shift.data_ptr(), scale.data_ptr(), mod_ld, ptr(y),
                                     D, ptr(stats), x.M, D, stream()))
+
+
+def ln_modulate_t(x: Rows, shift, scale, mod_ld, out, ld_out, D, stats=None):
+    ready = stats is not None
+    if not ready:
+        stats = scratch("ln_stats", 2 * x.M, F32, out.device)
+    check(lib().mgx_ln_modulate_fwd_t(ptr(x.t), x.ld, x.rpb, x.bstride, shift.data_ptr(), scale.data_ptr(), mod_ld, ptr(out),
+                                      ld_out, ptr(stats), int(ready), x.M, D, stream()))
 
 
 def ln_modulate_bwd(dy, x: Rows, scale, mod_ld, dx: Rows, accumulate, dshift, dscale, D):
@@ -158,6 +170,21 @@
     check(lib().mgx_qk_norm_rope_bwd_qs(ptr(qkv), qkv.shape[-1], ptr(wq), ptr(wk), ptr(cos), ptr(sin), ptr(dQ), ptr(dK),
                                         ptr(dV), dqkv.data_ptr(), qkv.shape[-1] if ld_dqkv is None else ld_dqkv, ptr(gwq),
                                         ptr(gwk), ptr(ws), B, H, S, Sp, rows_per_batch, s0, float(q_scale), stream()))
+
+
+def qk_norm_rope_bwd_t_ok(B, rows_per_batch):
+    return rows_per_batch % 128 == 0 or (B == 1 and rows_per_batch % 8 == 0)
+
+
+def qk_norm_rope_bwd_t(qkv, wq, wk, cos, sin, dQ, dK, dV, dqkv, gwq, gwk, B, H, S, Sp, rows_per_batch, s0, dct, ld_t, colsum_out,
+                       ld_dqkv=None, q_scale=1.0):
+    N, M = qkv.shape[-1], B * rows_per_batch
+    ws = scratch("qk_bwd", lib().mgx_qk_norm_rope_bwd_workspace(B, H, rows_per_batch), F32, qkv.device)
+    part = scratch("colsum_partial", lib().mgx_transpose_partial_elems(M, N), F32, qkv.device)
+    check(lib().mgx_qk_norm_rope_bwd_t(ptr(qkv), N, ptr(wq), ptr(wk), ptr(cos), ptr(sin), ptr(dQ), ptr(dK), ptr(dV),
+                                       dqkv.data_ptr(), N if ld_dqkv is None else ld_dqkv, ptr(gwq), ptr(gwk), ptr(ws), ptr(dct),
+                                       ld_t, ptr(part), B, H, S, Sp, rows_per_batch, s0, float(q_scale), stream()))
+    _colsum_finish(part, colsum_out, M, N)
 
 
 def linear_qk_norm_rope(X, Wqk, bias, wq, wk, cos, sin, Q, K, B, H, S, rows_per_batch, s0, Kdim, q_scale=1.0, pairs=None):
@@ -265,6 +292,15 @@
                              dgate.data_ptr(), ptr(ws), batches, rows_per_batch, D, stream()))
 
 
+def gate_bwd_t(dout: Rows, y, gate, gate_ld, dy, dgate, batches, rows_per_batch, D, dyt, ld_t, colsum_out):
+    M = batches * rows_per_batch
+    ws = scratch("gate_bwd", lib().mgx_gate_bwd_workspace(batches, rows_per_batch, D), F32, y.device)
+    part = scratch("colsum_partial", lib().mgx_transpose_partial_elems(M, D), F32, y.device)
+    check(lib().mgx_gate_bwd_t(ptr(dout.t), dout.ld, dout.bstride, ptr(y), D, gate.data_ptr(), gate_ld, ptr(dy), D,
+                               dgate.data_ptr(), ptr(ws), ptr(dyt), ld_t, ptr(part), batches, rows_per_batch, D, stream()))
+    _colsum_finish(part, colsum_out, M, D)
+
+
 def sqnorm(g, out, beta=0.0):
     ws = scratch("sqnorm", lib().mgx_sqnorm_workspace(), torch.float64, g.device)
     check(lib().mgx_sqnorm_f32(ptr(g), g.numel(), ptr(ws), ptr(out), beta, stream()))
diff --git a/scratch/ab_wgrad_operands.py b/scratch/ab_wgrad_operands.py
--- /dev/null
+++ b/scratch/ab_wgrad_operands.py
@@ -0,0 +1,72 @@
+import math
+import os
+import sys
+
+import torch
+
+sys.path.insert(0, os.path.dirname(os.path.dirname(os.path.abspath(__file__))))
+from mixgrpo_amd import ops
+from mixgrpo_amd.ops import Rows
+
+BF, dev = torch.bfloat16, "cuda"
+reps = int(sys.argv[1]) if len(sys.argv) > 1 else 20
+d, H, B, L, N = 3072, 24, 4, 512, 4096
+S = L + N
+QS = 1.4426950408889634 / math.sqrt(128)
+
+
+def timed(fn):
+    fn()
+    torch.cuda.synchronize()
+    out = []
+    for _ in range(5):
+        e0, e1 = torch.cuda.Event(enable_timing=True), torch.cuda.Event(enable_timing=True)
+        e0.record()
+        for _ in range(reps):
+            fn()
+        e1.record()
+        torch.cuda.synchronize()
+        out.append(e0.elapsed_time(e1) * 1e3 / reps)
+    return sorted(out)[2]
+
+
+def report(name, pair, fused):
+    a, b = timed(pair), timed(fused)
+    print(f"{name:44s} pair {a:8.1f} us   fused {b:8.1f} us   saved {a - b:7.1f} us ({100 * (a - b) / a:5.1f} %)", flush=True)
+
+
+g = torch.Generator(device=dev).manual_seed(0)
+rn = lambda *s: torch.randn(*s, device=dev, generator=g).to(BF)
+J = rn(B, S, d)
+for name, rows, off, k in (("txt", L, 0, 6), ("img", N, L, 6), ("single", S, 0, 3)):
+    M = B * rows
+    x = Rows(J[0, off:], M, d, rows, S * d)
+    mod = rn(B, k * d)
+    y, yt, stats = torch.empty(M, d, dtype=BF, device=dev), torch.empty(d, M, dtype=BF, device=dev), torch.empty(M, 2, device=dev)
+    ops.ln_modulate(x, mod[:, :d], mod[:, d:2 * d], k * d, y, d, stats=stats)
+    pair = lambda: (ops.ln_modulate(x, mod[:, :d], mod[:, d:2 * d], k * d, y, d), ops.transpose(Rows.of(y), d, yt, M))
+    report(f"ln_modulate {name} M={M} (stats recomputed)", pair, lambda: ops.ln_modulate_t(x, mod[:, :d], mod[:, d:2 * d], k * d, yt, M, d))
+    report(f"ln_modulate {name} M={M} (stats kept)", pair,
+           lambda: ops.ln_modulate_t(x, mod[:, :d], mod[:, d:2 * d], k * d, yt, M, d, stats=stats))
+    yy, dy, dg, gb = rn(M, d), torch.empty(M, d, dtype=BF, device=dev), torch.empty(B, d, dtype=BF, device=dev), torch.zeros(d, device=dev)
+    gate = mod[:, 2 * d:3 * d]
+    report(f"gate_bwd {name} M={M}",
+           lambda: (ops.gate_bwd(x, yy, gate, k * d, dy, dg, B, rows, d), ops.transpose(Rows.of(dy), d, yt, M, colsum_out=gb)),
+           lambda: ops.gate_bwd_t(x, yy, gate, k * d, dy, dg, B, rows, d, yt, M, gb))
+    del y, yy, dy
+cos = torch.rand(S, 128, device=dev, generator=g)
+sin = torch.rand(S, 128, device=dev, generator=g)
+wq, wk = torch.ones(128, device=dev), torch.ones(128, device=dev)
+dQ, dK, dV = rn(B, H, S, 128), rn(B, H, S, 128), rn(B, H, S, 128)
+for name, rows, s0, ldm in (("txt", L, 0, 3), ("img", N, L, 3), ("single", S, 0, 7)):
+    M = B * rows
+    qkv = rn(M, 3 * d)
+    dqkv = torch.empty(M, ldm * d, dtype=BF, device=dev)
+    dct = torch.empty(3 * d, M, dtype=BF, device=dev)
+    gwq, gwk, gb = torch.zeros(128, device=dev), torch.zeros(128, device=dev), torch.zeros(3 * d, device=dev)
+    args = (qkv, wq, wk, cos, sin, dQ, dK, dV, dqkv, gwq, gwk, B, H, S, S, rows, s0)
+    report(f"qk_norm_rope_bwd {name} M={M} ld={ldm}d",
+           lambda: (ops.qk_norm_rope_bwd(*args, ld_dqkv=ldm * d, q_scale=QS),
+                    ops.transpose(Rows(dqkv, M, ldm * d), 3 * d, dct, M, colsum_out=gb)),
+           lambda: ops.qk_norm_rope_bwd_t(*args, dct, M, gb, ld_dqkv=ldm * d, q_scale=QS))
+    del qkv, dqkv, dct
```

Result: no change. 0.4390, median of 2 (+0.2%).
